# justinhj/minbpe-cc

Hardware: AMD Instinct MI355X
Metric: bpe_train_merges_per_sec (higher is better)
Workload: dtype u16; 1 GPU; BASELINE config 4: SplitMix64(seed 42) uniform-random bytes, 4294967296 bytes whole job, basic encoder (one chunk), vocab 32000, lexicographic tie-break; a step is ONE WHOLE TRAINING (pair-count scan, stream and table setup, every merge up to the vocabulary: 31744 merges); corpus_bytes=4294967296, vocab_size=32000

## Files before the change

### include/mbpe.h

```cpp
#ifndef MBPE_H
#define MBPE_H

#include <stdint.h>

#ifdef __cplusplus
extern "C" {
#endif

#define MBPE_API __attribute__((visibility("default")))

#define MBPE_MAX_VOCAB_BASIC   65534u
#define MBPE_MAX_VOCAB_ENDBIT  32766u
#define MBPE_MAX_VOCAB_CHUNKED 65518u
#define MBPE_MAX_VOCAB_WIDE    16777216u
#define MBPE_NO_BARRIER 0xFFFFFFFFu

typedef enum {
    MBPE_NEED_EXCHANGE =  1,
    MBPE_OK            =  0,
    MBPE_ERR_ARG       = -1,
    MBPE_ERR_NO_DEVICE = -2,
    MBPE_ERR_HIP       = -3,
    MBPE_ERR_VOCAB     = -4,
    MBPE_ERR_STATE     = -5,
    MBPE_ERR_OOM       = -6,
    MBPE_ERR_REGEX     = -7,
    MBPE_ERR_SPLIT_GAP = -8,
    MBPE_ERR_COMM      = -9,
    MBPE_ERR_OVERFLOW  = -10,
    MBPE_ERR_IO        = -11
} mbpe_status;

typedef struct mbpe_ctx mbpe_ctx;

typedef struct {
    uint64_t n_bytes;
    uint64_t n_chunks;
    uint64_t n_slots;
    uint64_t n_live;
    uint32_t n_merges;
    uint32_t n_compactions;
    uint64_t n_pairs;
    float    ms_pair_count;
    float    ms_begin;
    float    ms_steps;
    uint32_t pair_count_launches;
    uint32_t merge_launches;
    float    ms_merge_kernel;
    uint32_t n_batches;
    uint32_t n_fused;
    uint32_t n_fused_dropped;
    uint32_t cut_conflict;
    uint32_t cut_bucket;
    uint32_t cut_single;
    uint32_t cut_full;
    uint32_t n_validation_drops;
    float    ms_grow_table;
    float    ms_compact;
    uint32_t n_table_grows;
    uint32_t n_sel_fallback;
    uint32_t fused_launches;
    float    ms_fused_kernel;
    uint64_t fused_slots;
    uint32_t n_sel_retry;
    uint32_t adapt_limit;
    uint64_t n_sel_blocks;
    uint32_t size_hist[8];
    uint32_t n_skipped;
    uint32_t n_skip_cut;
    uint64_t exchange_words;
    uint32_t exchanges;
    uint32_t pad_;
    uint64_t fused_live_tokens;
    float    ms_pair_count_kernel;
    uint32_t pad2_;
} mbpe_stats;

MBPE_API const char *mbpe_last_error(void);
MBPE_API const char *mbpe_version(void);


MBPE_API int  mbpe_create(int device_id, mbpe_ctx **out);
MBPE_API void mbpe_destroy(mbpe_ctx *ctx);


MBPE_API int mbpe_load_corpus(mbpe_ctx *ctx, const uint8_t *text, uint64_t n_bytes,
                              const uint64_t *chunk_off, uint64_t n_chunks,
                              int text_on_device);

MBPE_API int mbpe_load_corpus_endmask(mbpe_ctx *ctx, const uint8_t *text, uint64_t n_bytes, int text_on_device,
                                      const uint8_t *endmask_dev);

MBPE_API int mbpe_load_corpus_ranges(mbpe_ctx *ctx, const uint8_t *text, uint64_t n_bytes,
                                     const uint64_t *starts, const uint64_t *ends, uint64_t n_chunks,
                                     int text_on_device);

MBPE_API int mbpe_pair_count_u8(mbpe_ctx *ctx, uint32_t *table65536_out);


MBPE_API int mbpe_train_begin(mbpe_ctx *ctx, uint32_t vocab_size);

MBPE_API int mbpe_train_steps(mbpe_ctx *ctx, uint32_t n_steps, uint32_t *steps_done_out);

MBPE_API int mbpe_train_sequences(mbpe_ctx *ctx, uint32_t n_sequences, uint32_t *merges_done_out);

MBPE_API int mbpe_train_result(mbpe_ctx *ctx, uint32_t *merges_out, int32_t *counts_out,
                               uint32_t cap_merges, uint32_t *n_merges_out);

MBPE_API int mbpe_train_lexical(mbpe_ctx *ctx, const uint8_t *text, uint64_t n_bytes,
                                const uint64_t *chunk_off, uint64_t n_chunks,
                                uint32_t vocab_size,
                                uint32_t *merges_out, int32_t *counts_out,
                                uint32_t *n_merges_out, mbpe_stats *stats_out);

MBPE_API int mbpe_train(mbpe_ctx *ctx, const uint8_t *text, uint64_t n_bytes,
                        const uint64_t *chunk_off, uint64_t n_chunks, uint32_t vocab_size,
                        int conflict_resolution,
                        uint32_t *merges_out, int32_t *counts_out,
                        uint32_t *n_merges_out, mbpe_stats *stats_out);


MBPE_API int mbpe_merges_check(const uint32_t *merges, uint32_t n_merges);

MBPE_API int mbpe_train_begin_from(mbpe_ctx *ctx, uint32_t vocab_size, const uint32_t *prior_merges, uint32_t n_prior);

MBPE_API int mbpe_train_from(mbpe_ctx *ctx, const uint8_t *text, uint64_t n_bytes,
                             const uint64_t *chunk_off, uint64_t n_chunks, uint32_t vocab_size,
                             int conflict_resolution, const uint32_t *prior_merges, uint32_t n_prior,
                             uint32_t *merges_out, int32_t *counts_out,
                             uint32_t *n_merges_out, mbpe_stats *stats_out);

MBPE_API int mbpe_get_stats(mbpe_ctx *ctx, mbpe_stats *out);


MBPE_API int mbpe_get_stream(mbpe_ctx *ctx, uint32_t *tokens_out, uint8_t *chunk_end_out,
                             uint64_t cap, uint64_t *n_out);

MBPE_API int mbpe_stream_device(mbpe_ctx *ctx, const void **slots_out, uint64_t *n_slots_out,
                                uint32_t *slot_bits_out, uint32_t *end_bit_out, uint32_t *barrier_out);

MBPE_API int mbpe_table_device(mbpe_ctx *ctx, const void **cells_out, uint32_t *vshift_out);

MBPE_API int mbpe_get_pairs(mbpe_ctx *ctx, uint32_t *first_out, uint32_t *second_out,
                            int32_t *count_out, uint64_t cap, uint64_t *n_out);

MBPE_API int mbpe_compact(mbpe_ctx *ctx);

MBPE_API int mbpe_set_option(mbpe_ctx *ctx, const char *name, int64_t value);


MBPE_API int mbpe_encode_chunks(int device_id, const uint8_t *text, uint64_t n_bytes,
                                const uint64_t *chunk_off, uint64_t n_chunks,
                                const uint32_t *merges, uint32_t n_merges,
                                uint32_t *tokens_out, uint64_t cap, uint64_t *n_out,
                                uint32_t *n_passes_out);

MBPE_API int mbpe_encode_chunks_device(int device_id, const uint8_t *text, uint64_t n_bytes,
                                       const uint64_t *chunk_off, uint64_t n_chunks,
// ... 189 lines not shown
```

### minbpe-cc_amd/csrc/kernels.hip

```cpp
#include "mbpe_dev.h"
#include <hip/hip_ext.h>

#include <algorithm>
#include <cstdlib>

namespace mbpe {

namespace {

constexpr int kWave = 64;
constexpr uint32_t kSent = 0x10000u;

__device__ __forceinline__ uint32_t lane_id() { return threadIdx.x & (kWave - 1); }
__device__ __forceinline__ uint32_t rfl(uint32_t v) { return __builtin_amdgcn_readfirstlane(v); }

typedef unsigned int u32x4 __attribute__((ext_vector_type(4)));

__device__ __forceinline__ uint32_t wave_from_next(uint32_t v, uint32_t edge) {
    return (uint32_t)__builtin_amdgcn_update_dpp((int)edge, (int)v, 0x130, 0xf, 0xf, false);
}
__device__ __forceinline__ uint32_t wave_from_prev(uint32_t v, uint32_t edge) {
    return (uint32_t)__builtin_amdgcn_update_dpp((int)edge, (int)v, 0x138, 0xf, 0xf, false);
}

// ... 2286 lines not shown
    for (int j = 0; j < 8; ++j) {
        if (s[j] != kHole) {
            if (last == kHole) first_id = s[j] & idmask;
            if ((s[j] & idmask) == last) { ++len; repeats = true; }
            else { full = full && last == kHole; len = 1; }
            lodd |= (len & 1u) ? 0u : 1u << j;
            lead |= full ? 1u << j : 0u;
            last = s[j];
        }
    }
    const bool p1_runs = h.p1 != kHole && !(h.p1 & endbit);
    const uint32_t in_last = h.p1, in_len = p1_runs ? (rb_small & 1u) : 1u;
    uint32_t rl, rn;
    const bool cross = first_id == wave_from_prev(last, in_last);
    if (__ballot(last == kHole) == 0ull && __ballot(repeats || cross) == 0ull) {
        rl = rlane(last, kWave - 1);
        rn = 1u;
    } else {
    auto join = [&](uint32_t o_last, uint32_t o_len, bool o_full) {
        if (last == kHole) { last = o_last; len = o_len; full = o_full; }
        else if (o_last != kHole) {
            if (full && (last & idmask) == o_last) { len += o_len; full = o_full; }
            else full = false;
        }
    };
    if (__ballot(last == kHole || (full && cross)) != 0ull) {
        if (lane == 0) join(in_last, in_len, false);
#pragma unroll
        for (int d = 1; d < kWave; d <<= 1) {
            const uint32_t ol = __shfl_up(last, d, kWave), on = __shfl_up(len | (full ? 0x80000000u : 0u), d, kWave);
            if (lane >= (uint32_t)d) join(ol, on & 0x7FFFFFFFu, (on >> 31) != 0u);
        }
    }
    const uint32_t lv = wave_from_prev(last, in_last), ln = wave_from_prev(len, in_len);
    const uint32_t odd = lodd ^ ((first_id == lv && (ln & 1u)) ? lead : 0u);
    if (__ballot(odd != 0u) != 0ull) {
#pragma unroll
        for (int j = 0; j < 8; ++j)
            if ((odd >> j) & 1u) s[j] = stand_in(s[j]);
    }
    rl = rlane(last, kWave - 1);
    rn = rlane(len, kWave - 1);
    }
    if (h.n1 != kHole) {
        const uint32_t n1 = h.n1;
        const bool c1 = (n1 & idmask) == rl;
        if (c1 && (rn & 1u)) h.n1 = stand_in(n1);
        rn = c1 ? rn + 1u : 1u;
        rl = n1;
        if (h.n2 != kHole && (h.n2 & idmask) == rl && (rn & 1u)) h.n2 = stand_in(h.n2);
    }
    if (p1_runs) {
        const uint32_t p1 = h.p1, p2 = h.p2;
        if (!(rb_small & 1u)) h.p1 = stand_in(p1);
        if (p2 == p1 && (rb_small & 1u)) h.p2 = stand_in(p2);
    }
}

template <int MODE>
__device__ __forceinline__ bool tt_needed(const uint32_t s[8], const uint32_t nxt[8], const Halo &h,
                                          uint32_t tile_first, const TTInfo &ti, uint32_t live_mask = 0xFFu) {
    constexpr uint32_t idmask = MODE == 1 ? 0x7FFFu : 0xFFFFu;
    auto member = [&](uint32_t v) -> bool {
        const uint32_t id = v & idmask;
        return (ti.map[id & (kTTSlots - 1u)] & 0xFFFFu) == id;
    };
    uint32_t eqm = 0;
#pragma unroll
    for (int j = 0; j < 8; ++j) eqm |= (((s[j] ^ nxt[j]) & idmask) == 0u ? 1u : 0u) << j;
    eqm &= live_mask;
    bool need = false;
    if (__ballot(eqm != 0u) != 0ull) {
#pragma unroll
        for (int j = 0; j < 8; ++j)
            if ((eqm >> j) & 1u) need = need || member(s[j]);
    }
    bool hneed = false;
    if (h.p1 != kHole && (((h.p1 ^ tile_first) & idmask) == 0u || (h.p2 != kHole && ((h.p2 ^ h.p1) & idmask) == 0u)))
        hneed = member(h.p1);
    if (h.n1 != kHole && h.n2 != kHole && ((h.n1 ^ h.n2) & idmask) == 0u) hneed = hneed || member(h.n1);
    return __ballot(need) != 0ull || hneed;
}

template <int MODE, int DIAG, bool WRITE, bool TT, class DC>
__device__ __forceinline__ uint4 fused_tile_pf(const uint4 q_orig, const uint32_t s[8], const Halo h,
                                               uint32_t old_x, uint32_t old_y, uint32_t old_z, const BatchLut &lut,
                                               uint32_t X0, uint32_t tile, TileSum *sout, uint32_t *hdr_adj, uint32_t *LR,
                                               DC &dc, bool dc_on, uint32_t &wave_rm, bool &wrote_sum,
                                               __amdgpu_buffer_rsrc_t lr_rsrc, uint32_t adj_pitch, uint16_t *stage,
                                               uint32_t *chg, bool renamed, TTInfo *ti, bool &need_rename,
                                               __amdgpu_buffer_rsrc_t t_rsrc = __amdgpu_buffer_rsrc_t(), bool use_t = false);

template <int MODE, bool HOT, bool TT, int DIAG = 0>
__global__ __launch_bounds__(kLutThreads) void k_scan_batch(const uint16_t *tok0, const uint16_t *tok1,
                                                              const TileSum *__restrict__ sin, uint32_t n_tiles,
                                                              uint32_t *__restrict__ chg, const BatchState *bs,
                                                              uint32_t *hdr_m, uint32_t *hdr_adj, uint32_t *LR,
                                                              const DevCtl *ctl, const RankEdge *le,
                                                              const RankEdge *re,
                                                              const uint32_t *__restrict__ run_in, int hot_launched,
                                                              uint32_t *T) {
    constexpr uint32_t idmask = MODE == 1 ? 0x7FFFu : 0xFFFFu;
    __shared__ BatchLutMem lut_mem;
    const uint32_t waves_per_block = kLutThreads / kWave;
    const uint32_t n_waves = gridDim.x * waves_per_block;
    __shared__ DeltaCache dc;
    const uint32_t n_keys = ctl->batch_n;
    if (n_keys < 2 || ctl->fused) return;
    if ((bs->tt_index != kNoTT) != TT) return;
    __shared__ TTInfo ti;
    const uint16_t *tok = ctl->cur ? tok1 : tok0;
    const uint32_t ctl_k_done = rfl(ctl->k_done);
    const uint32_t adj_pitch = rfl(ctl->adj_pitch);
    if (hot_mismatch<HOT>(bs->packed[0] >> 32, ctl, hot_launched)) return;
    constexpr bool dc_on = HOT;
    if (dc_on) dc_init(dc);
    BatchLut lut(&lut_mem, bs, idmask);
    lut_build(lut, bs, n_keys, idmask - 1u);
    if (TT) tt_build(ti, bs, n_keys, idmask - 1u);
    uint32_t tile = rfl(blockIdx.x * waves_per_block + threadIdx.x / kWave);
    if (tile < n_tiles) {

    const uint32_t last_tile = n_tiles - 1;
    auto clamp_tile = [&](uint64_t t) { return (uint32_t)(t < n_tiles ? t : last_tile); };
    const __amdgpu_buffer_rsrc_t sums_rsrc =
        __builtin_amdgcn_make_buffer_rsrc(const_cast<TileSum *>(sin), 0, n_tiles * 16u, 0x00020000);
    const __amdgpu_buffer_rsrc_t lr_rsrc = __builtin_amdgcn_make_buffer_rsrc(LR, 0, 0xFFFFFFFCu, 0x00020000);
    const bool use_t = T != nullptr && !HOT && ctl->cells_on != 0u && n_keys >= ctl->cells_min;
    const __amdgpu_buffer_rsrc_t t_rsrc = __builtin_amdgcn_make_buffer_rsrc(T ? T : LR, 0, T ? 0xFFFFFFFCu : 0u, 0x00020000);
    TileIn t0 = tile_issue(tok, sums_rsrc, tile);
    TileIn t1 = tile_issue(tok, sums_rsrc, clamp_tile((uint64_t)tile + n_waves));
    bool v1 = (uint64_t)tile + n_waves < n_tiles;
    for (;;) {
        const bool v2 = (uint64_t)tile + 2ull * n_waves < n_tiles;
        TileIn t2 = tile_issue(tok, sums_rsrc, clamp_tile((uint64_t)tile + 2ull * n_waves));

        const uint32_t me_nlive = rlane(t0.smw, 6) & 0xFFFFu;
        if (me_nlive != 0) {
            uint32_t s[8];
            unpack8(t0.q, s);
            Halo h;
            const uint32_t pw1 = rlane(t0.smw, 1), pw2 = rlane(t0.smw, 2);
            const uint32_t nw0 = rlane(t0.smw, 8), nw2 = rlane(t0.smw, 10);
            const bool fast = tile > 0 && tile + 1 < n_tiles && (pw2 & 0xFFFFu) >= 2 && (nw2 & 0xFFFFu) >= 2;
            if (fast) {
                h.p1 = pw1 >> 16; h.p2 = pw1 & 0xFFFFu;
                h.n1 = nw0 & 0xFFFFu; h.n2 = nw0 >> 16;
            } else {
                h = halo_slow(sin, n_tiles, tile, le, re);
            }
            uint32_t rm_unused = 0;
            bool ws_unused = false, no_rename = false;
            if (TT) tt_rename<MODE>(s, h, ti, run_in[tile]);
            fused_tile_pf<MODE, 0, false, TT>(t0.q, s, h, rlane(t0.smw, 4), rlane(t0.smw, 5), rlane(t0.smw, 6), lut,
                                              256u + ctl_k_done, tile, nullptr, hdr_adj, LR, dc, dc_on, rm_unused, ws_unused,
                                              lr_rsrc, adj_pitch, nullptr, chg, TT, &ti, no_rename, t_rsrc, use_t);
        }
        if (!v1) break;
        tile += n_waves;
        t0 = t1; t1 = t2;
        v1 = v2;
    }
    }
    if (dc_on) dc_flush(dc, LR);
    if (TT) {
        tt_flush(ti, hdr_m);
    }
}

template <int MODE, int DIAG, bool WRITE, bool TT, class DC>
__device__ __forceinline__ uint4 fused_tile_pf(const uint4 q_orig, const uint32_t s[8], const Halo h,
                                               uint32_t old_x, uint32_t old_y, uint32_t old_z, const BatchLut &lut,
                                               uint32_t X0, uint32_t tile, TileSum *sout, uint32_t *hdr_adj, uint32_t *LR,
                                               DC &dc, bool dc_on, uint32_t &wave_rm, bool &wrote_sum,
                                               __amdgpu_buffer_rsrc_t lr_rsrc, uint32_t adj_pitch, uint16_t *stage,
                                               uint32_t *chg, bool renamed, TTInfo *ti, bool &need_rename,
                                               __amdgpu_buffer_rsrc_t t_rsrc, bool use_t) {
    constexpr uint32_t idmask = MODE == 1 ? 0x7FFFu : 0xFFFFu;
    constexpr uint32_t endbit = MODE == 1 ? kEndBit : 0u;
    constexpr uint32_t kNone = 0xFFFFu;
    const uint32_t pitch = lr_pitch(X0);
    const uint32_t xcd_off = DIAG == 6 ? (__builtin_amdgcn_s_getreg((3 << 11) | 20) & 7u) * (2u * 512u * pitch) : 0u;
    auto delta_add = [&](uint32_t idx, uint32_t delta) {
        if (dc_on) dc_add(dc, true, LR, idx, delta);
        else __builtin_amdgcn_raw_ptr_buffer_atomic_add_i32((int)delta, lr_rsrc, (idx + xcd_off) << 2, 0, 0);
    };
    uint32_t lane = lane_id();
    asm volatile("" : "+v"(lane));
    const uint32_t live = old_z & 0xFFFFu;
    if (live == 0u) return q_orig;
    uint32_t tile_first = old_x & 0xFFFFu, tile_last = old_y >> 16;
    if (TT && renamed) {
        const uint32_t li = live - 1u;
        uint32_t sl = s[0];
#pragma unroll
        for (uint32_t j = 1; j < 8; ++j) sl = (li & 7u) == j ? s[j] : sl;
        tile_first = rlane(s[0], 0);
        tile_last = rlane(sl, li >> 3);
    }
    uint32_t n[8];
#pragma unroll
    for (int j = 0; j < 7; ++j) n[j] = s[j + 1];
    n[7] = wave_from_next(s[0], h.n1);
    const uint32_t ef = lane == 0 ? h.p1 : lane == 1 ? h.p2 : lane == 2 ? tile_last : (TT && lane == 3) ? h.n1 : kHole;
    const uint32_t es = (lane == 0 ? tile_first : lane == 1 ? h.p1 : (TT && lane == 3) ? h.n2 : h.n1) & idmask;
    uint32_t idx[8], eidx;
    if (lut.bytes) {
#pragma unroll
        for (int j = 0; j < 8; ++j) idx[j] = byte_entry<TT>(lut, s[j], MODE == 1 ? n[j] & idmask : n[j], idmask);
        eidx = byte_entry<TT>(lut, ef, es, idmask);
        const uint32_t all = idx[0] & idx[1] & idx[2] & idx[3] & idx[4] & idx[5] & idx[6] & idx[7] & eidx;
        if (__ballot(all != kNone) == 0ull && DIAG != 3 && DIAG != 5) return q_orig;
        if (TT) {
            bool mark = eidx == kTTMark;
#pragma unroll
            for (int j = 0; j < 8; ++j) mark = mark || idx[j] == kTTMark;
            if (__ballot(mark) != 0ull) {
                if (!renamed) { need_rename = true; return q_orig; }
#pragma unroll
                for (int j = 0; j < 8; ++j) idx[j] = idx[j] == kTTMark ? kNone : idx[j];
                eidx = eidx == kTTMark ? kNone : eidx;
            }
            eidx = lane == 3 ? kNone : eidx;
        }
    } else {
        uint32_t Hm = 0, Wm = 0;
        {
            bool second_key;
            const bool hit = pair_hit2(lut, ef, es, second_key) && !(TT && lane == 3);
            Hm = hit ? 1u : 0u;
            Wm = second_key ? 1u : 0u;
        }
#pragma unroll
        for (int j = 7; j >= 0; --j) {
            bool second_key;
            const bool hit = pair_hit2(lut, s[j], MODE == 1 ? n[j] & idmask : n[j], second_key);
            Hm = Hm + Hm + (hit ? 1u : 0u);
            Wm = Wm + Wm + (second_key ? 1u : 0u);
        }
        if (__ballot(Hm != 0u) == 0ull && DIAG != 3 && DIAG != 5) return q_orig;
#pragma unroll
        for (int j = 0; j < 8; ++j) {
            idx[j] = kNone;
            if (__ballot(((Hm >> j) & 1u) != 0u) != 0ull) {
                const uint32_t got = lut_index_known(lut, s[j], MODE == 1 ? n[j] & idmask : n[j], ((Wm >> j) & 1u) != 0u);
                idx[j] = (Hm >> j) & 1u ? got : kNone;
            }
        }
        eidx = kNone;
        if (__ballot(((Hm >> 8) & 1u) != 0u) != 0ull) {
            const uint32_t got = lut_index_known(lut, ef, es, ((Wm >> 8) & 1u) != 0u);
            eidx = (Hm >> 8) & 1u ? got : kNone;
        }
    }
    if (DIAG == 3 || DIAG == 5) {
#pragma unroll
        for (int j = 0; j < 8; ++j) asm volatile("" :: "v"(idx[j]));
        asm volatile("" :: "v"(eidx));
        return q_orig;
    }
    const uint32_t in1 = rlane(eidx, 0), in2 = rlane(eidx, 1), out1 = rlane(eidx, 2);
    {
        const uint32_t li = live - 1u;
        const bool mine = lane == (li >> 3);
#pragma unroll
        for (uint32_t j = 0; j < 8; ++j)
            if ((li & 7u) == j) { n[j] = mine ? h.n1 : n[j]; idx[j] = mine ? out1 : idx[j]; }
    }
    const uint32_t prev7 = wave_from_prev(idx[7] | (s[7] << 16), in1 | (h.p1 << 16));
    const uint32_t prev6 = wave_from_prev(idx[6], in2);
    const int lrem = (int)live - (int)(lane * 8u);
    const uint32_t Lm = lrem >= 8 ? 0xFFu : lrem <= 0 ? 0u : (1u << lrem) - 1u;
    uint32_t Am = 0, Bm = 0;
#pragma unroll
    for (int j = 0; j < 8; ++j) {
        const uint32_t pj = j == 0 ? (prev7 & 0xFFFFu) : idx[j - 1];
        Am |= (idx[j] != kNone ? 1u : 0u) << j;
        Bm |= (pj != kNone ? 1u : 0u) << j;
    }
    Bm &= Lm;
    const uint32_t ABm = Am | Bm;
    if (__ballot(ABm != 0u) == 0ull) return q_orig;

    uint32_t n2_7 = wave_from_next(n[0], h.n2);
    uint32_t n2_patch = kSent;
    if (out1 != kNone) {
        const uint32_t li = live - 1u;
        if (lane == (li >> 3)) n2_patch = li & 7u;
    }
    uint32_t out[8];
#pragma unroll
    for (int j = 0; j < 8; ++j) {
        const uint32_t self = s[j];
        uint32_t nv = ((Bm >> j) & 1u) ? kHole : self;
        if (__ballot(((Am >> j) & 1u) != 0u) != 0ull) {
            if ((Am >> j) & 1u) {
                const uint32_t p1 = j == 0 ? prev7 >> 16 : s[j > 0 ? j - 1 : 0];
                const uint32_t ppj = j == 0 ? prev6 : j == 1 ? (prev7 & 0xFFFFu) : idx[j > 1 ? j - 2 : 0];
                const uint32_t ja = idx[j];
                const uint32_t btok = n[j];
                uint32_t n2 = j < 7 ? n[j < 7 ? j + 1 : 7] : n2_7;
                n2 = n2_patch == (uint32_t)j ? h.n2 : n2;
                nv = (X0 + ja) | (btok & endbit);
                if (TT && renamed && (btok & idmask) >= idmask - (uint32_t)kTTMax)
                    atomicAdd(&ti->cnt[idmask - 1u - (btok & idmask)], 1u);
                if (DIAG != 2) {
                    const bool lo = left_open<MODE>(p1), ro = right_open<MODE>(btok, n2);
                    const uint32_t xl = p1 & idmask, yr = n2 & idmask;
                    if (use_t && lo && ro && ppj == kNone && xl < 256u && yr < 256u) {
                        __builtin_amdgcn_raw_ptr_buffer_atomic_add_i32(1, t_rsrc, ((ja << 16) | (xl << 8) | yr) << 2, 0, 0);
                    } else {
                        if (lo) {
                            if (ppj != kNone) {
                                atomicAdd(&hdr_adj[ppj * adj_pitch + ja], 1u);
                                delta_add(lr_idx(pitch, self, ppj, 1), 0xFFFFFFFFu);
                            } else {
                                delta_add(lr_idx(pitch, xl, ja, 0u), 1u);
                            }
                        }
                        if (ro) delta_add(lr_idx(pitch, yr, ja, 1u), 1u);
                    }
                }
            }
        }
        out[j] = nv;
    }
    if (TT && renamed) {
#pragma unroll
        for (int j = 0; j < 8; ++j)
            if (out[j] != kHole && (out[j] & idmask) >= idmask - (uint32_t)kTTMax)
                out[j] = ti->tok[idmask - 1u - (out[j] & idmask)] | (out[j] & endbit);
    }
    if (!WRITE) {
        if (lane == 0) atomicOr(&chg[tile >> 5], 1u << (tile & 31u));
        return q_orig;
    }
    uint32_t n_out;
    const uint4 qc = tile_compact(out, stage, n_out);
    wave_rm += live - n_out;
    uint32_t em = lane == 0 ? 3u : 0u;
    {
        const uint32_t l1 = live - 1u, l2 = live >= 2u ? live - 2u : 0u;
        em |= lane == (l1 >> 3) ? 1u << (l1 & 7u) : 0u;
        em |= lane == (l2 >> 3) ? 1u << (l2 & 7u) : 0u;
    }
    const bool edge = __ballot((ABm & em) != 0u) != 0ull;
    uint4 ns;
    if (edge || (old_z >> 16) != 1u) {
        uint32_t c[8];
        unpack8(qc, c);
        ns = wave_summary(c);
    } else {
        ns = make_uint4(old_x, old_y, (old_z & 0xFFFF0000u) | n_out, 0u);
    }
    if (lane == 0) reinterpret_cast<uint4 *>(sout)[tile] = ns;
    wrote_sum = true;
    return qc;
}

#ifndef MBPE_SKIP_PENALTY0
#define MBPE_SKIP_PENALTY0 2
#endif
#ifndef MBPE_SKIP_PENALTY_MAX
#define MBPE_SKIP_PENALTY_MAX 256
#endif
#ifndef MBPE_FUSED_WAVES
#define MBPE_FUSED_WAVES 4
#endif
template <int MODE, bool HOT, bool TT, int DIAG = 0>
__global__ __launch_bounds__(kLutThreads, MBPE_FUSED_WAVES * 256 / kLutThreads) void k_fused_batch(uint16_t *tok0, uint16_t *tok1,
                                                               const TileSum *__restrict__ sin,
                                                               TileSum *__restrict__ sout, uint32_t n_tiles,
                                                               uint32_t *__restrict__ chg, const BatchState *bs,
                                                               uint32_t *hdr_adj, uint32_t *LR, DevCtl *ctl,
                                                               const RankEdge *le, const RankEdge *re,
                                                               uint32_t *hdr_m, const uint32_t *__restrict__ run_in,
                                                               int hot_launched, uint32_t *T) {
    constexpr uint32_t idmask = MODE == 1 ? 0x7FFFu : 0xFFFFu;
    __shared__ BatchLutMem lut_mem;
    const uint32_t lane = lane_id();
    const uint32_t waves_per_block = kLutThreads / kWave;
    const uint32_t n_waves = gridDim.x * waves_per_block;
    __shared__ DeltaCacheSmall dc;
    const uint32_t n_keys = ctl->batch_n;
    if (n_keys < 2 || !ctl->fused) return;
    if ((bs->tt_index != kNoTT) != TT) return;
    __shared__ TTInfo ti;
    __shared__ __attribute__((aligned(16))) uint16_t stage_mem[kLutThreads / kWave][kTileSlots];
    uint16_t *stage = stage_mem[threadIdx.x / kWave];
    const uint16_t *tok = ctl->cur ? tok1 : tok0;
    uint16_t *dst = ctl->cur ? tok0 : tok1;
    const uint32_t X0 = 256u + ctl->k_done;
    if (hot_mismatch<HOT>(bs->packed[0] >> 32, ctl, hot_launched)) return;
    constexpr bool dc_on = HOT;
    if (dc_on) dc_init(dc);
    BatchLut lut(&lut_mem, bs, idmask);
    lut_build(lut, bs, n_keys, idmask - 1u, TT);
    if (TT) tt_build(ti, bs, n_keys, idmask - 1u);
    if (blockIdx.x == 0 && threadIdx.x == 0) ctl->marks_all = 1;
    uint32_t tile = rfl(blockIdx.x * waves_per_block + threadIdx.x / kWave);
    uint32_t wave_rm = 0;
    if (tile < n_tiles) {

    const uint32_t last_tile = n_tiles - 1;
    auto clamp_tile = [&](uint64_t t) { return (uint32_t)(t < n_tiles ? t : last_tile); };
    const __amdgpu_buffer_rsrc_t sums_rsrc =
        __builtin_amdgcn_make_buffer_rsrc(const_cast<TileSum *>(sin), 0, n_tiles * 16u, 0x00020000);
    const __amdgpu_buffer_rsrc_t lr_rsrc = __builtin_amdgcn_make_buffer_rsrc(LR, 0, 0xFFFFFFFCu, 0x00020000);
    const bool use_t = T != nullptr && !HOT && ctl->cells_on != 0u && n_keys >= ctl->cells_min;
    const __amdgpu_buffer_rsrc_t t_rsrc = __builtin_amdgcn_make_buffer_rsrc(T ? T : LR, 0, T ? 0xFFFFFFFCu : 0u, 0x00020000);
    const uint32_t adj_pitch = rfl(ctl->adj_pitch);
#ifndef MBPE_FUSED_DEPTH
#define MBPE_FUSED_DEPTH 2
#endif
    constexpr int kDepth = MBPE_FUSED_DEPTH;
    TileIn ring[kDepth];
#pragma unroll
    for (int d = 0; d < kDepth; ++d) ring[d] = tile_issue(tok, sums_rsrc, clamp_tile((uint64_t)tile + (uint64_t)d * n_waves));
    for (;;) {
        const bool v1 = (uint64_t)tile + n_waves < n_tiles;
        const TileIn t_new = tile_issue(tok, sums_rsrc, clamp_tile((uint64_t)tile + (uint64_t)kDepth * n_waves));
        const TileIn t0 = ring[0];

        uint4 outq = t0.q;
        bool wrote_sum = false;
        const uint32_t old_x = rlane(t0.smw, 4), old_y = rlane(t0.smw, 5), old_z = rlane(t0.smw, 6);
        if (DIAG == 4) {
            asm volatile("" :: "v"(t0.smw));
        } else if ((old_z & 0xFFFFu) != 0) {
            uint32_t s[8];
            unpack8(t0.q, s);
            Halo h;
            const uint32_t pw1 = rlane(t0.smw, 1), pw2 = rlane(t0.smw, 2);
            const uint32_t nw0 = rlane(t0.smw, 8), nw2 = rlane(t0.smw, 10);
            const bool fast = tile > 0 && tile + 1 < n_tiles && (pw2 & 0xFFFFu) >= 2 && (nw2 & 0xFFFFu) >= 2;
            if (fast) {
                h.p1 = pw1 >> 16; h.p2 = pw1 & 0xFFFFu;
                h.n1 = nw0 & 0xFFFFu; h.n2 = nw0 >> 16;
            } else {
                h = halo_slow(sin, n_tiles, tile, le, re);
            }
            bool renamed = false;
            bool need_rename = false;
            if (TT && !lut.bytes) {
                uint32_t nx[8];
#pragma unroll
                for (int j = 0; j < 7; ++j) nx[j] = s[j + 1];
                nx[7] = wave_from_next(s[0], h.n1);
                const uint32_t li = (old_z & 0xFFFFu) - 1u;
                const bool mine = lane == (li >> 3);
#pragma unroll
                for (uint32_t j = 0; j < 8; ++j)
                    if ((li & 7u) == j) nx[j] = mine ? h.n1 : nx[j];
                const int lrem = (int)(old_z & 0xFFFFu) - (int)(lane * 8u);
                const uint32_t lm = lrem >= 8 ? 0xFFu : lrem <= 0 ? 0u : (1u << lrem) - 1u;
                if (tt_needed<MODE>(s, nx, h, old_x & 0xFFFFu, ti, lm)) {
                    tt_rename<MODE>(s, h, ti, run_in[tile]);
                    renamed = true;
                }
            }
            outq = fused_tile_pf<MODE, DIAG, true, TT>(t0.q, s, h, old_x, old_y, old_z, lut, X0, tile, sout, hdr_adj, LR, dc,
                                                       dc_on, wave_rm, wrote_sum, lr_rsrc, adj_pitch, stage, chg, renamed, &ti,
                                                       need_rename, t_rsrc, use_t);
            if (TT && need_rename) {
                tt_rename<MODE>(s, h, ti, run_in[tile]);
                outq = fused_tile_pf<MODE, DIAG, true, TT>(t0.q, s, h, old_x, old_y, old_z, lut, X0, tile, sout, hdr_adj, LR,
                                                           dc, dc_on, wave_rm, wrote_sum, lr_rsrc, adj_pitch, stage, chg, true,
                                                           &ti, need_rename, t_rsrc, use_t);
            }
        }
        if (!wrote_sum && lane == 0) reinterpret_cast<uint4 *>(sout)[tile] = make_uint4(old_x, old_y, old_z, 0u);
        MBPE_GLOBAL_AS char *obase =
            (MBPE_GLOBAL_AS char *)uniform_ptr(reinterpret_cast<uintptr_t>(dst) + (uint64_t)tile * (kWave * 16u));
        u32x4 oq; oq.x = outq.x; oq.y = outq.y; oq.z = outq.z; oq.w = outq.w;
        __builtin_nontemporal_store(oq, (MBPE_GLOBAL_AS u32x4 *)(obase + lane * 16u));

        if (!v1) break;
        tile += n_waves;
#pragma unroll
        for (int d = 0; d + 1 < kDepth; ++d) ring[d] = ring[d + 1];
        ring[kDepth - 1] = t_new;
    }
    }
    if (dc_on) dc_flush(dc, LR);
    if (lane == 0 && wave_rm) atomicAdd(&ctl->rm, wave_rm);
    if (TT) {
        tt_flush(ti, hdr_m);
    }
}

__global__ __launch_bounds__(256) void k_pair_cells_fold(uint32_t *__restrict__ T, uint32_t *__restrict__ LR, const DevCtl *ctl) {
    __shared__ uint32_t rows[256];
    const uint32_t n = ctl->batch_n;
    if (n < ctl->cells_min || !ctl->cells_on) return;
    const uint32_t pitch = lr_pitch(256u + ctl->k_done);
    uint32_t hits = 0;
    const uint32_t t = threadIdx.x;
    for (uint32_t j = blockIdx.x; j < n; j += gridDim.x) {
        uint32_t *tj = T + (size_t)j * 65536u;
        rows[t] = 0;
        __syncthreads();
        uint32_t col = 0;
#pragma unroll 8
        for (uint32_t x = 0; x < 256u; ++x) {
            const uint32_t v = tj[x * 256u + t];
            if (__ballot(v != 0u) == 0ull) continue;
            if (v) tj[x * 256u + t] = 0;
            col += v;
            const uint32_t rs = wave_sum(v);
            if (lane_id() == 0 && rs) atomicAdd(&rows[x], rs);
        }
        __syncthreads();
        if (col) LR[lr_idx(pitch, t, j, 1u)] += col;
        if (rows[t]) LR[lr_idx(pitch, t, j, 0u)] += rows[t];
        hits += col;
        __syncthreads();
    }
    hits = wave_sum(hits);
    if (lane_id() == 0 && hits) atomicAdd(const_cast<uint32_t *>(&ctl->cell_hits), hits);
}


__global__ __launch_bounds__(kWave) void k_adj_sums(const uint32_t *__restrict__ hdr_adj, BatchState *bs, const DevCtl *ctl) {
    const uint32_t n = ctl->batch_n;
    if (n < 2) return;
    for (uint32_t j = blockIdx.x; j < n; j += gridDim.x) {
        uint32_t in = 0, out = 0;
        for (uint32_t p = threadIdx.x; p < n; p += kWave) { in += hdr_adj[p * ctl->adj_pitch + j]; out += hdr_adj[j * ctl->adj_pitch + p]; }
        in = wave_sum(in);
        out = wave_sum(out);
        if (threadIdx.x == 0) { bs->adj_in[j] = in; bs->adj_out[j] = out; }
    }
}

constexpr uint32_t kLrChunk = 4096;
__global__ __launch_bounds__(256) void k_delta_max(const uint32_t *__restrict__ LR, BatchState *bs, const DevCtl *ctl) {
    const uint32_t n_keys = ctl->batch_n;
    if (n_keys < 2) return;
    const uint32_t X = 256u + ctl->k_done;
    const uint32_t pitch = lr_pitch(X);
    const uint32_t chunks = (X + kLrChunk - 1u) / kLrChunk;
    const uint32_t n_items = 2u * n_keys * chunks;
    for (uint32_t item = blockIdx.x; item < n_items; item += gridDim.x) {
        const uint32_t row = item / chunks, x0 = (item - row * chunks) * kLrChunk;
        const uint32_t j = row >> 1, side = row & 1u, Xj = X + j;
        const uint32_t add = side ? bs->adj_out[j] : bs->adj_in[j];
        const uint32_t *cells = LR + (size_t)row * pitch;
        unsigned long long mp = 0;
#pragma unroll 4
        for (uint32_t x = x0 + threadIdx.x; x < x0 + kLrChunk && x < X; x += 256u) {
            const uint32_t v = cells[x];
            if (v) {
                const unsigned long long p = pack_best((int32_t)(v + add), side ? (Xj << 16) | x : (x << 16) | Xj);
                mp = p > mp ? p : mp;
            }
        }
        mp = wave_max_u64(mp);
        if (lane_id() == 0 && mp > __hip_atomic_load(&bs->maxp[j], __ATOMIC_RELAXED, __HIP_MEMORY_SCOPE_AGENT))
            atomicMax(&bs->maxp[j], mp);
    }
}

constexpr int kValThreads = kBatchMax < 256 ? 256 : kBatchMax > 1024 ? 1024 : kBatchMax;
constexpr int kValSlots = kBatchMax < 256 ? 256 : kBatchMax;
__global__ __launch_bounds__(256) void k_adj_max(const uint32_t *__restrict__ hdr_adj, BatchState *bs, const DevCtl *ctl) {
    const uint32_t n = ctl->batch_n;
    if (n < 2) return;
    const uint32_t X0 = 256u + ctl->k_done;
    const uint32_t n_waves = gridDim.x * (blockDim.x / kWave);
    for (uint32_t p = blockIdx.x * (blockDim.x / kWave) + threadIdx.x / kWave; p < n; p += n_waves) {
        for (uint32_t q = lane_id(); q < n; q += kWave) {
            const uint32_t w = hdr_adj[p * ctl->adj_pitch + q];
            if (!w) continue;
            const uint32_t bp = bs->key[p] & 0xFFFFu, aq = bs->key[q] >> 16;
            auto raise = [&](uint32_t j, unsigned long long v) {
                if (v > __hip_atomic_load(&bs->maxp[j], __ATOMIC_RELAXED, __HIP_MEMORY_SCOPE_AGENT)) atomicMax(&bs->maxp[j], v);
            };
            raise(q > p ? q : p, pack_best((int32_t)w, ((X0 + p) << 16) | (X0 + q)));
            raise(q, pack_best((int32_t)bs->adj_in[q], (bp << 16) | (X0 + q)));
            raise(p, pack_best((int32_t)bs->adj_out[p], ((X0 + p) << 16) | aq));
        }
    }
}

__global__ __launch_bounds__(kValThreads) void k_validate(PairTable t, DevCtl *ctl, BatchState *bs, uint32_t *hdr_m,
                                                          uint32_t *hdr_adj, uint32_t *LR) {
    static_assert(kValSlots % kValThreads == 0, "one workgroup validates a batch, kValSlots / kValThreads pairs per thread");
    constexpr uint32_t kPer = kValSlots / kValThreads;
    __shared__ unsigned long long s_run[kValSlots];
    __shared__ uint32_t s_commit, s_minfrac;
    const uint32_t tid = threadIdx.x;
    const uint32_t n = ctl->batch_n;
    if (n < 2) return;
    if (tid == 0) s_minfrac = 0xFFFFFFFFu;
    const uint32_t X0 = 256u + ctl->k_done;
    const uint32_t pitch = lr_pitch(X0);
#pragma unroll
    for (uint32_t u = 0; u < kPer; ++u) { const uint32_t p = tid + u * kValThreads; s_run[p] = p < n ? bs->maxp[p] : 0ull; }
    if (tid == 0) s_commit = n;
    __syncthreads();
    uint32_t nsh = 6;
    while ((1u << nsh) < n) ++nsh;
// ... 345 lines not shown
    if (TT) tt_build(ti, bs, n_keys, idmask - 1u);
    const uint32_t lane = lane_id();
    const uint32_t waves_per_block = kLutThreads / kWave;
    const uint32_t n_waves = gridDim.x * waves_per_block;
    uint32_t i = rfl(blockIdx.x * waves_per_block + threadIdx.x / kWave);
    if (i >= n_list) return;
    const __amdgpu_buffer_rsrc_t sums_rsrc =
        __builtin_amdgcn_make_buffer_rsrc(const_cast<TileSum *>(sin), 0, n_tiles * 16u, 0x00020000);
    const uint32_t last = n_list - 1;
    auto tile_at = [&](uint64_t k) { return list[k < n_list ? k : last]; };
    uint32_t tile0 = tile_at(i), tile1 = tile_at((uint64_t)i + n_waves), tile2 = tile_at((uint64_t)i + 2ull * n_waves);
    TileIn t0 = tile_issue(tok, sums_rsrc, tile0);
    TileIn t1 = tile_issue(tok, sums_rsrc, tile1);
    uint32_t wave_rm = 0;
    for (;;) {
        const bool has_next = (uint64_t)i + n_waves < n_list;
        const uint32_t tile3 = tile_at((uint64_t)i + 3ull * n_waves);
        const TileIn t2 = tile_issue(tok, sums_rsrc, tile2);

        const uint32_t tile = tile0;
        uint32_t s[8];
        unpack8(t0.q, s);
        Halo h;
        const uint32_t pw1 = rlane(t0.smw, 1), pw2 = rlane(t0.smw, 2);
        const uint32_t nw0 = rlane(t0.smw, 8), nw2 = rlane(t0.smw, 10);
        const bool fast = tile > 0 && tile + 1 < n_tiles && (pw2 & 0xFFFFu) >= 2 && (nw2 & 0xFFFFu) >= 2;
        if (fast) {
            h.p1 = pw1 >> 16; h.p2 = pw1 & 0xFFFFu;
            h.n1 = nw0 & 0xFFFFu; h.n2 = nw0 >> 16;
        } else {
            h = halo_slow(sin, n_tiles, tile, le, re);
        }
        uint32_t rm = 0;
        bool wrote = false;
        bool no_rename = false;
        DeltaCacheSmall no_dc;
        if (TT) tt_rename<MODE>(s, h, ti, run_in[tile]);
        const uint4 qn = fused_tile_pf<MODE, 2, true, TT>(t0.q, s, h, rlane(t0.smw, 4), rlane(t0.smw, 5), rlane(t0.smw, 6), lut,
                                                          X0, tile, sout, nullptr, nullptr, no_dc, false, rm, wrote,
                                                          __amdgpu_buffer_rsrc_t(), 0u, stage, chg, TT, &ti, no_rename);
        if (wrote) {
            reinterpret_cast<uint4 *>(tok)[(uint64_t)tile * kWave + lane] = qn;
            if (lane == 0 && marks_all) atomicOr(&chg[tile >> 5], 1u << (tile & 31u));
        } else if (lane == 0 && !marks_all) {
            atomicAnd(&chg[tile >> 5], ~(1u << (tile & 31u)));
        }
        wave_rm += rm;

        if (!has_next) break;
        i += n_waves;
        tile0 = tile1; tile1 = tile2; tile2 = tile3;
        t0 = t1; t1 = t2;
    }
    if (lane == 0 && wave_rm) atomicAdd(&ctl->rm, wave_rm);
}

__global__ void k_seq_finish(DevCtl *ctl, uint32_t *fused_flag, const BatchState *bs) {
    if (blockIdx.x || threadIdx.x) return;
    const uint32_t bs_skip_n = bs->skip_n;
    const uint32_t rm_seq = ctl->batch_n >= 2 ? ctl->rm : 0u;
    if (fused_flag) *fused_flag = ctl->fused && ctl->batch_n >= 2 ? 1u : 0u;
    if (ctl->batch_n >= 2) {
        const uint32_t rm = ctl->rm;
        ctl->removed_total += rm;
        ctl->n_live -= rm;
        ctl->rm = 0;
    }
    if (ctl->batch_n >= 2) {
        uint32_t lim = ctl->adapt_limit ? ctl->adapt_limit : (uint32_t)kBatchMax;
        if (ctl->commit_n < ctl->batch_n) lim = ctl->commit_n * 2u < 4u ? 4u : ctl->commit_n * 2u;
        else if (ctl->batch_n >= lim) lim = lim * 2u;
        ctl->adapt_limit = lim > (uint32_t)kBatchMax ? (uint32_t)kBatchMax : lim;
    }
    if (ctl->skip_off) ctl->skip_off -= 1;
    if (ctl->batch_n >= 2 && ctl->skip_failed) {
        const uint32_t pen = ctl->skip_penalty ? (ctl->skip_penalty * 2u > (uint32_t)MBPE_SKIP_PENALTY_MAX ? (uint32_t)MBPE_SKIP_PENALTY_MAX : ctl->skip_penalty * 2u)
                                               : (uint32_t)MBPE_SKIP_PENALTY0;
        ctl->skip_penalty = pen;
        ctl->skip_off = pen;
    } else if (ctl->batch_n >= 2 && bs_skip_n > 0 && ctl->skip_penalty) {
        ctl->skip_penalty /= 2u;
    }
    ctl->skip_failed = 0;
    if (ctl->cells_on && ctl->cells_min >= kCellsMinBatch && ctl->batch_n >= ctl->cells_min &&
        ctl->cell_hits * 2ull < (unsigned long long)rm_seq)
        ctl->cells_on = 0;
    ctl->cell_hits = 0;
    if (ctl->fused && ctl->batch_n >= 2) {
        ctl->n_fused += 1;
        if (ctl->commit_n == ctl->batch_n) ctl->cur ^= 1u;
        else ctl->n_fused_dropped += 1;
    }
    ctl->fused = 0;
    ctl->marks_all = 0;
    if (ctl->commit_n) ctl->size_hist[31 - __builtin_clz(ctl->commit_n) > 7 ? 7 : 31 - __builtin_clz(ctl->commit_n)] += 1;
    if (fused_flag) {
        fused_flag[1] = (uint32_t)ctl->n_live;
        fused_flag[2] = (uint32_t)(ctl->n_live >> 32);
        fused_flag[3] = ctl->commit_n;
    }
    ctl->k_done += ctl->commit_n;
    ctl->batch_n = 0;
    ctl->commit_n = 0;
    ctl->n_marked = 0;
}


constexpr int kScanThreads = 256;
constexpr int kScanPerThread = 16;
constexpr uint32_t kScanChunk = kScanThreads * kScanPerThread;

__device__ __forceinline__ unsigned long long block_sum_u64(unsigned long long v, unsigned long long *sh) {
#pragma unroll
    for (int d = kWave / 2; d > 0; d >>= 1) v += shfl_xor_u64(v, d);
    __syncthreads();
    if (lane_id() == 0) sh[threadIdx.x / kWave] = v;
    __syncthreads();
    unsigned long long r = 0;
    for (uint32_t w = 0; w < blockDim.x / kWave; ++w) r += sh[w];
    return r;
}

__global__ __launch_bounds__(kScanThreads) void k_tile_scan_partial(const TileSum *__restrict__ sums,
                                                                    uint32_t n_tiles,
                                                                    unsigned long long *__restrict__ part) {
    __shared__ unsigned long long sh[kScanThreads / kWave];
    const uint64_t base = (uint64_t)blockIdx.x * kScanChunk;
    unsigned long long s = 0;
    for (uint32_t i = threadIdx.x; i < kScanChunk; i += kScanThreads)
        if (base + i < n_tiles) s += sums[base + i].n_live;
    s = block_sum_u64(s, sh);
    if (threadIdx.x == 0) part[blockIdx.x] = s;
}

__global__ __launch_bounds__(1024) void k_tile_scan_top(unsigned long long *__restrict__ part, uint32_t n_parts,
                                                        DevCtl *ctl) {
    __shared__ unsigned long long tot[1024];
    const uint32_t per = (n_parts + 1023u) / 1024u;
    const uint32_t lo = threadIdx.x * per < n_parts ? threadIdx.x * per : n_parts;
    const uint32_t hi = lo + per < n_parts ? lo + per : n_parts;
    unsigned long long s = 0;
    for (uint32_t i = lo; i < hi; ++i) s += part[i];
    tot[threadIdx.x] = s;
    __syncthreads();
    if (threadIdx.x == 0) {
        unsigned long long run = 0;
        for (int i = 0; i < 1024; ++i) { const unsigned long long v = tot[i]; tot[i] = run; run += v; }
        ctl->scan_total = run;
    }
    __syncthreads();
    unsigned long long run = tot[threadIdx.x];
    for (uint32_t i = lo; i < hi; ++i) { const unsigned long long v = part[i]; part[i] = run; run += v; }
}

__global__ __launch_bounds__(kScanThreads) void k_tile_scan_final(const TileSum *__restrict__ sums, uint32_t n_tiles,
                                                                  const unsigned long long *__restrict__ part,
                                                                  unsigned long long *__restrict__ offsets) {
    __shared__ unsigned long long th[kScanThreads];
    const uint64_t first = (uint64_t)blockIdx.x * kScanChunk + (uint64_t)threadIdx.x * kScanPerThread;
    uint32_t v[kScanPerThread];
    unsigned long long s = 0;
#pragma unroll
    for (int i = 0; i < kScanPerThread; ++i) {
        v[i] = first + i < n_tiles ? sums[first + i].n_live : 0u;
        s += v[i];
    }
    th[threadIdx.x] = s;
// ... 487 lines not shown
    if (!v.n_tiles) return;
    const uint32_t n_chunks = (v.n_tiles + kRunChunk - 1) / kRunChunk;
    hipLaunchKernelGGL(k_run_partial, dim3(n_chunks), dim3(kRunThreads), 0, v.stream, v.sums, v.n_tiles, best, v.ctl, seq, bs,
                       v.run_part);
    hipLaunchKernelGGL(k_run_final, dim3(n_chunks), dim3(kRunThreads), 0, v.stream, v.sums, v.n_tiles, best, v.ctl, seq, bs,
                       v.run_part, v.left_edge, v.run_in);
}

void launch_merge(const StreamView &v, const BatchView &b, const unsigned long long *best, uint32_t new_id,
                  uint32_t *m_adj, int seq, const Inst &w) {
    if (!v.n_tiles) return;
    const BatchState *bs = seq ? b.bs : nullptr;
    if (inst_may_tt(w)) launch_run_lengths(v, bs, best, seq);
    static const int occ[3] = {resident_blocks(k_merge<0, false, 0>), resident_blocks(k_merge<1, false, 0>),
                               resident_blocks(k_merge<2, false, 0>)};
    const dim3 grid(tile_grid(v.n_tiles, v.n_cus, occ[slot_mode(v.endbit)])), block(kMergeThreads);
    const int hot_launched = w.hot;
#define MBPE_MERGE_ARGS v.tok, v.tok_other, v.sums, v.side, v.n_tiles, v.chg, best, new_id, b.LR, v.ctl, m_adj, v.left_edge, \
                        v.right_edge, seq, v.run_in, hot_launched
#ifdef MBPE_DIAG
    static const int diag = getenv("MBPE_MERGE_DIAG") ? atoi(getenv("MBPE_MERGE_DIAG")) : 0;
    if (diag == 1 && !v.endbit) {
        hipLaunchKernelGGL((k_merge<0, false, 1>), grid, block, 0, v.stream, MBPE_MERGE_ARGS);
        return;
    }
    if (diag == 2 && !v.endbit) {
        hipLaunchKernelGGL((k_merge<0, false, 2>), grid, block, 0, v.stream, MBPE_MERGE_ARGS);
        return;
    }
#endif
    MBPE_BY_MODE(v.endbit, {
        if (inst_takes(w, w.tt, false)) hipLaunchKernelGGL((k_merge<M, false, 0>), grid, block, 0, v.stream, MBPE_MERGE_ARGS);
        if (inst_takes(w, w.tt, true)) hipLaunchKernelGGL((k_merge<M, true, 0>), grid, block, 0, v.stream, MBPE_MERGE_ARGS);
    });
#undef MBPE_MERGE_ARGS
}

void launch_apply(const StreamView &v, const BatchView &b, PairTable t, const unsigned long long *best, uint32_t new_id,
                  const uint32_t *gm_gadj, int seq) {
    const uint32_t n_words = (v.n_tiles + 31u) / 32u;
    uint32_t blocks = (new_id + 255) / 256;
    const uint32_t want = (n_words + 255) / 256;
    if (want > blocks) blocks = want < 2048 ? want : 2048;
    hipLaunchKernelGGL(k_apply, dim3(blocks), dim3(256), 0, v.stream, t, v.ctl, best, new_id, b.LR, gm_gadj, v.sums, v.side,
                       v.chg, n_words, seq);
}

void launch_patch_sums(const StreamView &v, const unsigned long long *best, int seq) {
    const uint32_t n_words = (v.n_tiles + 31u) / 32u;
    uint32_t blocks = (n_words + 255) / 256;
    if (blocks > 2048) blocks = 2048;
    if (blocks < 1) blocks = 1;
    hipLaunchKernelGGL(k_patch_sums, dim3(blocks), dim3(256), 0, v.stream, best, v.sums, v.side, v.chg, n_words, v.ctl, seq,
                       v.n_tiles);
}

void launch_select_batch(const StreamView &v, const BatchView &b, PairTable t, unsigned long long *best,
                         const SelectArgs &a, int attempts, int first_attempt, bool fallback) {
    const hipStream_t s = v.stream;
    const uint32_t fake_id = (v.endbit == kEndBit ? 0x7FFFu : 0xFFFFu) - 1u;
    const uint32_t tt_max = 256u + a.n_target <= fake_id + 1u - (uint32_t)kTTMax ? (uint32_t)kTTMax : 1u;
    const uint32_t sel_cap = a.sel_cap < 64u ? 64u : a.sel_cap > kSelCap ? kSelCap : a.sel_cap;
    if (a.sel) {
        const int blocks = (v.n_cus > 0 ? v.n_cus : 256) * 4;
        for (int attempt = first_attempt < 0 ? 0 : first_attempt; attempt < (attempts < 1 ? 1 : attempts > 3 ? 3 : attempts); ++attempt) {
            hipLaunchKernelGGL(k_sel_scan, dim3(blocks), dim3(256), 0, s, t, v.ctl, a.sel, a.n_target, sel_cap, attempt);
            hipLaunchKernelGGL(k_sel_pick, dim3(1), dim3(kPickThreads), 0, s, v.ctl, b.bs, a.sel, best, a.n_target, a.max_batch,
                               a.fused_min, (uint32_t)v.n_ranks, attempt, fake_id, sel_cap, tt_max, a.byte_table ? 1u : 0u);
        }
    }
    if (fallback)
        hipLaunchKernelGGL(k_select_batch, dim3(1), dim3(kHierThreads), 0, s, t, v.ctl, b.bs, best, a.n_target, a.max_batch,
                           a.fused_min, (uint32_t)v.n_ranks);
}

void launch_fused_batch(const StreamView &v, const BatchView &b, const Inst &w) {
    if (!v.n_tiles) return;
    static const int occ[3] = {resident_blocks(k_fused_batch<0, false, false, 0>, kLutThreads),
                               resident_blocks(k_fused_batch<1, false, false, 0>, kLutThreads),
                               resident_blocks(k_fused_batch<2, false, false, 0>, kLutThreads)};
    const dim3 grid(tile_grid(v.n_tiles, v.n_cus, occ[slot_mode(v.endbit)], kLutThreads)), block(kLutThreads);
    const int hot_launched = w.hot;
#define MBPE_FUSED_ARGS v.tok, v.tok_other, v.sums, v.side, v.n_tiles, v.chg, b.bs, b.hdr_adj, b.LR, v.ctl, v.left_edge, \
                        v.right_edge, b.hdr_m, v.run_in, hot_launched, b.pair_cells
#ifdef MBPE_DIAG
    const int diag = getenv("MBPE_FUSED_DIAG") ? atoi(getenv("MBPE_FUSED_DIAG")) : 0;
#define MBPE_FUSED_DIAG_CASE(D)                                                                                            \
    if (diag == D && !v.endbit) {                                                                                          \
        hipLaunchKernelGGL((k_fused_batch<0, false, false, D>), grid, block, 0, v.stream, MBPE_FUSED_ARGS);                \
        hipLaunchKernelGGL((k_fused_batch<0, false, true, D>), grid, block, 0, v.stream, MBPE_FUSED_ARGS);                 \
        return;                                                                                                            \
    }
    MBPE_FUSED_DIAG_CASE(2)
    MBPE_FUSED_DIAG_CASE(3)
    MBPE_FUSED_DIAG_CASE(4)
    MBPE_FUSED_DIAG_CASE(5)
    MBPE_FUSED_DIAG_CASE(6)
#undef MBPE_FUSED_DIAG_CASE
#endif
    MBPE_BY_MODE(v.endbit, MBPE_BY_INST(w, hipLaunchKernelGGL((k_fused_batch<M, HOT, TT>), grid, block, 0, v.stream, MBPE_FUSED_ARGS)));
#undef MBPE_FUSED_ARGS
}

void launch_scan_batch(const StreamView &v, const BatchView &b, const Inst &w) {
    if (!v.n_tiles) return;
    static const int occ[3] = {resident_blocks(k_scan_batch<0, false, false, 0>, kLutThreads),
                               resident_blocks(k_scan_batch<1, false, false, 0>, kLutThreads),
                               resident_blocks(k_scan_batch<2, false, false, 0>, kLutThreads)};
    const dim3 grid(tile_grid(v.n_tiles, v.n_cus, occ[slot_mode(v.endbit)], kLutThreads)), block(kLutThreads);
    const int hot_launched = w.hot;
    MBPE_BY_MODE(v.endbit, MBPE_BY_INST(w, hipLaunchKernelGGL((k_scan_batch<M, HOT, TT, 0>), grid, block, 0, v.stream, v.tok,
                                                             v.tok_other, v.sums, v.n_tiles, v.chg, b.bs, b.hdr_m, b.hdr_adj, b.LR,
                                                             v.ctl, v.left_edge, v.right_edge, v.run_in, hot_launched,
                                                             b.pair_cells)));
}

void launch_pair_cells_fold(const StreamView &v, const BatchView &b, uint32_t n_hint) {
    if (!b.pair_cells) return;
    if (n_hint < 64u) n_hint = 64u;
    if (n_hint > 1024u) n_hint = 1024u;
    hipLaunchKernelGGL(k_pair_cells_fold, dim3(n_hint), dim3(256), 0, v.stream, b.pair_cells, b.LR, v.ctl);
}

void launch_batch_tables(const StreamView &v, const BatchView &b, PairTable t, uint32_t id_upper, uint32_t n_hint) {
    const hipStream_t s = v.stream;
    if (n_hint < 64u) n_hint = 64u;
    if (n_hint > (uint32_t)kBatchMax) n_hint = kBatchMax;
    const uint64_t cells = (uint64_t)id_upper * kBatchMax;
    uint32_t blocks = (uint32_t)((cells + 255) / 256);
    if (blocks > 2048) blocks = 2048;
    if (blocks < 8) blocks = 8;
    hipLaunchKernelGGL(k_adj_sums, dim3(n_hint), dim3(kWave), 0, s, b.hdr_adj, b.bs, v.ctl);
    hipLaunchKernelGGL(k_delta_max, dim3(blocks < 1024 ? blocks : 1024), dim3(256), 0, s, b.LR, b.bs, v.ctl);
    hipLaunchKernelGGL(k_adj_max, dim3(n_hint / 4), dim3(256), 0, s, b.hdr_adj, b.bs, v.ctl);
    hipLaunchKernelGGL(k_validate, dim3(1), dim3(kValThreads), 0, s, t, v.ctl, b.bs, b.hdr_m, b.hdr_adj, b.LR);
    if (t.cells) {
        uint32_t j_parts = (n_hint + kApplyTile - 1) / kApplyTile;
        if (j_parts > kApplyJParts) j_parts = kApplyJParts;
        uint32_t grid = ((id_upper + kApplyTile - 1) / kApplyTile) * j_parts;
        if (grid < 256u) grid = 256u;
        hipLaunchKernelGGL(k_apply_batch_dense, dim3(grid), dim3(256), 0, s, t, v.ctl, b.bs, b.hdr_m, b.hdr_adj, b.LR, j_parts);
    } else {
        hipLaunchKernelGGL(k_apply_batch, dim3(blocks), dim3(256), 0, s, t, v.ctl, b.bs, b.hdr_m, b.hdr_adj, b.LR);
    }
}

void launch_rewrite_marked(const StreamView &v, const BatchView &b, const Inst &w) {
    if (!v.n_tiles) return;
    const uint32_t n_words = (v.n_tiles + 31u) / 32u;
    hipLaunchKernelGGL(k_list_marked, dim3((n_words + 255) / 256), dim3(256), 0, v.stream, v.chg, n_words, v.tile_list, v.ctl,
                       v.n_tiles);
    static const int occ[3] = {resident_blocks(k_rewrite_marked<0, false>, kLutThreads),
                               resident_blocks(k_rewrite_marked<1, false>, kLutThreads),
                               resident_blocks(k_rewrite_marked<2, false>, kLutThreads)};
    const dim3 grid(tile_grid(v.n_tiles, v.n_cus, occ[slot_mode(v.endbit)], kLutThreads)), block(kLutThreads);
#define MBPE_REWRITE_ARGS v.tok, v.tok_other, v.sums, v.side, v.n_tiles, v.chg, v.tile_list, b.bs, v.ctl, v.left_edge, \
                          v.right_edge, v.run_in
    MBPE_BY_MODE(v.endbit, {
        hipLaunchKernelGGL((k_rewrite_marked<M, false>), grid, block, 0, v.stream, MBPE_REWRITE_ARGS);
        if (inst_may_tt(w)) hipLaunchKernelGGL((k_rewrite_marked<M, true>), grid, block, 0, v.stream, MBPE_REWRITE_ARGS);
    });
#undef MBPE_REWRITE_ARGS
}

__global__ void k_seq_info(const DevCtl *ctl, const BatchState *bs, const unsigned long long *best, uint32_t *out) {
    if (blockIdx.x || threadIdx.x) return;
    const uint32_t n = ctl->batch_n;
    unsigned long long top = 0;
    uint32_t tt = 0;
    if (n >= 2) {
        top = bs->packed[0] >> 32;
        tt = bs->tt_index != kNoTT ? 1u : 0u;
    } else if (n == 1) {
        const unsigned long long b = best[ctl->k_done];
        const uint32_t key = ~(uint32_t)b;
        top = b >> 32;
        tt = (top != 0 && (key >> 16) == (key & 0xFFFFu)) ? 1u : 0u;
    }
    out[0] = ctl->k_done;
    out[1] = n;
    out[2] = ctl->fused;
    out[3] = tt;
    out[4] = dc_wanted(top, ctl->n_live * ctl->n_ranks) ? 1u : 0u;
    out[5] = ctl->k_limit;
    out[6] = ctl->sel_ok;
    out[7] = 0;
}

void launch_seq_info(const StreamView &v, const BatchView &b, const unsigned long long *best, uint32_t *out) {
    hipLaunchKernelGGL(k_seq_info, dim3(1), dim3(64), 0, v.stream, v.ctl, b.bs, best, out);
}

void launch_seq_finish(const StreamView &v, const BatchView &b, uint32_t *fused_flag) {
    hipLaunchKernelGGL(k_seq_finish, dim3(1), dim3(64), 0, v.stream, v.ctl, fused_flag, b.bs);
}

void launch_tile_scan(const StreamView &v, unsigned long long *offsets) {
    if (!v.n_tiles) return;
    unsigned long long *part = offsets + v.n_tiles;
    const uint32_t n_parts = (v.n_tiles + kScanChunk - 1) / kScanChunk;
    hipLaunchKernelGGL(k_tile_scan_partial, dim3(n_parts), dim3(kScanThreads), 0, v.stream, v.sums, v.n_tiles, part);
    hipLaunchKernelGGL(k_tile_scan_top, dim3(1), dim3(1024), 0, v.stream, part, n_parts, v.ctl);
    hipLaunchKernelGGL(k_tile_scan_final, dim3(n_parts), dim3(kScanThreads), 0, v.stream, v.sums, v.n_tiles, part, offsets);
}
// ... 70 lines not shown
```

### minbpe-cc_amd/csrc/mbpe_dev.h

```cpp
#ifndef MBPE_DEV_H
#define MBPE_DEV_H

#include <hip/hip_runtime.h>
#include <stdint.h>

namespace mbpe {

constexpr uint32_t kHole = 0xFFFFu;
constexpr uint32_t kEndBit = 0x8000u;
constexpr uint32_t kBarrier = 0xFFEEu;

constexpr int kTile = 512;
constexpr int kMergeThreads = 256;
#ifndef MBPE_LUT_THREADS
#define MBPE_LUT_THREADS 1024
#endif
constexpr int kLutThreads = MBPE_LUT_THREADS;
constexpr int kSlotsPerLane = 8;

struct __attribute__((aligned(16))) TileSum {
    uint16_t head0, head1;
    uint16_t tail1, tail0;
    uint16_t n_live;
    uint16_t tail_run;
    uint16_t pad0, pad1;
};
static_assert(sizeof(TileSum) == 16, "TileSum must be 16 bytes");

struct RankEdge {
    uint32_t head0, head1;
    uint32_t tail1, tail0;
    uint32_t n_live_lo, n_live_hi;
    uint32_t tail_run_lo, tail_run_hi;
};

constexpr uint32_t kEmptyKey = 0xFFFFFFFFu;
constexpr unsigned long long kEmptySlot = 0xFFFFFFFFFFFFFFFFull;

constexpr int kBlockShift = 10;
constexpr uint32_t kBlockSize = 1u << kBlockShift;

struct PairTable {
    unsigned long long *hslot;
    uint32_t *ekey;
    int32_t  *ecnt;
    unsigned long long *bmax;
    unsigned long long *smax;
    uint32_t  hmask;
    uint32_t  ecap;
    uint32_t *cells;
    uint32_t  vshift;
};
constexpr uint32_t kPresent = 0x80000000u;

struct DevCtl {
    uint32_t n_entries;
    uint32_t err;
    uint32_t m;
    uint32_t adj;
    unsigned long long removed_total;
    unsigned long long n_live;
    unsigned long long scan_total;
    uint32_t rm;
    uint32_t k_done;
    uint32_t k_limit;
    uint32_t batch_n;
    uint32_t commit_n;
    uint32_t n_batches;
    uint32_t n_marked;
    uint32_t cur;
    uint32_t fused;
    uint32_t n_fused;
    uint32_t n_fused_dropped;
    uint32_t cut_conflict, cut_bucket, cut_single, cut_full;
    uint32_t n_validation_drops;
    unsigned long long sel_T;
    uint32_t sel_n;
    uint32_t sel_ok;
    uint32_t n_sel_fallback;
    uint32_t sel_retry;
    uint32_t adapt_limit;
    uint32_t recent_n;
    uint32_t n_sel_retry;
    uint32_t sel_mode;
    uint32_t n_ranks;
    uint32_t size_hist[8];
    uint32_t n_skipped;
    uint32_t n_skip_cut;
    uint32_t skip_off;
    uint32_t skip_penalty;
    uint32_t skip_failed;
    uint32_t skip_red_q16;
    unsigned long long n_sel_blocks;
    uint32_t first_mode;
    uint32_t first_tie;
    uint32_t marks_all;
    uint32_t cells_on;
    uint32_t cell_hits;
    uint32_t cells_min;
    uint32_t adj_pitch;

};

#ifndef MBPE_BATCH_MAX
#define MBPE_BATCH_MAX 4096
#endif
constexpr int kBatchMax = MBPE_BATCH_MAX;
constexpr int kBatchDefault = kBatchMax;
static_assert((kBatchMax & (kBatchMax - 1)) == 0 && kBatchMax >= 64,
              "a power of two: grid strides over the delta arrays keep a thread on one pair index");
#ifndef MBPE_SEL_CAP
#define MBPE_SEL_CAP 8192
#endif
constexpr uint32_t kSelCap = MBPE_SEL_CAP;
struct SelList {
    unsigned long long packed[kSelCap];
    uint32_t eidx[kSelCap];
};

#ifndef MBPE_TT_MAX
#define MBPE_TT_MAX 16
#endif
constexpr int kTTMax = MBPE_TT_MAX;
static_assert(0xFFFFu - (uint32_t)MBPE_TT_MAX > kBarrier, "the barrier id must lie below the stand-in ids");
constexpr uint32_t kTTSlots = 256;
#ifndef MBPE_SKIP_MAX
#define MBPE_SKIP_MAX 32
#endif
constexpr int kSkipMax = MBPE_SKIP_MAX;
constexpr uint32_t kCellsMinBatch = 512;
constexpr uint32_t kNoTT = 0xFFFFFFFFu;
struct BatchState {
    uint32_t key[kBatchMax];
    uint32_t eidx[kBatchMax];
    unsigned long long packed[kBatchMax];
    unsigned long long maxp[kBatchMax];
    uint32_t adj_in[kBatchMax];
    uint32_t adj_out[kBatchMax];
    uint32_t tt_index;
    uint32_t tt_token;
    uint32_t tt_n;
    uint32_t hash_mul;
    uint32_t byte_lut;
    uint32_t skip_n;
    uint32_t skip_key[kSkipMax];
    uint32_t skip_pos[kSkipMax];
    unsigned long long skip_packed[kSkipMax];
};

inline uint32_t batch_header_words(uint32_t adj_pitch) { return (uint32_t)kBatchMax + adj_pitch * adj_pitch; }
__host__ __device__ inline uint32_t lr_pitch(uint32_t ids) { return (ids + 63u) & ~63u; }
__host__ __device__ inline unsigned long long lr_words(uint32_t ids, uint32_t n_pairs) {
    return 2ull * (n_pairs ? n_pairs : 1u) * lr_pitch(ids);
}

constexpr uint32_t kErrTableFull   = 1u;
constexpr uint32_t kErrNegCount    = 2u;
constexpr uint32_t kErrMissingPair = 4u;
constexpr uint32_t kErrCountRange  = 8u;
constexpr uint32_t kErrHotSkipped  = 16u;

__host__ __device__ inline unsigned long long pack_best(int32_t count, uint32_t key) {
    return ((unsigned long long)(uint32_t)count << 32) | (uint32_t)(~key);
}

struct StreamView {
    hipStream_t stream;
    uint16_t *tok, *tok_other;
    TileSum *sums;
    TileSum *side;
    uint32_t n_tiles;
    uint32_t *chg;
    uint32_t *tile_list;
    uint32_t *run_in;
    unsigned long long *run_part;
    DevCtl *ctl;
    const RankEdge *left_edge, *right_edge;
    int rank, n_ranks;
    uint32_t endbit;
    int n_cus;
};

struct BatchView {
    BatchState *bs;
    uint32_t *hdr_m, *hdr_adj;
    uint32_t *LR;
    uint32_t *pair_cells;
};

struct Inst { bool known, tt, hot; };
inline Inst inst_any(bool hot_possible) { return Inst{false, false, hot_possible}; }
inline Inst inst_known(bool tt, bool hot) { return Inst{true, tt, hot}; }
inline bool inst_takes(const Inst &w, bool tt, bool hot) { return w.known ? w.tt == tt && w.hot == hot : !hot || w.hot; }
inline bool inst_may_tt(const Inst &w) { return !w.known || w.tt; }

void launch_fill_u32(hipStream_t s, uint32_t *p, uint64_t n, uint32_t v);
void launch_fill_u16(hipStream_t s, uint16_t *p, uint64_t n, uint16_t v);

size_t pair_count_scratch_bytes(int n_workgroups);
void launch_pair_count_u8(hipStream_t s, const uint8_t *text, uint64_t n,
                          const uint8_t *endmask, uint32_t *bp, int n_workgroups, uint32_t *scratch,
                          hipEvent_t start = nullptr, hipEvent_t stop = nullptr);

void launch_widen(hipStream_t s, const uint8_t *text, uint64_t n, const uint8_t *endmask,
                  uint16_t *tok, uint64_t n_slots_padded);
void launch_widen_barrier(hipStream_t s, const uint8_t *text, uint64_t n, const uint8_t *endmask,
                          uint16_t *tok, uint64_t n_slots);

void launch_summarize(const StreamView &v);

void launch_table_init(hipStream_t s, const uint32_t *bp, PairTable t, DevCtl *ctl);
void launch_table_rehash(hipStream_t s, PairTable t, DevCtl *ctl);

void launch_argmax(hipStream_t s, PairTable t, const DevCtl *ctl, unsigned long long *best, bool hierarchical);

size_t first_state_bytes();
void launch_first_init(hipStream_t s, void *fs);
void launch_first_tiebreak(const StreamView &v, PairTable t, unsigned long long *best, void *fs, uint32_t *xf, int seq,
                           int phase);

void launch_merge(const StreamView &v, const BatchView &b, const unsigned long long *best, uint32_t new_id,
                  uint32_t *m_adj, int seq, const Inst &w);
void launch_run_lengths(const StreamView &v, const BatchState *bs, const unsigned long long *best, int seq);

void launch_apply(const StreamView &v, const BatchView &b, PairTable t, const unsigned long long *best, uint32_t new_id,
                  const uint32_t *gm_gadj, int seq);
void launch_patch_sums(const StreamView &v, const unsigned long long *best, int seq);

struct SelectArgs {
    SelList *sel;
    uint32_t n_target, max_batch, fused_min, sel_cap;
    bool byte_table;
};
void launch_select_batch(const StreamView &v, const BatchView &b, PairTable t, unsigned long long *best,
                         const SelectArgs &a, int attempts = 3,
                         int first_attempt = 0 ,
                         bool fallback = true );
void launch_scan_batch(const StreamView &v, const BatchView &b, const Inst &w);
void launch_fused_batch(const StreamView &v, const BatchView &b, const Inst &w);
void launch_pair_cells_fold(const StreamView &v, const BatchView &b, uint32_t n_hint);
void launch_batch_tables(const StreamView &v, const BatchView &b, PairTable t, uint32_t id_upper, uint32_t n_hint);
void launch_rewrite_marked(const StreamView &v, const BatchView &b, const Inst &w);
void launch_seq_info(const StreamView &v, const BatchView &b, const unsigned long long *best, uint32_t *out);
void launch_seq_finish(const StreamView &v, const BatchView &b, uint32_t *fused_flag);

inline size_t tile_scan_scratch(uint32_t n_tiles) { return (size_t)n_tiles / 4096 + 2; }
void launch_tile_scan(const StreamView &v, unsigned long long *offsets);
void launch_compact_scatter(const StreamView &v, const unsigned long long *offsets);

inline uint32_t exchange_header_words(int n_ranks) { return (uint32_t)((2 + 8 * n_ranks + 3) / 4 * 4); }
void launch_rank_edge(const StreamView &v, uint32_t *hdr);
void launch_compose_edges(hipStream_t s, uint32_t *hdr, int rank, int n_ranks, RankEdge *left, RankEdge *right);
constexpr uint32_t kPairCountWords = 4;
void launch_boundary_pairs(hipStream_t s, uint32_t *bp, const uint32_t *hdr, int n_ranks, uint32_t endbit,
                           uint32_t *pcount);
void launch_pair_total(hipStream_t s, const uint32_t *bp, const uint32_t *pcount, unsigned long long expect,
                       unsigned long long *sum_out, DevCtl *ctl);

struct PairBins { uint32_t *key, *cnt; uint32_t mask; };
struct ResumeTally { unsigned long long positions, total; uint32_t distinct, err; };
void launch_slots_from_tokens(hipStream_t s, const uint32_t *tok, uint64_t n_tok, uint32_t endbit, uint16_t *slots,
                              uint64_t n_slots);
void launch_token_ends(hipStream_t s, const uint32_t *tok, uint64_t n_tok, unsigned long long *n_ends);
void launch_pair_count_tokens(hipStream_t s, const uint32_t *tok, uint64_t n_tok, uint32_t ids, PairTable t, PairBins bins,
                              ResumeTally *tally, int n_cus);
void launch_bins_seal_dense(hipStream_t s, PairTable t, uint32_t ids, DevCtl *ctl, ResumeTally *tally);
void launch_bins_tally(hipStream_t s, PairBins bins, ResumeTally *tally);
void launch_bins_insert(hipStream_t s, PairBins bins, PairTable t, DevCtl *ctl);
void launch_resume_check(hipStream_t s, const ResumeTally *tally, DevCtl *ctl);

}

#endif
```

### minbpe-cc_amd/csrc/train.cpp

```cpp
#include "mbpe.h"
#include "mbpe_dev.h"
#include "wide.h"
#include "split.h"
#include "hip_host.h"

#include <dlfcn.h>
#include <rccl/rccl.h>

#include <algorithm>
#include <chrono>
#include <cstddef>
#include <cstdio>
#include <cstring>
#include <map>
#include <string>
#include <unordered_map>
#include <vector>

using namespace mbpe;

namespace {

#define HIPCHK(expr) MBPE_HIP_CHECK(expr, false)

// ... 37 lines not shown
    static Rccl r;
    static bool tried = false;
    if (tried) return r;
    tried = true;
    for (const char *n : {"librccl.so.1", "librccl.so", "/opt/rocm/lib/librccl.so.1"}) {
        r.lib = dlopen(n, RTLD_NOW | RTLD_LOCAL);
        if (r.lib) break;
    }
    if (!r.lib) { r.why = "librccl.so.1 not found"; return r; }
#define MBPE_BIND(field, name) \
    r.field = reinterpret_cast<decltype(r.field)>(dlsym(r.lib, name)); \
    if (!r.field) { r.why = std::string("missing RCCL symbol ") + name; return r; }
    MBPE_BIND(GetUniqueId, "ncclGetUniqueId")
    MBPE_BIND(CommInitRank, "ncclCommInitRank")
    MBPE_BIND(CommDestroy, "ncclCommDestroy")
    MBPE_BIND(AllReduce, "ncclAllReduce")
    MBPE_BIND(GetErrorString, "ncclGetErrorString")
#undef MBPE_BIND
    r.ok = true;
    return r;
}
}

enum class Phase {
    None,
    BeginCounts,
    BeginFirst,
    StepDeltas,
    StepFirst,
    SeqDeltas,
    SeqEdges,
};

struct Exchange { uint32_t *buf; size_t words; };

struct mbpe_ctx {
    int device = 0;
    hipStream_t stream = nullptr;
    hipEvent_t ev0 = nullptr, ev1 = nullptr;
    int n_cus = 256;

    const uint8_t *d_text = nullptr;
    uint8_t *d_text_owned = nullptr;
    uint8_t *d_endmask = nullptr;
    uint64_t n_bytes = 0;
    uint64_t n_chunks = 0;
    bool chunked = false;
    uint64_t n_barriers = 0;
    bool barrier = false;
    bool loaded = false;
    bool inert = false;

    uint32_t *pc_scratch = nullptr;
    uint32_t *pc_bp = nullptr;
    void *first_state = nullptr;
    uint32_t *xf = nullptr;

    uint16_t *tok[2] = {nullptr, nullptr};
    int cur = 0;
    uint64_t cap_slots = 0;
    uint64_t n_slots = 0;
    uint32_t n_tiles = 0;
    TileSum *sums = nullptr;
    TileSum *side = nullptr;
    uint32_t *chg = nullptr;
    uint32_t *tile_list = nullptr;
    SelList *sel = nullptr;
    uint32_t *run_in = nullptr;
    int seq_slot = -1;
    unsigned long long *offsets = nullptr;

    PairTable tab = {};
    uint32_t hcap = 0;
    DevCtl *ctl = nullptr;
    unsigned long long *best = nullptr;
    uint32_t *xb = nullptr;
    uint32_t hdr_words = 0;
    uint32_t hdrb_words = 0;
    uint32_t *hdr_m = nullptr, *hdr_adj = nullptr;
    uint32_t *LR = nullptr;
    BatchState *bs = nullptr;
    uint32_t *xb0 = nullptr;
    uint32_t h_pcount[kPairCountWords] = {};
    uint32_t *pair_cells = nullptr;
    RankEdge *d_left = nullptr, *d_right = nullptr;

    uint32_t vocab_size = 0;
    uint32_t n_target = 0;
    uint32_t k = 0;
    uint32_t n_valid = 0;
    bool begun = false;
    bool exhausted = false;
    uint32_t n_prior = 0;
    std::vector<unsigned long long> h_prior;
    ResumeTally *tally = nullptr;
    float ms_replay = 0;
    double merges_per_seq = 0;
    uint32_t first_b = 0, first_s = 0;
    bool first_legacy = false;
    DevCtl h_ctl = {};

    int rank = 0, n_ranks = 1;
    bool comm_external = false;
    void *nccl_comm = nullptr;
    Phase pending = Phase::None;
    Exchange pending_x = {};
    uint32_t pending_target = 0;

    int64_t opt_compact_den = 16;
    int64_t opt_batch = 16;
    int64_t opt_time_kernels = 0;
    int64_t opt_force_exchange = 0;
    int64_t opt_hier_argmax = -1;
    int64_t opt_multi_merge = 1;
    int64_t opt_max_batch = kBatchDefault;
    int64_t opt_fused_min = 24;
    bool opt_byte_table = true;
    int64_t opt_sel_cap = kSelCap;
    int64_t opt_threshold_select = 1;
    int64_t opt_dense_table = -1;
    int hot_possible = 1;
    unsigned long long last_top = ~0ull;
    int64_t opt_barrier = -1;
    int64_t opt_first_batches = 0;
    int64_t opt_first = 0;
    int64_t opt_pc_repeat = 1;
    uint32_t k_upper = 0;
    int sel_attempts = 3;
    uint32_t max_batch_eff = kBatchMax, adj_pitch = kBatchMax;
    uint32_t *h_seq = nullptr;
    uint32_t *d_seq_info = nullptr;
    int64_t opt_pair_cells = -1;
    int64_t opt_lockstep = -1;
    hipEvent_t ev_sel = nullptr;
    std::vector<hipEvent_t> kev;
    std::vector<hipEvent_t> kev_f;
    uint32_t *seq_flags = nullptr;
    std::vector<uint32_t> h_seq_flags;

    bool wide = false;
    bool wide_active = false;
    uint32_t vocab_total = 0;
    uint32_t n_target_total = 0;
    int64_t opt_wide_from = -1;
    int64_t opt_first_wide = 0;
    bool wfirst = false;
    uint32_t *wtok[2] = {nullptr, nullptr};
    int wcur = 0;
    uint32_t *wval = nullptr, *wscratch = nullptr;
    WideTable wtab = {};
    WideCtl *wctl = nullptr;
    WideBest *wbest = nullptr;
    unsigned long long *warg = nullptr;
    WideFirst *wfs = nullptr;
    uint64_t wn_upper = 0;
    uint32_t wk = 0;
    WideCtl h_wctl = {};
    std::vector<WideBest> h_wbest;

    mbpe_stats stats = {};

    std::unordered_map<void *, size_t> pool_live;
    std::multimap<size_t, void *> pool_idle;
};

namespace {

template <typename T>
hipError_t tmalloc(mbpe_ctx *c, T **p, size_t bytes) {
    if (bytes == 0) bytes = 4;
    auto it = c->pool_idle.find(bytes);
    if (it != c->pool_idle.end()) {
        *p = static_cast<T *>(it->second);
        c->pool_live[it->second] = bytes;
        c->pool_idle.erase(it);
        return hipSuccess;
    }
    void *q = nullptr;
    hipError_t e = hipMalloc(&q, bytes);
    if (e == hipErrorOutOfMemory && !c->pool_idle.empty()) {
        pool_trim(c);
        e = hipMalloc(&q, bytes);
    }
    if (e != hipSuccess) return e;
    c->pool_live[q] = bytes;
    *p = static_cast<T *>(q);
    return hipSuccess;
}

template <typename T>
void tfree(mbpe_ctx *c, T *&p) {
    if (!p) return;
    auto it = c->pool_live.find((void *)p);
    if (it != c->pool_live.end()) {
        c->pool_idle.emplace(it->second, it->first);
        c->pool_live.erase(it);
    } else {
        (void)hipFree((void *)p);
    }
    p = nullptr;
}

template <typename T>
void trelease(mbpe_ctx *c, T *p) {
    if (!p) return;
    c->pool_live.erase((void *)p);
    (void)hipFree((void *)p);
}

void pool_trim(mbpe_ctx *c) {
    for (auto &kv : c->pool_idle) (void)hipFree(kv.second);
    c->pool_idle.clear();
}

int sync_ctl(mbpe_ctx *c) {
    HIPCHK(hipMemcpyAsync(&c->h_ctl, c->ctl, sizeof(DevCtl), hipMemcpyDeviceToHost, c->stream));
    HIPCHK(hipStreamSynchronize(c->stream));
    c->cur = (int)(c->h_ctl.cur & 1u);
#ifdef MBPE_DIAG
    if (getenv("MBPE_MERGE_DIAG") || getenv("MBPE_FUSED_DIAG")) c->h_ctl.err = 0;
#endif
    if (c->h_ctl.err) {
        char buf[320];
        snprintf(buf, sizeof(buf), "device error flags 0x%x (1=pair table full, 2=negative count, 4=missing pair, "
                                   "8=a pair occurs 2^31 times or more, or the byte-pair counts do not add up to the "
                                   "pairs scanned (a count reached 2^32), 16=a stream pass was skipped)",
                 c->h_ctl.err);
        mbpe_host::set_last_error(buf);
        return MBPE_ERR_OVERFLOW;
    }
    return MBPE_OK;
}

template <typename Enqueue>
int timed_group(mbpe_ctx *c, Enqueue enqueue) {
    HIPCHK(hipEventRecord(c->ev0, c->stream));
    int rc = enqueue();
    if (rc != MBPE_OK) return rc;
    HIPCHK(hipEventRecord(c->ev1, c->stream));
    rc = sync_ctl(c);
    if (rc != MBPE_OK) return rc;
    HIPCHK(hipGetLastError());
    float ms = 0;
    HIPCHK(hipEventElapsedTime(&ms, c->ev0, c->ev1));
    c->stats.ms_steps += ms;
    return MBPE_OK;
}

void free_training(mbpe_ctx *c) {
    tfree(c, c->tok[0]); tfree(c, c->tok[1]);
    tfree(c, c->sums); tfree(c, c->side); tfree(c, c->chg); tfree(c, c->tile_list);
    tfree(c, c->offsets);
    tfree(c, c->tab.hslot); tfree(c, c->tab.ekey); tfree(c, c->tab.ecnt); tfree(c, c->tab.cells);
    tfree(c, c->tab.bmax); tfree(c, c->tab.smax);
    tfree(c, c->ctl); tfree(c, c->best); tfree(c, c->xb); tfree(c, c->xb0); tfree(c, c->pair_cells);
    tfree(c, c->d_left); tfree(c, c->d_right); tfree(c, c->bs); tfree(c, c->sel); tfree(c, c->seq_flags); tfree(c, c->run_in);
    tfree(c, c->first_state);
    tfree(c, c->xf);
    tfree(c, c->tally);
    tfree(c, c->wtok[0]); tfree(c, c->wtok[1]); tfree(c, c->wval); tfree(c, c->wscratch);
    tfree(c, c->wtab.keys); tfree(c, c->wtab.cnts); tfree(c, c->wctl); tfree(c, c->wbest); tfree(c, c->warg);
    tfree(c, c->wfs);
    c->wtab = {};
    c->wfirst = false;
    c->wide_active = false;
    c->wk = 0;
    c->wn_upper = 0;
    c->h_wbest.clear();
    c->LR = nullptr;
    c->pending = Phase::None;
    c->begun = false;
    c->k = c->n_valid = c->n_prior = 0;
    c->exhausted = false;
}

void free_corpus(mbpe_ctx *c) {
    dfree(c->d_text_owned);
    dfree(c->d_endmask);
    c->d_text = nullptr;
    c->loaded = false;
}

static inline bool dense_possible(const mbpe_ctx *c) { return c->vocab_size <= 32768; }
static inline bool use_dense(const mbpe_ctx *c) {
    if (!dense_possible(c)) return false;
    if (c->wide) return false;
    return c->opt_dense_table != 0;
}

int alloc_table_dense(mbpe_ctx *c) {
    uint32_t vshift = 8;
    while ((1u << vshift) < c->vocab_size) ++vshift;
    c->tab = {};
    c->tab.vshift = vshift;
    c->tab.ecap = 1u << (2 * vshift);
    const size_t cells = (size_t)1 << (2 * vshift);
    HIPCHK(tmalloc(c, &c->tab.cells, cells * 4));
    HIPCHK(hipMemsetAsync(c->tab.cells, 0, cells * 4, c->stream));
    const size_t nb = (cells >> kBlockShift) + 2, ns = (cells >> (2 * kBlockShift)) + 2;
    HIPCHK(tmalloc(c, &c->tab.bmax, nb * 8));
    HIPCHK(tmalloc(c, &c->tab.smax, ns * 8));
    HIPCHK(hipMemsetAsync(c->tab.bmax, 0, nb * 8, c->stream));
    HIPCHK(hipMemsetAsync(c->tab.smax, 0, ns * 8, c->stream));
    return MBPE_OK;
}

int alloc_table(mbpe_ctx *c, uint32_t ecap) {
    c->tab.ecap = ecap;
    c->hcap = next_pow2((uint64_t)ecap * 2);
    c->tab.hmask = c->hcap - 1;
    HIPCHK(tmalloc(c, &c->tab.hslot, (size_t)c->hcap * 8));
    HIPCHK(tmalloc(c, &c->tab.ekey, (size_t)ecap * 4));
    HIPCHK(tmalloc(c, &c->tab.ecnt, (size_t)ecap * 4));
    const size_t nb = ((size_t)ecap >> kBlockShift) + 2, ns = ((size_t)ecap >> (2 * kBlockShift)) + 2;
    HIPCHK(tmalloc(c, &c->tab.bmax, nb * 8));
    HIPCHK(tmalloc(c, &c->tab.smax, ns * 8));
    HIPCHK(hipMemsetAsync(c->tab.bmax, 0, nb * 8, c->stream));
    HIPCHK(hipMemsetAsync(c->tab.smax, 0, ns * 8, c->stream));
    launch_fill_u32(c->stream, reinterpret_cast<uint32_t *>(c->tab.hslot), (uint64_t)c->hcap * 2, 0xFFFFFFFFu);
    return MBPE_OK;
}

uint64_t batch_headroom(const mbpe_ctx *c, uint32_t steps) {
    uint64_t per = 2ull * c->vocab_size + 1;
    return per * steps;
}

uint64_t table_cap_limit(const mbpe_ctx *c) {
    uint64_t v = c->vocab_size;
    uint64_t lim = v * v;
    if (lim > (1ull << 30)) lim = 1ull << 30;
    return std::max<uint64_t>(lim, 1024);
}

struct WallTimer {
    float *acc;
    std::chrono::steady_clock::time_point t0 = std::chrono::steady_clock::now();
    explicit WallTimer(float *a) : acc(a) {}
    ~WallTimer() { *acc += std::chrono::duration<float, std::milli>(std::chrono::steady_clock::now() - t0).count(); }
};

int grow_table(mbpe_ctx *c, uint64_t want) {
    if (c->tab.cells) return MBPE_OK;
    WallTimer timer(&c->stats.ms_grow_table);
    c->stats.n_table_grows++;
    uint64_t lim = table_cap_limit(c);
    uint64_t ecap = std::min<uint64_t>(std::max<uint64_t>(want, (uint64_t)c->tab.ecap * 4), lim);
    if (ecap <= c->tab.ecap) return MBPE_OK;
    PairTable old = c->tab;
    c->tab = {};
    int rc = alloc_table(c, (uint32_t)ecap);
    if (rc != MBPE_OK) return rc;
    uint32_t n = c->h_ctl.n_entries;
    HIPCHK(hipMemcpyAsync(c->tab.ekey, old.ekey, (size_t)n * 4, hipMemcpyDeviceToDevice, c->stream));
    HIPCHK(hipMemcpyAsync(c->tab.ecnt, old.ecnt, (size_t)n * 4, hipMemcpyDeviceToDevice, c->stream));
    HIPCHK(hipMemcpyAsync(c->tab.bmax, old.bmax, (((size_t)old.ecap >> kBlockShift) + 2) * 8,
                          hipMemcpyDeviceToDevice, c->stream));
    HIPCHK(hipMemcpyAsync(c->tab.smax, old.smax, (((size_t)old.ecap >> (2 * kBlockShift)) + 2) * 8,
                          hipMemcpyDeviceToDevice, c->stream));
    launch_table_rehash(c->stream, c->tab, c->ctl);
    HIPCHK(hipStreamSynchronize(c->stream));
    trelease(c, old.hslot); trelease(c, old.ekey); trelease(c, old.ecnt);
    trelease(c, old.bmax); trelease(c, old.smax);
    return MBPE_OK;
}

int ensure_pc_scratch(mbpe_ctx *c) {
    if (!c->pc_scratch) HIPCHK(hipMalloc(&c->pc_scratch, pair_count_scratch_bytes(c->n_cus)));
    return MBPE_OK;
}

int ensure_events(std::vector<hipEvent_t> &pool, size_t n) {
    while (pool.size() < n) {
        hipEvent_t e;
        HIPCHK(hipEventCreate(&e));
        pool.push_back(e);
    }
    return MBPE_OK;
}

inline uint32_t endbit_of(const mbpe_ctx *c) { return !c->chunked ? 0u : c->barrier ? kBarrier : kEndBit; }

inline bool is_multi(const mbpe_ctx *c) { return c->n_ranks > 1 || c->opt_force_exchange; }

enum TokOrder { kBuffers01, kLiveFirst };

StreamView stream_view(const mbpe_ctx *c, TokOrder order) {
    const int first = order == kLiveFirst ? c->cur : 0;
    const bool multi = is_multi(c);
    StreamView v = {};
    v.stream = c->stream;
    v.tok = c->tok[first], v.tok_other = c->tok[1 - first];
    v.sums = c->sums, v.side = c->side, v.n_tiles = c->n_tiles;
    v.chg = c->chg, v.tile_list = c->tile_list;
    v.run_in = c->run_in, v.run_part = c->offsets + c->n_tiles;
    v.ctl = c->ctl;
    v.left_edge = multi ? c->d_left : nullptr, v.right_edge = multi ? c->d_right : nullptr;
    v.rank = c->rank, v.n_ranks = std::max(1, c->n_ranks);
    v.endbit = endbit_of(c), v.n_cus = c->n_cus;
    return v;
}

BatchView batch_view(const mbpe_ctx *c) { return BatchView{c->bs, c->hdr_m, c->hdr_adj, c->LR, c->pair_cells}; }

int do_compact(mbpe_ctx *c) {
    if (!c->n_tiles) return MBPE_OK;
    WallTimer timer(&c->stats.ms_compact);
    const int dst = 1 - c->cur;
    const StreamView v = stream_view(c, kLiveFirst);
    launch_tile_scan(v, c->offsets);
    launch_compact_scatter(v, c->offsets);
    const uint64_t live = c->h_ctl.n_live;
    const uint64_t padded = std::max<uint64_t>(round_up(live, kTile), kTile);
    launch_fill_u16(c->stream, c->tok[dst] + live, padded - live, (uint16_t)kHole);
    c->cur = dst;
    c->n_slots = padded;
    c->n_tiles = (uint32_t)(padded / kTile);
    launch_summarize(stream_view(c, kLiveFirst));
    DevCtl patch = c->h_ctl;
    patch.removed_total = 0;
    HIPCHK(hipMemcpyAsync(&c->ctl->removed_total, &patch.removed_total, sizeof(patch.removed_total),
                          hipMemcpyHostToDevice, c->stream));
    HIPCHK(hipMemsetD32Async(reinterpret_cast<hipDeviceptr_t>(&c->ctl->cur), c->cur, 1, c->stream));
    c->h_ctl.cur = (uint32_t)c->cur;
    HIPCHK(hipStreamSynchronize(c->stream));
    c->h_ctl.removed_total = 0;
    c->stats.n_compactions++;
    return MBPE_OK;
}

}

namespace mbpe_host {
int ctx_device(const mbpe_ctx *c) { return c->device; }
}

extern "C" {

int mbpe_create(int device_id, mbpe_ctx **out) {
    if (!out) { mbpe_host::set_last_error("mbpe_create: out is NULL"); return MBPE_ERR_ARG; }
    *out = nullptr;
    int n = 0;
    hipError_t e = hipGetDeviceCount(&n);
    if (e != hipSuccess || n <= 0 || device_id < 0 || device_id >= n) {
        mbpe_host::set_last_error("no usable HIP device (the MI355X path has no CPU fallback)");
        return MBPE_ERR_NO_DEVICE;
    }
    HIPCHK(hipSetDevice(device_id));
    mbpe_ctx *c = new mbpe_ctx();
    c->device = device_id;
    hipDeviceProp_t prop;
    if (hipGetDeviceProperties(&prop, device_id) == hipSuccess) c->n_cus = prop.multiProcessorCount;
    if (hipStreamCreateWithFlags(&c->stream, hipStreamNonBlocking) != hipSuccess ||
        hipEventCreate(&c->ev0) != hipSuccess || hipEventCreate(&c->ev1) != hipSuccess ||
        hipEventCreateWithFlags(&c->ev_sel, hipEventDisableTiming) != hipSuccess ||
        hipHostMalloc(reinterpret_cast<void **>(&c->h_seq), 64, hipHostMallocDefault) != hipSuccess) {
        mbpe_host::set_last_error("could not create HIP stream / events");
        delete c;
        return MBPE_ERR_HIP;
    }
    *out = c;
    return MBPE_OK;
}

void mbpe_destroy(mbpe_ctx *c) {
    if (!c) return;
    (void)hipSetDevice(c->device);
    if (c->stream) (void)hipStreamSynchronize(c->stream);
    free_training(c);
    pool_trim(c);
    free_corpus(c);
    dfree(c->pc_scratch);
    dfree(c->pc_bp);
    if (c->nccl_comm && rccl().ok) rccl().CommDestroy(c->nccl_comm);
    for (hipEvent_t e : c->kev) (void)hipEventDestroy(e);
    for (hipEvent_t e : c->kev_f) (void)hipEventDestroy(e);
    if (c->ev0) (void)hipEventDestroy(c->ev0);
    if (c->ev1) (void)hipEventDestroy(c->ev1);
    if (c->ev_sel) (void)hipEventDestroy(c->ev_sel);
    if (c->h_seq) (void)hipHostFree(c->h_seq);
    dfree(c->d_seq_info);
    if (c->stream) (void)hipStreamDestroy(c->stream);
    delete c;
}

int mbpe_set_option(mbpe_ctx *c, const char *name, int64_t value) {
    if (!c || !name) return MBPE_ERR_ARG;
    std::string n(name);
    if (n == "compact_den") c->opt_compact_den = value;
    else if (n == "batch") c->opt_batch = std::max<int64_t>(1, value);
    else if (n == "time_kernels") c->opt_time_kernels = value;
    else if (n == "force_exchange") c->opt_force_exchange = value;
    else if (n == "hier_argmax") c->opt_hier_argmax = value;
    else if (n == "multi_merge") c->opt_multi_merge = value;
    else if (n == "max_batch") c->opt_max_batch = std::min<int64_t>(std::max<int64_t>(1, value), kBatchMax);
    else if (n == "fused_min") c->opt_fused_min = std::max<int64_t>(2, value);
    else if (n == "dense_table") c->opt_dense_table = value;
    else if (n == "threshold_select") c->opt_threshold_select = value != 0;
    else if (n == "conflict_resolution") {
        if (value != 0 && value != 1) { mbpe_host::set_last_error("conflict_resolution: 0 = first, 1 = lexical"); return MBPE_ERR_ARG; }
        if (c->begun && (c->pending != Phase::None || (c->k < c->n_target && !c->exhausted))) {
            mbpe_host::set_last_error("conflict_resolution cannot change in the middle of a training");
            return MBPE_ERR_STATE;
        }
        c->opt_first = value == 0;
    }
    else if (n == "chunk_barrier") c->opt_barrier = value < 0 ? -1 : value != 0;
    else if (n == "first_batches") c->opt_first_batches = value != 0;
    else if (n == "sel_cap") c->opt_sel_cap = std::min<int64_t>(std::max<int64_t>(64, value), kSelCap);
    else if (n == "byte_table") c->opt_byte_table = value != 0;
    else if (n == "lockstep") c->opt_lockstep = value < 0 ? -1 : value != 0;
    else if (n == "pair_cells") c->opt_pair_cells = value < 0 ? -1 : value != 0;
    else if (n == "wide_from") c->opt_wide_from = value < 0 ? -1 : value;
    else if (n == "first_wide") c->opt_first_wide = value != 0;
    else if (n == "pc_repeat") c->opt_pc_repeat = std::min<int64_t>(std::max<int64_t>(1, value), 1000);
    else { mbpe_host::set_last_error("unknown option " + n); return MBPE_ERR_ARG; }
    return MBPE_OK;
}

static int load_reset(mbpe_ctx *c, uint64_t n_bytes, bool chunked, uint64_t n_chunks) {
    HIPCHK(hipSetDevice(c->device));
    free_training(c);
    free_corpus(c);
    if (n_bytes != c->n_bytes || chunked != c->chunked) pool_trim(c);
    c->n_bytes = n_bytes;
    c->chunked = chunked;
    c->n_chunks = chunked ? n_chunks : 1;
    c->n_barriers = 0;
    c->barrier = false;
    c->inert = false;
    return MBPE_OK;
}

static int load_finish(mbpe_ctx *c, const uint8_t *text, uint64_t n_bytes, int text_on_device, const uint8_t *mask,
                       size_t mask_bytes, hipMemcpyKind mask_kind) {
    const uint64_t n_vec = (n_bytes + 15) / 16;
    if (text_on_device) {
        c->d_text = text;
    } else {
        HIPCHK(hipMalloc(&c->d_text_owned, std::max<uint64_t>(n_vec * 16, 16)));
        if (n_bytes) HIPCHK(hipMemcpyAsync(c->d_text_owned, text, n_bytes, hipMemcpyHostToDevice, c->stream));
        c->d_text = c->d_text_owned;
    }
    if (mask) {
        HIPCHK(hipMalloc(&c->d_endmask, mask_bytes));
        HIPCHK(hipMemcpyAsync(c->d_endmask, mask, mask_bytes, mask_kind, c->stream));
    }
    HIPCHK(hipStreamSynchronize(c->stream));
    c->loaded = true;
    c->stats = {};
    c->stats.n_bytes = n_bytes;
    c->stats.n_chunks = c->n_chunks;
    return MBPE_OK;
}

int mbpe_load_corpus(mbpe_ctx *c, const uint8_t *text, uint64_t n_bytes, const uint64_t *chunk_off,
                     uint64_t n_chunks, int text_on_device) {
    if (!c || (!text && n_bytes)) { mbpe_host::set_last_error("mbpe_load_corpus: NULL argument"); return MBPE_ERR_ARG; }
    const int rc0 = load_reset(c, n_bytes, chunk_off != nullptr, n_chunks);
    if (rc0 != MBPE_OK) return rc0;
    if (chunk_off) {
        if (chunk_off[0] != 0 || chunk_off[n_chunks] != n_bytes) {
            mbpe_host::set_last_error("chunk_off must start at 0 and end at n_bytes");
            return MBPE_ERR_ARG;
        }
        for (uint64_t i = 0; i < n_chunks; ++i)
            if (chunk_off[i] > chunk_off[i + 1]) {
                mbpe_host::set_last_error("chunk_off must be ascending");
                return MBPE_ERR_ARG;
            }
    }
    if (text_on_device && ((uintptr_t)text & 15)) {
        mbpe_host::set_last_error("device text must be 16-byte aligned");
        return MBPE_ERR_ARG;
    }

    std::vector<uint8_t> tmp;
    const uint8_t *h_text = text;
    if (text_on_device && n_bytes) {
        bool need_all = chunk_off != nullptr;
        uint64_t take = need_all ? n_bytes : std::min<uint64_t>(n_bytes, 64);
        tmp.resize(take);
        HIPCHK(hipMemcpy(tmp.data(), text, take, hipMemcpyDeviceToHost));
        h_text = tmp.data();
    }
    const uint64_t n_vec = (n_bytes + 15) / 16;
    std::vector<uint8_t> mask;
    if (chunk_off) {
        mask.assign(n_vec * 2 + 16, 0);
        uint64_t dropped = 0;
        for (uint64_t ci = 0; ci < n_chunks; ++ci) {
            uint64_t s = chunk_off[ci], e = chunk_off[ci + 1];
            if (e == s) continue;
            mask[(e - 1) >> 3] |= (uint8_t)(1u << ((e - 1) & 7));
            if (h_text[s] == 0 && stoi_parses(h_text + s + 1, e - s - 1)) {
// ... 137 lines not shown
    c->stats.ms_pair_count /= (float)reps;
    c->stats.ms_pair_count_kernel = 0;
    if (!c->inert && c->n_bytes >= 2) {
        float sum = 0;
        for (int r = 0; r < reps; ++r) {
            float km = 0;
            HIPCHK(hipEventElapsedTime(&km, c->kev[2 * r], c->kev[2 * r + 1]));
            sum += km;
        }
        c->stats.ms_pair_count_kernel = sum / (float)reps;
    }
    c->stats.pair_count_launches += (uint32_t)reps;
#ifdef MBPE_PC_STAMPS
    {
        std::vector<unsigned long long> st((size_t)c->n_cus * 16);
        HIPCHK(hipMemcpy(st.data(), reinterpret_cast<const char *>(c->pc_scratch) + (size_t)c->n_cus * 32768 * 4, st.size() * 8,
                         hipMemcpyDeviceToHost));
        unsigned long long t0 = ~0ull;
        for (int w = 0; w < c->n_cus; ++w) if (st[16 * w] && st[16 * w] < t0) t0 = st[16 * w];
        for (int k = 0; k < 16; ++k) {
            double lo = 1e30, hi = 0, sum = 0; int cnt = 0;
            for (int w = 0; w < c->n_cus; ++w) {
                if (!st[16 * w + k]) continue;
                const double us = (double)(st[16 * w + k] - t0) * 0.01;
                lo = std::min(lo, us); hi = std::max(hi, us); sum += us; ++cnt;
            }
            if (cnt) fprintf(stderr, "pc stamp %2d: min %8.2f avg %8.2f max %8.2f us (%d workgroups)\n", k, lo, sum / cnt, hi, cnt);
        }
    }
#endif
    return MBPE_OK;
}


static inline bool use_hier(const mbpe_ctx *c) {
    if (c->opt_hier_argmax >= 0) return c->opt_hier_argmax != 0;
    if (c->tab.cells) return c->tab.ecap > (1u << 20);
    return c->h_ctl.n_entries > (1u << 20);
}

static size_t begin_exchange_words(const mbpe_ctx *c) { return 65536 + (size_t)c->hdr_words + kPairCountWords; }

struct ResumeSrc { const uint32_t *tok; uint64_t n_tok; const uint32_t *prior; uint32_t n_prior; };

static int count_token_pairs(mbpe_ctx *c, const ResumeSrc *rs, uint64_t want);

static int begin_local(mbpe_ctx *c, uint32_t vocab_size, const ResumeSrc *rs = nullptr) {
    free_training(c);
    c->vocab_size = vocab_size;
    c->n_target = vocab_size - 256;
    c->k = c->n_valid = c->n_prior = rs ? rs->n_prior : 0;
    c->exhausted = false;
    c->first_legacy = false;
    c->sel_attempts = 3;
    c->merges_per_seq = 0;
    c->first_b = c->first_s = 0;

    const uint64_t n = rs ? rs->n_tok : c->inert ? 0 : c->n_bytes;
    const uint64_t n_bar = c->barrier ? c->n_barriers : 0;
    const uint64_t dense_slots = std::max<uint64_t>(round_up(n + n_bar, kTile), kTile);
    c->n_slots = c->barrier ? std::max<uint64_t>(2 * round_up(n, kTile / 2), kTile) : dense_slots;
    c->cap_slots = dense_slots;
    if (c->n_slots / kTile > 0x0FFFFFF0ull) { mbpe_host::set_last_error("corpus shard too large"); return MBPE_ERR_ARG; }
    c->n_tiles = (uint32_t)(c->n_slots / kTile);
    c->hdr_words = exchange_header_words(c->n_ranks);
    c->max_batch_eff = (uint32_t)std::min<int64_t>(c->opt_max_batch, is_multi(c) ? 1024 : kBatchMax);
    c->adj_pitch = (uint32_t)round_up(std::max<uint32_t>(c->max_batch_eff, 64u), 64);
    c->hdrb_words = (batch_header_words(c->adj_pitch) + 3) / 4 * 4;
    HIPCHK(tmalloc(c, &c->tok[0], c->n_slots * 2));
    HIPCHK(tmalloc(c, &c->tok[1], c->cap_slots * 2));
    HIPCHK(tmalloc(c, &c->sums, (size_t)c->n_tiles * sizeof(TileSum)));
    HIPCHK(tmalloc(c, &c->side, (size_t)c->n_tiles * sizeof(TileSum)));
    HIPCHK(tmalloc(c, &c->chg, ((size_t)c->n_tiles / 32 + 2) * 4));
    HIPCHK(tmalloc(c, &c->tile_list, ((size_t)c->n_tiles + 64) * 4));
    HIPCHK(hipMemsetAsync(c->chg, 0, ((size_t)c->n_tiles / 32 + 2) * 4, c->stream));
    HIPCHK(tmalloc(c, &c->offsets, ((size_t)c->n_tiles + tile_scan_scratch(c->n_tiles)) * 8));
    const size_t xb_words = (size_t)c->hdr_words + c->hdrb_words + lr_words(vocab_size, c->max_batch_eff) + 8;
    const size_t xb0_words = begin_exchange_words(c);
    HIPCHK(tmalloc(c, &c->xb, xb_words * 4));
    HIPCHK(tmalloc(c, &c->xb0, xb0_words * 4));
    HIPCHK(hipMemsetAsync(c->xb, 0, xb_words * 4, c->stream));
    HIPCHK(hipMemsetAsync(c->xb0, 0, xb0_words * 4, c->stream));
    if (c->opt_pair_cells > 0 || (c->opt_pair_cells < 0 && c->n_slots >= (64ull << 20))) {
        const size_t cells = (size_t)c->max_batch_eff * 65536u;
        HIPCHK(tmalloc(c, &c->pair_cells, cells * 4));
        HIPCHK(hipMemsetAsync(c->pair_cells, 0, cells * 4, c->stream));
    }
    c->hdr_m = c->xb + c->hdr_words;
    c->hdr_adj = c->hdr_m + kBatchMax;
    c->LR = c->xb + c->hdr_words + c->hdrb_words;
    HIPCHK(tmalloc(c, &c->bs, sizeof(BatchState)));
    HIPCHK(tmalloc(c, &c->sel, sizeof(SelList)));
    HIPCHK(tmalloc(c, &c->run_in, ((size_t)c->n_tiles + 64) * 4));
    HIPCHK(tmalloc(c, &c->seq_flags, 4096 * 4 * 4));
    HIPCHK(hipMemsetAsync(c->bs, 0, sizeof(BatchState), c->stream));
    HIPCHK(hipMemsetAsync(c->seq_flags, 0, 4096 * 4 * 4, c->stream));
    if (c->opt_first) {
        HIPCHK(tmalloc(c, &c->first_state, first_state_bytes()));
        launch_first_init(c->stream, c->first_state);
        if (is_multi(c)) {
            HIPCHK(tmalloc(c, &c->xf, (size_t)c->hdr_words * 4));
            HIPCHK(hipMemsetAsync(c->xf, 0, (size_t)c->hdr_words * 4, c->stream));
        }
    }
    c->k_upper = c->k;
    HIPCHK(tmalloc(c, &c->d_left, sizeof(RankEdge)));
    HIPCHK(tmalloc(c, &c->d_right, sizeof(RankEdge)));
    HIPCHK(tmalloc(c, &c->ctl, sizeof(DevCtl)));
    HIPCHK(tmalloc(c, &c->best, ((size_t)c->n_target + 2) * 8));
    {
        DevCtl init = {};
        init.n_live = n + n_bar;
        init.k_done = c->k;
        init.n_ranks = (uint32_t)std::max(1, c->n_ranks);
        init.first_mode = c->opt_first ? 1u : 0u;
        init.adj_pitch = c->adj_pitch;
        init.cells_on = c->pair_cells ? 1u : 0u;
        init.cells_min = c->opt_pair_cells > 0 ? 2u : kCellsMinBatch;
        c->h_ctl = init;
        HIPCHK(hipMemcpyAsync(c->ctl, &c->h_ctl, sizeof(DevCtl), hipMemcpyHostToDevice, c->stream));
    }
    HIPCHK(hipMemsetAsync(c->best, 0, ((size_t)c->n_target + 2) * 8, c->stream));
    if (c->k) {
        c->h_prior.resize(c->k);
        for (uint32_t i = 0; i < c->k; ++i)
            c->h_prior[i] = pack_best(-1, (rs->prior[2 * i] << 16) | rs->prior[2 * i + 1]);
        HIPCHK(hipMemcpyAsync(c->best, c->h_prior.data(), (size_t)c->k * 8, hipMemcpyHostToDevice, c->stream));
    }

    uint64_t want = 65536 + 2 * batch_headroom(c, (uint32_t)c->opt_batch);
    want = std::max<uint64_t>(want, n / 8);
    want = std::min<uint64_t>(want, table_cap_limit(c));
    int rc = use_dense(c) ? alloc_table_dense(c) : rs ? MBPE_OK : alloc_table(c, (uint32_t)want);
    if (rc != MBPE_OK) return rc;

    rc = ensure_pc_scratch(c);
    if (rc != MBPE_OK) return rc;
    pool_trim(c);
    HIPCHK(hipEventRecord(c->ev0, c->stream));
    if (!rs && n >= 2) launch_pair_count_u8(c->stream, c->d_text, n, c->d_endmask, c->xb0, c->n_cus, c->pc_scratch);
    c->cur = 0;
    if (rs) launch_slots_from_tokens(c->stream, rs->tok, n, endbit_of(c), c->tok[0], c->n_slots);
    if (c->barrier) {
        if (!rs) launch_widen_barrier(c->stream, c->d_text, n, c->d_endmask, c->tok[0], c->n_slots);
        launch_summarize(stream_view(c, kLiveFirst));
        const double ms_compact = c->stats.ms_compact;
        rc = do_compact(c);
        if (rc != MBPE_OK) return rc;
        c->stats.n_compactions--;
        c->stats.ms_compact = ms_compact;
        tfree(c, c->tok[0]);
        pool_trim(c);
        HIPCHK(tmalloc(c, &c->tok[0], c->cap_slots * 2));
    } else {
        if (!rs) launch_widen(c->stream, c->d_text, n, c->d_endmask, c->tok[0], c->n_slots);
        launch_summarize(stream_view(c, kLiveFirst));
    }
    if (rs) return count_token_pairs(c, rs, want);
    if (is_multi(c)) {
        uint32_t *hdr = c->xb0 + 65536;
        launch_rank_edge(stream_view(c, kLiveFirst), hdr);
        const uint64_t p = pairs_scanned(c);
        for (uint32_t i = 0; i < kPairCountWords; ++i) c->h_pcount[i] = (uint32_t)(p >> (16 * i)) & 0xFFFFu;
        HIPCHK(hipMemcpyAsync(hdr + c->hdr_words, c->h_pcount, sizeof(c->h_pcount), hipMemcpyHostToDevice, c->stream));
    }
    return MBPE_OK;
}

static int count_token_pairs(mbpe_ctx *c, const ResumeSrc *rs, uint64_t want) {
    const uint32_t ids = 256 + rs->n_prior;
    HIPCHK(tmalloc(c, &c->tally, sizeof(ResumeTally)));
    HIPCHK(hipMemsetAsync(c->tally, 0, sizeof(ResumeTally), c->stream));
    if (c->tab.cells) {
        launch_pair_count_tokens(c->stream, rs->tok, rs->n_tok, ids, c->tab, PairBins{nullptr, nullptr, 0}, c->tally, c->n_cus);
        launch_bins_seal_dense(c->stream, c->tab, ids, c->ctl, c->tally);
    } else {
        const uint64_t most = std::min<uint64_t>(rs->n_tok, (uint64_t)ids * ids);
        if (most > (1ull << 30)) {
            mbpe_host::set_last_error("mbpe_train_begin_from: more than 2^30 pairs to count into the hashed table");
            return MBPE_ERR_OVERFLOW;
        }
        PairBins bins = {nullptr, nullptr, next_pow2(std::max<uint64_t>(2 * most, 1024)) - 1};
        const size_t slots = (size_t)bins.mask + 1;
        HIPCHK(tmalloc(c, &bins.key, slots * 4));
        HIPCHK(tmalloc(c, &bins.cnt, slots * 4));
        launch_fill_u32(c->stream, bins.key, slots, kEmptyKey);
        HIPCHK(hipMemsetAsync(bins.cnt, 0, slots * 4, c->stream));
        launch_pair_count_tokens(c->stream, rs->tok, rs->n_tok, ids, c->tab, bins, c->tally, c->n_cus);
        launch_bins_tally(c->stream, bins, c->tally);
        ResumeTally h = {};
        HIPCHK(hipMemcpyAsync(&h, c->tally, sizeof(h), hipMemcpyDeviceToHost, c->stream));
        HIPCHK(hipStreamSynchronize(c->stream));
        int rc = MBPE_OK;
        if (h.distinct > table_cap_limit(c)) {
            mbpe_host::set_last_error("mbpe_train_begin_from: the stream holds more distinct pairs than the pair table can");
            rc = MBPE_ERR_OVERFLOW;
        }
        want = std::max<uint64_t>(want, (uint64_t)h.distinct + 2 * batch_headroom(c, (uint32_t)c->opt_batch));
        want = std::min<uint64_t>(want, table_cap_limit(c));
        if (rc == MBPE_OK) rc = alloc_table(c, (uint32_t)want);
// ... 65 lines not shown
    }
}

static void step_finish_a(mbpe_ctx *c) {
    const bool multi = is_multi(c);
    launch_apply(stream_view(c, kLiveFirst), batch_view(c), c->tab, c->best + c->k, 256 + c->k, multi ? c->xb : nullptr, 0);
    if (multi) launch_compose_edges(c->stream, c->xb, c->rank, c->n_ranks, c->d_left, c->d_right);
    launch_argmax(c->stream, c->tab, c->ctl, c->best + c->k + 1, use_hier(c));
    if (c->opt_first) first_tiebreak(c, c->best + c->k + 1, 0, first_sharded(c) ? 1 : 0);
}

static size_t exchange_words(const mbpe_ctx *c, uint32_t ids, uint32_t n_pairs) {
    return (size_t)c->hdr_words + c->hdrb_words + (size_t)lr_words(ids, n_pairs);
}

static_assert(offsetof(DevCtl, batch_n) == offsetof(DevCtl, k_done) + 8 && offsetof(DevCtl, commit_n) == offsetof(DevCtl, k_done) + 12,
              "seq_info_enqueue copies k_done, k_limit, batch_n, commit_n as four consecutive words");
static int seq_info_enqueue(mbpe_ctx *c) {
    HIPCHK(hipMemcpyAsync(c->h_seq, &c->ctl->k_done, 16, hipMemcpyDeviceToHost, c->stream));
    HIPCHK(hipEventRecord(c->ev_sel, c->stream));
    return MBPE_OK;
}
static int seq_info_wait(mbpe_ctx *c, uint32_t *ids, uint32_t *n_pairs) {
    HIPCHK(hipEventSynchronize(c->ev_sel));
    *ids = 256u + c->h_seq[0];
    *n_pairs = c->h_seq[2];
    return MBPE_OK;
}


static inline bool use_batches(const mbpe_ctx *c) {
    return c->opt_multi_merge != 0 && (!c->opt_first || (c->opt_first_batches && !c->first_legacy && !is_multi(c)));
}

static constexpr uint64_t kLockstepSlots = 32ull << 20;
static inline bool use_lockstep(const mbpe_ctx *c) {
    if (is_multi(c) || c->opt_first) return false;
    if (c->opt_lockstep >= 0) return c->opt_lockstep != 0;
    return c->n_slots <= kLockstepSlots;
}

static SelectArgs select_args(const mbpe_ctx *c) {
    SelectArgs a = {};
    a.sel = c->opt_threshold_select ? c->sel : nullptr;
    a.n_target = c->n_target, a.max_batch = std::min<uint32_t>((uint32_t)c->opt_max_batch, c->max_batch_eff);
    a.fused_min = (uint32_t)c->opt_fused_min, a.sel_cap = (uint32_t)c->opt_sel_cap, a.byte_table = c->opt_byte_table;
    return a;
}

static uint32_t *seq_flags_of(const mbpe_ctx *c) { return c->seq_slot >= 0 ? c->seq_flags + 4 * c->seq_slot : nullptr; }

static uint32_t batch_hint(const mbpe_ctx *c) {
    return c->merges_per_seq > 0 && c->merges_per_seq < 128.0 ? 256u : c->max_batch_eff;
}

static int seq_lockstep(mbpe_ctx *c, int ev_slot, bool *nothing_left) {
    const StreamView v = stream_view(c, kBuffers01);
    const BatchView b = batch_view(c);
    const SelectArgs sa = select_args(c);
    *nothing_left = false;
    const bool stepwise = sa.sel != nullptr;
    launch_select_batch(v, b, c->tab, c->best, sa, stepwise ? 1 : c->sel_attempts, 0, !stepwise);
    if (!c->d_seq_info) HIPCHK(hipMalloc(&c->d_seq_info, 32));
    for (int round = 0;; ++round) {
        launch_seq_info(v, b, c->best, c->d_seq_info);
        HIPCHK(hipMemcpyAsync(c->h_seq + 8, c->d_seq_info, 32, hipMemcpyDeviceToHost, c->stream));
        HIPCHK(hipEventRecord(c->ev_sel, c->stream));
        HIPCHK(hipEventSynchronize(c->ev_sel));
        if (!stepwise || round > 0 || c->h_seq[14] != 0) break;
        launch_select_batch(v, b, c->tab, c->best, sa, 3, 1, true);
    }
    const uint32_t batch_n = c->h_seq[9], fused = c->h_seq[10];
    const Inst w = inst_known(c->h_seq[11] != 0, c->h_seq[12] != 0);
    if (ev_slot >= 0) { (void)hipEventRecord(c->kev[2 * ev_slot], c->stream); (void)hipEventRecord(c->kev_f[2 * ev_slot], c->stream); }
    if (batch_n == 0) {
        if (ev_slot >= 0) { (void)hipEventRecord(c->kev_f[2 * ev_slot + 1], c->stream); (void)hipEventRecord(c->kev[2 * ev_slot + 1], c->stream); }
        *nothing_left = true;
        return MBPE_OK;
    }
    if (batch_n == 1) {
        launch_merge(v, b, c->best, 0, &c->ctl->m, 1, w);
    } else {
        if (w.tt) launch_run_lengths(v, b.bs, c->best, 1);
        if (fused) launch_fused_batch(v, b, w);
        else launch_scan_batch(v, b, w);
        launch_pair_cells_fold(v, b, batch_n);
    }
    if (ev_slot >= 0) { (void)hipEventRecord(c->kev_f[2 * ev_slot + 1], c->stream); (void)hipEventRecord(c->kev[2 * ev_slot + 1], c->stream); }
    c->k_upper = std::min<uint32_t>(c->n_target, c->h_seq[8] + batch_n);
    const uint32_t id_upper = 256 + c->k_upper;
    if (batch_n == 1) {
        launch_apply(v, b, c->tab, c->best, id_upper, nullptr, 1);
    } else {
        launch_batch_tables(v, b, c->tab, id_upper, batch_n);
        launch_rewrite_marked(v, b, w);
        launch_patch_sums(v, c->best, 1);
    }
    launch_seq_finish(v, b, seq_flags_of(c));
    return MBPE_OK;
}

static int seq_stage_a(mbpe_ctx *c, int ev_slot) {
    const StreamView v = stream_view(c, kBuffers01);
    const BatchView b = batch_view(c);
    const Inst w = inst_any(c->hot_possible != 0);
    launch_select_batch(v, b, c->tab, c->best, select_args(c), c->sel_attempts);
    if (c->opt_first) first_tiebreak(c, c->best, 1, 0);
    if (is_multi(c)) {
        const int rc = seq_info_enqueue(c);
        if (rc != MBPE_OK) return rc;
    }
    if (ev_slot >= 0) (void)hipEventRecord(c->kev[2 * ev_slot], c->stream);
    launch_merge(v, b, c->best, 0, is_multi(c) ? c->xb : &c->ctl->m, 1, w);
    launch_scan_batch(v, b, w);
    if (ev_slot >= 0) (void)hipEventRecord(c->kev_f[2 * ev_slot], c->stream);
    launch_fused_batch(v, b, w);
    launch_pair_cells_fold(v, b, batch_hint(c));
    if (ev_slot >= 0) {
        (void)hipEventRecord(c->kev_f[2 * ev_slot + 1], c->stream);
        (void)hipEventRecord(c->kev[2 * ev_slot + 1], c->stream);
    }
    return MBPE_OK;
}

static void seq_stage_b(mbpe_ctx *c) {
    const StreamView v = stream_view(c, kBuffers01);
    const BatchView b = batch_view(c);
    c->k_upper = std::min<uint32_t>(c->n_target, c->k_upper + std::min<uint32_t>((uint32_t)c->opt_max_batch, c->max_batch_eff));
    const uint32_t id_upper = 256 + c->k_upper;
    launch_batch_tables(v, b, c->tab, id_upper, batch_hint(c));
    launch_apply(v, b, c->tab, c->best, id_upper, is_multi(c) ? c->xb : nullptr, 1);
    launch_rewrite_marked(v, b, inst_any(c->hot_possible != 0));
    launch_patch_sums(v, c->best, 1);
    launch_seq_finish(v, b, seq_flags_of(c));
    if (is_multi(c)) launch_rank_edge(v, c->xb);
}

static void seq_stage_c(mbpe_ctx *c) {
    if (is_multi(c)) launch_compose_edges(c->stream, c->xb, c->rank, c->n_ranks, c->d_left, c->d_right);
}


static int phase_exchange(mbpe_ctx *c, Phase p, Exchange *x) {
    switch (p) {
    case Phase::BeginCounts: *x = {c->xb0, begin_exchange_words(c)}; return MBPE_OK;
    case Phase::StepDeltas: *x = {c->xb, exchange_words(c, 256 + c->k, 1)}; return MBPE_OK;
    case Phase::SeqDeltas: {
        uint32_t ids = 0, n_pairs = 0;
        const int rc = seq_info_wait(c, &ids, &n_pairs);
        if (rc != MBPE_OK) return rc;
        *x = {c->xb, exchange_words(c, ids, n_pairs)};
        c->stats.exchange_words += x->words;
        c->stats.exchanges++;
        return MBPE_OK;
    }
    case Phase::SeqEdges: *x = {c->xb, c->hdr_words}; return MBPE_OK;
    case Phase::BeginFirst: case Phase::StepFirst: *x = {c->xf, c->hdr_words}; return MBPE_OK;
    case Phase::None: break;
    }
    *x = {};
    return MBPE_OK;
}

static Phase continue_after(mbpe_ctx *c, Phase p) {
    switch (p) {
    case Phase::BeginCounts: begin_finish_a(c); return first_sharded(c) ? Phase::BeginFirst : Phase::None;
    case Phase::BeginFirst: first_tiebreak(c, c->best, 0, 2); return Phase::None;
    case Phase::StepDeltas: step_finish_a(c); return first_sharded(c) ? Phase::StepFirst : Phase::None;
    case Phase::StepFirst: first_tiebreak(c, c->best + c->k + 1, 0, 2); return Phase::None;
    case Phase::SeqDeltas: seq_stage_b(c); return Phase::SeqEdges;
    case Phase::SeqEdges: seq_stage_c(c); return Phase::None;
    case Phase::None: break;
    }
    return Phase::None;
}

static int comm_allreduce(mbpe_ctx *c, uint32_t *buf, size_t count);

static int finish_unit(mbpe_ctx *c, Phase p) {
    for (; p != Phase::None; p = continue_after(c, p)) {
        if (!is_multi(c)) continue;
        Exchange x = {};
        int rc = phase_exchange(c, p, &x);
        if (rc == MBPE_OK) rc = comm_allreduce(c, x.buf, x.words);
        if (rc != MBPE_OK) return rc;
    }
    return MBPE_OK;
}

static int suspend(mbpe_ctx *c, Phase p) {
    HIPCHK(hipStreamSynchronize(c->stream));
    const int rc = phase_exchange(c, p, &c->pending_x);
    if (rc != MBPE_OK) return rc;
    c->pending = p;
    return MBPE_NEED_EXCHANGE;
}

static uint64_t seq_headroom(const mbpe_ctx *c) {
    return (uint64_t)c->opt_max_batch * (2ull * c->vocab_size + kBatchMax + 1);
}
// ... 413 lines not shown
                }
                rc = after_batch(c);
                if (rc != MBPE_OK) return rc;
                break;
            }
        }
        done += batch;
        rc = after_batch(c);
        if (rc != MBPE_OK) return rc;
    }
    if (steps_done_out) *steps_done_out = done;
    return MBPE_OK;
}


static int wide_alloc_table(mbpe_ctx *c, WideTable *t, uint64_t want_entries) {
    uint32_t bits = 12;
    while ((1ull << bits) < 2 * want_entries && bits < 31) ++bits;
    if ((1ull << bits) < 2 * want_entries) { mbpe_host::set_last_error("pair table beyond 2^30 entries"); return MBPE_ERR_OVERFLOW; }
    *t = {};
    t->mask = (uint32_t)((1ull << bits) - 1);
    t->shift = 64 - bits;
    HIPCHK(tmalloc(c, &t->keys, (size_t)8 << bits));
    HIPCHK(tmalloc(c, &t->cnts, (size_t)4 << bits));
    launch_wide_table_clear(c->stream, *t);
    return MBPE_OK;
}

static uint64_t wide_headroom(unsigned long long top, uint32_t merges) { return (uint64_t)merges * (2ull * top + 2); }

static int wide_sync(mbpe_ctx *c) {
    HIPCHK(hipMemcpyAsync(&c->h_wctl, c->wctl, sizeof(WideCtl), hipMemcpyDeviceToHost, c->stream));
    HIPCHK(hipStreamSynchronize(c->stream));
    HIPCHK(hipGetLastError());
    if (c->h_wctl.err) {
        mbpe_host::set_last_error("device error: the 32-bit pair table is full");
        return MBPE_ERR_OVERFLOW;
    }
    return MBPE_OK;
}

static int wide_convert(mbpe_ctx *c) {
    int rc = sync_ctl(c);
    if (rc != MBPE_OK) return rc;
    rc = do_compact(c);
    if (rc != MBPE_OK) return rc;
    const uint64_t n_live_slots = c->h_ctl.n_live;
    const uint64_t n_tok = n_live_slots - (c->barrier ? c->n_barriers : 0);
    const uint32_t n_wide = c->n_target_total - c->n_target;
    HIPCHK(tmalloc(c, &c->wtok[0], std::max<uint64_t>(n_tok, 1) * 4));
    HIPCHK(tmalloc(c, &c->wtok[1], std::max<uint64_t>(n_tok, 1) * 4));
    HIPCHK(tmalloc(c, &c->wval, std::max<uint64_t>(n_live_slots, 1) * 4));
    HIPCHK(tmalloc(c, &c->wscratch, wide_scratch_words(n_live_slots) * 4));
    HIPCHK(tmalloc(c, &c->wctl, sizeof(WideCtl)));
    HIPCHK(tmalloc(c, &c->wbest, ((size_t)n_wide + 2) * sizeof(WideBest)));
    HIPCHK(tmalloc(c, &c->warg, 2 * 1024 * 8));
    HIPCHK(hipMemsetAsync(c->wctl, 0, sizeof(WideCtl), c->stream));
    c->wfirst = c->opt_first != 0;
    if (c->wfirst) {
        HIPCHK(tmalloc(c, &c->wfs, sizeof(WideFirst)));
        HIPCHK(hipMemsetAsync(c->wfs, 0, sizeof(WideFirst), c->stream));
        HIPCHK(hipMemsetAsync(&c->wfs->pos, 0xFF, sizeof(c->wfs->pos), c->stream));
        HIPCHK(hipMemsetD32Async(reinterpret_cast<hipDeviceptr_t>(&c->wctl->first), 1, 1, c->stream));
    }
    const uint32_t barrier = c->barrier ? kBarrier : 0xFFFFFFFFu;
    const uint32_t endbit = c->chunked && !c->barrier ? kEndBit : 0u;
    launch_wide_from_slots(c->stream, c->tok[c->cur], n_live_slots, barrier, endbit, c->wval, c->wscratch, c->wtok[0], c->wctl);
    c->wcur = 0;
    unsigned long long top = c->last_top == ~0ull ? n_tok : c->last_top;
    rc = wide_alloc_table(c, &c->wtab, (uint64_t)c->h_ctl.n_entries + wide_headroom(top, 16));
    if (rc != MBPE_OK) return rc;
    launch_wide_table_from16(c->stream, c->tab.ekey, c->tab.ecnt, c->h_ctl.n_entries, c->wtab, c->wctl);
    rc = wide_sync(c);
    if (rc != MBPE_OK) return rc;
    if (c->h_wctl.n != n_tok || c->h_wctl.n_entries != c->h_ctl.n_entries) {
        mbpe_host::set_last_error("conversion to 32-bit tokens lost tokens or pairs");
        return MBPE_ERR_OVERFLOW;
    }
    c->wn_upper = n_tok;
    c->wk = 0;
    c->h_wbest.clear();
    c->wide_active = true;
    tfree(c, c->tok[0]); tfree(c, c->tok[1]); tfree(c, c->sums); tfree(c, c->side); tfree(c, c->chg); tfree(c, c->tile_list);
    tfree(c, c->offsets); tfree(c, c->run_in); tfree(c, c->xb); tfree(c, c->pair_cells);
    tfree(c, c->tab.hslot); tfree(c, c->tab.ekey); tfree(c, c->tab.ecnt); tfree(c, c->tab.bmax); tfree(c, c->tab.smax);
    tfree(c, c->first_state);
    c->LR = nullptr;
    pool_trim(c);
    return MBPE_OK;
}

static int wide_steps(mbpe_ctx *c, uint32_t n_steps, uint32_t *done_out) {
    *done_out = 0;
    const uint32_t n_wide = c->n_target_total - c->n_target;
    uint32_t done = 0;
    unsigned long long top = c->h_wbest.empty() ? (c->last_top == ~0ull ? c->wn_upper : c->last_top)
                                                : (unsigned long long)c->h_wbest.back().count;
    while (done < n_steps && c->wk < n_wide) {
        const uint32_t group = std::min<uint32_t>({16u, n_steps - done, n_wide - c->wk});
        if (2 * ((uint64_t)c->h_wctl.n_entries + wide_headroom(top, group)) > (uint64_t)c->wtab.mask + 1) {
            WideTable old = c->wtab;
            int rc = wide_alloc_table(c, &c->wtab, 2 * ((uint64_t)c->h_wctl.n_entries + wide_headroom(top, group)));
            if (rc != MBPE_OK) return rc;
            HIPCHK(hipMemsetD32Async(reinterpret_cast<hipDeviceptr_t>(&c->wctl->n_entries), 0, 1, c->stream));
            launch_wide_rehash(c->stream, old, c->wtab, c->wctl);
            HIPCHK(hipStreamSynchronize(c->stream));
            trelease(c, old.keys); trelease(c, old.cnts);
            c->stats.n_table_grows++;
        }
        HIPCHK(hipMemsetD32Async(reinterpret_cast<hipDeviceptr_t>(&c->wctl->k_limit), (int)(c->wk + group), 1, c->stream));
        HIPCHK(hipEventRecord(c->ev0, c->stream));
        for (uint32_t g = 0; g < group; ++g) {
            launch_wide_argmax(c->stream, c->wtab, c->wctl, c->wbest, c->warg);
            if (c->wfirst)
                launch_wide_first(c->stream, c->wtok[c->wcur ^ (g & 1)], c->wn_upper, c->wtab, c->wctl, c->wbest, c->warg,
                                  c->wfs);
            launch_wide_merge(c->stream, c->wtok[c->wcur ^ (g & 1)], c->wtok[c->wcur ^ (g & 1) ^ 1], c->wn_upper, c->wval,
                              c->wscratch, c->wtab, c->wctl, 256 + c->n_target);
        }
        HIPCHK(hipEventRecord(c->ev1, c->stream));
        int rc = wide_sync(c);
        if (rc != MBPE_OK) return rc;
        float ms = 0;
        HIPCHK(hipEventElapsedTime(&ms, c->ev0, c->ev1));
        c->stats.ms_steps += ms;
        const uint32_t ran = c->h_wctl.k - c->wk;
        if (ran == 0) break;
        c->h_wbest.resize((size_t)c->wk + ran);
        HIPCHK(hipMemcpy(c->h_wbest.data() + c->wk, c->wbest + c->wk, (size_t)ran * sizeof(WideBest), hipMemcpyDeviceToHost));
        c->wcur ^= (int)(ran & 1u);
        c->wn_upper = c->h_wctl.n;
        c->wk += ran;
        done += ran;
        top = (unsigned long long)std::max(0, c->h_wbest.back().count);
        if (!c->wfirst && c->h_wbest.back().count == 0 && done < n_steps && c->wk < n_wide) {
            const uint32_t fill = std::min<uint32_t>(n_steps - done, n_wide - c->wk);
            c->h_wbest.resize((size_t)c->wk + fill, c->h_wbest.back());
            c->wk += fill;
            done += fill;
            HIPCHK(hipMemsetD32Async(reinterpret_cast<hipDeviceptr_t>(&c->wctl->k), (int)c->wk, 1, c->stream));
            HIPCHK(hipStreamSynchronize(c->stream));
            c->h_wctl.k = c->wk;
        }
        if (ran < group) break;
    }
    *done_out = done;
    return MBPE_OK;
}

int mbpe_train_sequences(mbpe_ctx *c, uint32_t n_sequences, uint32_t *merges_done_out) {
    if (merges_done_out) *merges_done_out = 0;
    if (!c) return MBPE_ERR_ARG;
    if (!c->begun) { mbpe_host::set_last_error("mbpe_train_sequences before mbpe_train_begin"); return MBPE_ERR_STATE; }
    if (c->pending != Phase::None || (is_multi(c) && c->comm_external)) {
        mbpe_host::set_last_error("mbpe_train_sequences: not available with an external transport (use mbpe_train_steps)");
        return MBPE_ERR_STATE;
    }
    if (c->wide_active || (c->wide && c->k >= c->n_target))
        return mbpe_train_steps(c, n_sequences, merges_done_out);
    if (!use_batches(c)) return mbpe_train_steps(c, n_sequences, merges_done_out);
    HIPCHK(hipSetDevice(c->device));
    return train_steps_batched(c, c->n_target, merges_done_out, n_sequences);
}

int mbpe_comm_exchange_buffer(mbpe_ctx *c, void **dev_ptr_out, uint64_t *n_u32_out) {
    if (!c || !dev_ptr_out || !n_u32_out) return MBPE_ERR_ARG;
    if (c->pending == Phase::None) { mbpe_host::set_last_error("no exchange pending"); return MBPE_ERR_STATE; }
    *dev_ptr_out = c->pending_x.buf;
    *n_u32_out = c->pending_x.words;
    return MBPE_OK;
}

int mbpe_comm_exchange_done(mbpe_ctx *c) {
    if (!c) return MBPE_ERR_ARG;
    HIPCHK(hipSetDevice(c->device));
    const Phase p = c->pending;
    if (p == Phase::None) { mbpe_host::set_last_error("no exchange pending"); return MBPE_ERR_STATE; }
    c->pending = Phase::None;
    const Phase next = continue_after(c, p);
    if (next != Phase::None) return suspend(c, next);
    if (p == Phase::BeginCounts || p == Phase::BeginFirst) return begin_end(c);
    const bool batched = p == Phase::SeqEdges;
    if (!batched) c->k++;
    int rc = sync_ctl(c);
    if (rc != MBPE_OK) return rc;
    HIPCHK(hipGetLastError());
    const uint32_t before = c->k;
    if (batched) c->k = c->h_ctl.k_done;
    rc = after_batch(c);
    if (rc != MBPE_OK) return rc;
    if (c->k >= c->pending_target || (batched && c->k == before)) return MBPE_OK;
    return start_unit_external(c, batched);
}

int mbpe_train_result(mbpe_ctx *c, uint32_t *merges_out, int32_t *counts_out, uint32_t cap_merges,
                      uint32_t *n_merges_out) {
    if (!c) return MBPE_ERR_ARG;
    if (!c->begun) { mbpe_host::set_last_error("mbpe_train_result before mbpe_train_begin"); return MBPE_ERR_STATE; }
    HIPCHK(hipSetDevice(c->device));
    uint32_t n = c->exhausted ? c->n_prior : c->n_valid;
    std::vector<unsigned long long> h(n);
    if (n) HIPCHK(hipMemcpy(h.data(), c->best, (size_t)n * 8, hipMemcpyDeviceToHost));
    if (c->opt_first) {
        uint32_t real = 0;
        while (real < n && (h[real] >> 32) != 0) ++real;
        n = real;
    }
    const uint32_t nw = c->wide_active ? (uint32_t)c->h_wbest.size() : 0u;
    if (n_merges_out) *n_merges_out = n + nw;
    if (n + nw > cap_merges && merges_out) { mbpe_host::set_last_error("merges_out too small"); return MBPE_ERR_ARG; }
    if (!(n + nw) || !merges_out) return MBPE_OK;
    for (uint32_t i = 0; i < n; ++i) {
        uint32_t key = ~(uint32_t)h[i];
        merges_out[2 * i] = key >> 16;
        merges_out[2 * i + 1] = key & 0xFFFFu;
        if (counts_out) counts_out[i] = (int32_t)(h[i] >> 32);
    }
    for (uint32_t i = 0; i < nw; ++i) {
        merges_out[2 * (n + i)] = c->h_wbest[i].first;
        merges_out[2 * (n + i) + 1] = c->h_wbest[i].second;
        if (counts_out) counts_out[n + i] = c->h_wbest[i].count;
    }
    return MBPE_OK;
}

int mbpe_get_stats(mbpe_ctx *c, mbpe_stats *out) {
    if (!c || !out) return MBPE_ERR_ARG;
    c->stats.n_slots = c->begun ? c->n_slots : 0;
    c->stats.n_live = c->begun ? c->h_ctl.n_live - (c->barrier ? c->n_barriers : 0) : 0;
    c->stats.n_merges = c->exhausted ? c->n_prior : c->n_valid;
    c->stats.n_pairs = c->begun ? c->h_ctl.n_entries : 0;
    c->stats.n_batches = c->begun ? (use_batches(c) ? c->h_ctl.n_batches : c->k - c->n_prior) : 0;
    c->stats.n_fused = c->begun ? c->h_ctl.n_fused : 0;
    c->stats.n_fused_dropped = c->begun ? c->h_ctl.n_fused_dropped : 0;
    c->stats.cut_conflict = c->begun ? c->h_ctl.cut_conflict : 0;
    c->stats.cut_bucket = c->begun ? c->h_ctl.cut_bucket : 0;
    c->stats.cut_single = c->begun ? c->h_ctl.cut_single : 0;
    c->stats.cut_full = c->begun ? c->h_ctl.cut_full : 0;
    c->stats.n_validation_drops = c->begun ? c->h_ctl.n_validation_drops : 0;
    c->stats.n_sel_fallback = c->begun ? c->h_ctl.n_sel_fallback : 0;
    c->stats.n_sel_retry = c->begun ? c->h_ctl.n_sel_retry : 0;
    c->stats.adapt_limit = c->begun ? c->h_ctl.adapt_limit : 0;
    c->stats.n_sel_blocks = c->begun ? c->h_ctl.n_sel_blocks : 0;
    for (int i = 0; i < 8; ++i) c->stats.size_hist[i] = c->begun ? c->h_ctl.size_hist[i] : 0;
    c->stats.n_skipped = c->begun ? c->h_ctl.n_skipped : 0;
    c->stats.n_skip_cut = c->begun ? c->h_ctl.n_skip_cut : 0;
    if (c->begun && c->wide_active) {
        c->stats.n_slots = c->h_wctl.n;
        c->stats.n_live = c->h_wctl.n;
        c->stats.n_merges += (uint32_t)c->h_wbest.size();
        c->stats.n_pairs = c->h_wctl.n_entries;
        c->stats.n_batches += c->wk;
    }
    *out = c->stats;
    return MBPE_OK;
}

int mbpe_train(mbpe_ctx *c, const uint8_t *text, uint64_t n_bytes, const uint64_t *chunk_off, uint64_t n_chunks,
               uint32_t vocab_size, int conflict_resolution, uint32_t *merges_out, int32_t *counts_out,
               uint32_t *n_merges_out, mbpe_stats *stats_out) {
    return mbpe_train_from(c, text, n_bytes, chunk_off, n_chunks, vocab_size, conflict_resolution, nullptr, 0, merges_out,
                           counts_out, n_merges_out, stats_out);
}

int mbpe_train_from(mbpe_ctx *c, const uint8_t *text, uint64_t n_bytes, const uint64_t *chunk_off, uint64_t n_chunks,
                    uint32_t vocab_size, int conflict_resolution, const uint32_t *prior_merges, uint32_t n_prior,
                    uint32_t *merges_out, int32_t *counts_out, uint32_t *n_merges_out, mbpe_stats *stats_out) {
    if (!c || !merges_out) { mbpe_host::set_last_error("mbpe_train: NULL argument"); return MBPE_ERR_ARG; }
    if (conflict_resolution != 0 && conflict_resolution != 1) {
        mbpe_host::set_last_error("conflict_resolution: 0 = first, 1 = lexical");
        return MBPE_ERR_ARG;
    }
    int rc = mbpe_load_corpus(c, text, n_bytes, chunk_off, n_chunks, 0);
    if (rc != MBPE_OK) return rc;
    const int64_t keep = c->opt_first;
    c->opt_first = conflict_resolution == 0;
    rc = mbpe_train_begin_from(c, vocab_size, prior_merges, n_prior);
    if (rc == MBPE_OK) rc = mbpe_train_steps(c, vocab_size - 256, nullptr);
    if (rc == MBPE_OK) rc = mbpe_train_result(c, merges_out, counts_out, vocab_size - 256, n_merges_out);
    if (rc == MBPE_OK && stats_out) mbpe_get_stats(c, stats_out);
    c->opt_first = keep;
    return rc;
}

int mbpe_train_lexical(mbpe_ctx *c, const uint8_t *text, uint64_t n_bytes, const uint64_t *chunk_off,
                       uint64_t n_chunks, uint32_t vocab_size, uint32_t *merges_out, int32_t *counts_out,
                       uint32_t *n_merges_out, mbpe_stats *stats_out) {
    return mbpe_train(c, text, n_bytes, chunk_off, n_chunks, vocab_size, 1, merges_out, counts_out, n_merges_out,
                      stats_out);
}

int mbpe_get_stream(mbpe_ctx *c, uint32_t *tokens_out, uint8_t *chunk_end_out, uint64_t cap, uint64_t *n_out) {
    if (!c || !n_out) return MBPE_ERR_ARG;
    if (!c->begun) { mbpe_host::set_last_error("mbpe_get_stream before mbpe_train_begin"); return MBPE_ERR_STATE; }
    HIPCHK(hipSetDevice(c->device));
    HIPCHK(hipStreamSynchronize(c->stream));
    if (c->wide_active) {
        const uint64_t n = c->h_wctl.n;
        *n_out = n;
        if (!tokens_out) return MBPE_OK;
        if (cap < n) { mbpe_host::set_last_error("tokens_out too small"); return MBPE_ERR_ARG; }
        if (n) HIPCHK(hipMemcpy(tokens_out, c->wtok[c->wcur], n * 4, hipMemcpyDeviceToHost));
        for (uint64_t i = 0; i < n; ++i) {
            if (chunk_end_out) chunk_end_out[i] = c->chunked ? (uint8_t)(tokens_out[i] >> 31) : 0;
            tokens_out[i] &= kTokIdMask;
        }
        return MBPE_OK;
    }
    std::vector<uint16_t> h(c->n_slots);
    HIPCHK(hipMemcpy(h.data(), c->tok[c->cur], c->n_slots * 2, hipMemcpyDeviceToHost));
    const bool endflag = c->chunked && !c->barrier;
    const uint32_t idmask = endflag ? 0x7FFFu : 0xFFFFu;
    uint64_t w = 0;
    for (uint64_t i = 0; i < c->n_slots; ++i) {
        if (h[i] == kHole) continue;
        if (c->barrier && h[i] == kBarrier) {
            if (tokens_out && chunk_end_out && w) chunk_end_out[w - 1] = 1;
            continue;
        }
        if (tokens_out) {
            if (w >= cap) { mbpe_host::set_last_error("tokens_out too small"); return MBPE_ERR_ARG; }
            tokens_out[w] = h[i] & idmask;
            if (chunk_end_out) chunk_end_out[w] = endflag ? (h[i] >> 15) & 1 : 0;
// ... 190 lines not shown
```

### minbpe-cc_amd/python/mbpe/__init__.py

```python
import ctypes
import os

import numpy as np

_PKG_DIR = os.path.dirname(os.path.dirname(os.path.dirname(os.path.abspath(__file__))))
LIB_PATH = os.environ.get("MBPE_LIB") or os.path.join(_PKG_DIR, "libmbpe.so")

OK = 0
NEED_EXCHANGE = 1
ERR_ARG, ERR_NO_DEVICE, ERR_HIP, ERR_VOCAB, ERR_STATE = -1, -2, -3, -4, -5
ERR_OOM, ERR_REGEX, ERR_SPLIT_GAP, ERR_COMM, ERR_OVERFLOW, ERR_IO = -6, -7, -8, -9, -10, -11
COMM_ID_BYTES = 128

EXPORTS = [
    "mbpe_last_error", "mbpe_version", "mbpe_create", "mbpe_destroy", "mbpe_load_corpus",
    "mbpe_pair_count_u8", "mbpe_train_begin", "mbpe_train_steps", "mbpe_train_sequences", "mbpe_train_result",
    "mbpe_train_lexical", "mbpe_train", "mbpe_get_stats", "mbpe_get_stream", "mbpe_stream_device", "mbpe_table_device", "mbpe_get_pairs", "mbpe_compact",
    "mbpe_set_option", "mbpe_comm_unique_id", "mbpe_comm_init", "mbpe_comm_init_external",
    "mbpe_comm_exchange_buffer", "mbpe_comm_exchange_done", "mbpe_presplit",
    "mbpe_split_count", "mbpe_split_offsets", "mbpe_split_has_gaps", "mbpe_split_starts", "mbpe_split_ends",
    "mbpe_split_free", "mbpe_load_corpus_ranges", "mbpe_split_pattern", "mbpe_encode_chunks",
    "mbpe_encode_chunks_device", "mbpe_decoder_create", "mbpe_decoder_destroy", "mbpe_decode_tokens",
    "mbpe_decode_slots", "mbpe_decoder_kernel_ms", "mbpe_decode_stream", "mbpe_encoder_create",
    "mbpe_encoder_destroy", "mbpe_encoder_encode", "mbpe_encoder_set_option", "mbpe_encoder_kernel_ms",
    "mbpe_encoder_alloc_count", "mbpe_encoder_pass_tokens", "mbpe_decode_batch", "mbpe_decoder_alloc_count",
    "mbpe_pack_tokens", "mbpe_unpack_tokens", "mbpe_pack_kernel_ms", "mbpe_encoder_encode_batch", "mbpe_encoder_pack_ms",
    "mbpe_pack_tokens_aux", "mbpe_pack_cu_seqlens", "mbpe_encoder_encode_batch_aux",
    "mbpe_load_corpus_endmask", "mbpe_splitter_create", "mbpe_splitter_destroy", "mbpe_splitter_split",
    "mbpe_splitter_endmask", "mbpe_splitter_set_option", "mbpe_splitter_kernel_ms", "mbpe_splitter_alloc_count",
    "mbpe_splitter_host_spans", "mbpe_splitter_split_docs", "mbpe_splitter_ranges", "mbpe_splitter_find_ms",
    "mbpe_encoder_encode_endmask", "mbpe_encoder_encode_batch_endmask", "mbpe_split_unicode_table",
    "mbpe_merges_check", "mbpe_train_begin_from", "mbpe_train_from",
]
TOK_EXPORTS = [
    "mbpe_tok_create", "mbpe_tok_destroy", "mbpe_tok_set_special_tokens", "mbpe_tok_train", "mbpe_tok_set_merges",
    "mbpe_tok_get_merges", "mbpe_tok_save", "mbpe_tok_load", "mbpe_tok_encode", "mbpe_tok_encode_device",
    "mbpe_tok_decode", "mbpe_tok_decode_device", "mbpe_tok_encode_batch_device", "mbpe_tok_decode_batch_device",
    "mbpe_tok_encode_batch_packed_device", "mbpe_tok_decode_padded_device", "mbpe_tok_encode_batch_aux_device",
    "mbpe_tok_train_split_device", "mbpe_tok_set_encode_split", "mbpe_tok_set_split_unicode",
    "mbpe_tok_set_encode_order", "mbpe_tok_train_continue",
]


class Stats(ctypes.Structure):
    _fields_ = [
        ("n_bytes", ctypes.c_uint64), ("n_chunks", ctypes.c_uint64), ("n_slots", ctypes.c_uint64),
        ("n_live", ctypes.c_uint64), ("n_merges", ctypes.c_uint32), ("n_compactions", ctypes.c_uint32),
        ("n_pairs", ctypes.c_uint64), ("ms_pair_count", ctypes.c_float), ("ms_begin", ctypes.c_float),
        ("ms_steps", ctypes.c_float), ("pair_count_launches", ctypes.c_uint32), ("merge_launches", ctypes.c_uint32),
        ("ms_merge_kernel", ctypes.c_float), ("n_batches", ctypes.c_uint32),
        ("n_fused", ctypes.c_uint32), ("n_fused_dropped", ctypes.c_uint32), ("cut_conflict", ctypes.c_uint32),
        ("cut_bucket", ctypes.c_uint32), ("cut_single", ctypes.c_uint32), ("cut_full", ctypes.c_uint32),
        ("n_validation_drops", ctypes.c_uint32), ("ms_grow_table", ctypes.c_float), ("ms_compact", ctypes.c_float),
        ("n_table_grows", ctypes.c_uint32), ("n_sel_fallback", ctypes.c_uint32),
        ("fused_launches", ctypes.c_uint32), ("ms_fused_kernel", ctypes.c_float), ("fused_slots", ctypes.c_uint64),
        ("n_sel_retry", ctypes.c_uint32), ("adapt_limit", ctypes.c_uint32), ("n_sel_blocks", ctypes.c_uint64), ("size_hist", ctypes.c_uint32 * 8),
        ("n_skipped", ctypes.c_uint32), ("n_skip_cut", ctypes.c_uint32),
        ("exchange_words", ctypes.c_uint64), ("exchanges", ctypes.c_uint32), ("pad_", ctypes.c_uint32),
        ("fused_live_tokens", ctypes.c_uint64), ("ms_pair_count_kernel", ctypes.c_float), ("pad2_", ctypes.c_uint32),
    ]

    def as_dict(self):
        d = {k: getattr(self, k) for k, _ in self._fields_}
        d["size_hist"] = list(self.size_hist)
        return d



PACK_PADDED, PACK_PACKED = 0, 1
SPLIT_BLOCK, SPLIT_TILE, SPLIT_MAX_SPAN = 64, 16384, 4096
NO_TOKEN = 0xFFFFFFFF


class PackSpec(ctypes.Structure):
    _fields_ = [
        ("layout", ctypes.c_uint32), ("seq_len", ctypes.c_uint32), ("out_bits", ctypes.c_uint32),
        ("pad_id", ctypes.c_uint32), ("bos_id", ctypes.c_uint32), ("eos_id", ctypes.c_uint32),
        ("pad_left", ctypes.c_uint32), ("trunc_left", ctypes.c_uint32),
    ]


class PackAux(ctypes.Structure):
    _fields_ = [
        ("labels", ctypes.c_void_p), ("pos", ctypes.c_void_p), ("seg", ctypes.c_void_p),
        ("ignore_label", ctypes.c_int64),
    ]


_ID_DTYPES = {16: np.uint16, 32: np.uint32, 64: np.uint64}
_LABEL_DTYPES = {16: np.uint16, 32: np.int32, 64: np.int64}


def pack_spec(seq_len, layout="padded", out_bits=32, pad_id=0, bos_id=None, eos_id=None, pad_left=False,
              trunc_left=False):
    if isinstance(layout, str):
        if layout not in ("padded", "packed"):
            raise ValueError("layout must be \"padded\" or \"packed\"")
        layout = PACK_PADDED if layout == "padded" else PACK_PACKED
    return PackSpec(layout, seq_len, out_bits, pad_id, NO_TOKEN if bos_id is None else bos_id,
                    NO_TOKEN if eos_id is None else eos_id, int(bool(pad_left)), int(bool(trunc_left)))


class MbpeError(RuntimeError):
    def __init__(self, code, msg):
        super().__init__("mbpe error %d: %s" % (code, msg))
        self.code = code


_lib = None


def lib():
    global _lib
    if _lib is not None:
        return _lib
    if not os.path.exists(LIB_PATH):
        raise ImportError("libmbpe.so is not built (%s); run __graft_entry__.build()" % LIB_PATH)
    L = ctypes.CDLL(LIB_PATH)
    vp, u64, u32, i32, i64 = ctypes.c_void_p, ctypes.c_uint64, ctypes.c_uint32, ctypes.c_int, ctypes.c_int64
    L.mbpe_last_error.restype = ctypes.c_char_p
    L.mbpe_version.restype = ctypes.c_char_p
    L.mbpe_create.argtypes = [i32, ctypes.POINTER(vp)]
    L.mbpe_destroy.argtypes = [vp]
    L.mbpe_destroy.restype = None
    L.mbpe_load_corpus.argtypes = [vp, vp, u64, vp, u64, i32]
    L.mbpe_pair_count_u8.argtypes = [vp, vp]
    L.mbpe_train_begin.argtypes = [vp, u32]
    L.mbpe_train_steps.argtypes = [vp, u32, vp]
    L.mbpe_train_sequences.argtypes = [vp, u32, vp]
    L.mbpe_train_result.argtypes = [vp, vp, vp, u32, vp]
    L.mbpe_train_lexical.argtypes = [vp, vp, u64, vp, u64, u32, vp, vp, vp, vp]
    L.mbpe_train.argtypes = [vp, vp, u64, vp, u64, u32, i32, vp, vp, vp, vp]
    L.mbpe_merges_check.argtypes = [vp, u32]
    L.mbpe_train_begin_from.argtypes = [vp, u32, vp, u32]
    L.mbpe_train_from.argtypes = [vp, vp, u64, vp, u64, u32, i32, vp, u32, vp, vp, vp, vp]
    L.mbpe_get_stats.argtypes = [vp, vp]
    L.mbpe_get_stream.argtypes = [vp, vp, vp, u64, vp]
    L.mbpe_stream_device.argtypes = [vp, ctypes.POINTER(vp), ctypes.POINTER(u64), ctypes.POINTER(u32), ctypes.POINTER(u32),
                                     ctypes.POINTER(u32)]
    L.mbpe_table_device.argtypes = [vp, ctypes.POINTER(vp), ctypes.POINTER(u32)]
    L.mbpe_get_pairs.argtypes = [vp, vp, vp, vp, u64, vp]
    L.mbpe_compact.argtypes = [vp]
# ... 1140 lines not shown
```

Measured before the change: 80760 merges/s.

## Replace dense pair-cell atomic table with per-wave delta log and partitioned consume

Instead of doing atomic adds into a dense max_batch×65536 pair-cell table and folding it afterwards, the scan and fused kernels now append compact delta records to a device log. Each wave claims chunks of the log with one atomic. A planning kernel sizes per-bucket partitions, and a partition/consume pass bucket-sorts the records before applying them. The aim is to remove scattered global atomics and the cost of folding a large table, at the price of extra kernels, chunk-refill atomics, and a spill path back to direct atomics when the log fills.

```diff
diff --git a/include/mbpe.h b/include/mbpe.h
--- a/include/mbpe.h
+++ b/include/mbpe.h
@@ -70,10 +70,12 @@
     uint32_t n_skip_cut;
     uint64_t exchange_words;
     uint32_t exchanges;
-    uint32_t pad_;
+    uint32_t log_spilled;
     uint64_t fused_live_tokens;
     float    ms_pair_count_kernel;
-    uint32_t pad2_;
+    uint32_t log_passes;
+    uint32_t log_refills;
+    uint32_t pad3_;
 } mbpe_stats;
 
 MBPE_API const char *mbpe_last_error(void);
diff --git a/minbpe-cc_amd/csrc/kernels.hip b/minbpe-cc_amd/csrc/kernels.hip
--- a/minbpe-cc_amd/csrc/kernels.hip
+++ b/minbpe-cc_amd/csrc/kernels.hip
@@ -2392,6 +2392,47 @@
     return __ballot(need) != 0ull || hneed;
 }
 
+struct LogWave {
+    uint32_t pos, end;
+    uint32_t cap, chunk;
+    bool full;
+    uint32_t spilled;
+    LogState *ls;
+    uint32_t *refills;
+};
+__device__ __forceinline__ LogWave log_wave(LogState *ls, bool use_log, const DevCtl *ctl) {
+    return LogWave{0u, 0u, use_log ? rfl(ls->cap) : 0u, use_log ? rfl(ls->chunk) : 0u, false, 0u, ls,
+                   const_cast<uint32_t *>(&ctl->log_refills)};
+}
+__device__ __forceinline__ void log_pad(const LogWave &lw, __amdgpu_buffer_rsrc_t log_rsrc) {
+    for (uint32_t i = lw.pos + lane_id(); i < lw.end; i += kWave)
+        __builtin_amdgcn_raw_buffer_store_b32(kLogNull, log_rsrc, i << 2, 0, 0);
+}
+__device__ __forceinline__ void log_refill(LogWave *lw, __amdgpu_buffer_rsrc_t log_rsrc) {
+    log_pad(*lw, log_rsrc);
+    uint32_t base = 0;
+    if (lane_id() == 0) {
+        if (lw->end) atomicAdd(lw->refills, 1u);
+        base = atomicAdd(&lw->ls->cursor, lw->chunk);
+    }
+    base = rfl(base);
+    if (base <= lw->cap - lw->chunk) {
+        lw->pos = base;
+        lw->end = base + lw->chunk;
+    } else {
+        lw->pos = lw->end = 0u;
+        lw->full = true;
+    }
+}
+__device__ __forceinline__ void log_finish(const LogWave &lw, __amdgpu_buffer_rsrc_t log_rsrc, const DevCtl *ctl) {
+    log_pad(lw, log_rsrc);
+    const uint32_t sp = wave_sum(lw.spilled);
+    if (lane_id() == 0 && sp) {
+        atomicAdd(const_cast<uint32_t *>(&ctl->cell_hits), sp);
+        atomicAdd(const_cast<uint32_t *>(&ctl->log_spilled), sp);
+    }
+}
+
 template <int MODE, int DIAG, bool WRITE, bool TT, class DC>
 __device__ __forceinline__ uint4 fused_tile_pf(const uint4 q_orig, const uint32_t s[8], const Halo h,
                                                uint32_t old_x, uint32_t old_y, uint32_t old_z, const BatchLut &lut,
@@ -2399,9 +2440,10 @@
                                                DC &dc, bool dc_on, uint32_t &wave_rm, bool &wrote_sum,
                                                __amdgpu_buffer_rsrc_t lr_rsrc, uint32_t adj_pitch, uint16_t *stage,
                                                uint32_t *chg, bool renamed, TTInfo *ti, bool &need_rename,
-                                               __amdgpu_buffer_rsrc_t t_rsrc = __amdgpu_buffer_rsrc_t(), bool use_t = false);
-
-template <int MODE, bool HOT, bool TT, int DIAG = 0>
+                                               __amdgpu_buffer_rsrc_t log_rsrc = __amdgpu_buffer_rsrc_t(), bool use_log = false,
+                                               LogWave *lw = nullptr);
+
+template <int MODE, bool HOT, bool TT, int DIAG = 0, bool LOG = false>
 __global__ __launch_bounds__(kLutThreads) void k_scan_batch(const uint16_t *tok0, const uint16_t *tok1,
                                                               const TileSum *__restrict__ sin, uint32_t n_tiles,
                                                               uint32_t *__restrict__ chg, const BatchState *bs,
@@ -2409,7 +2451,7 @@
                                                               const DevCtl *ctl, const RankEdge *le,
                                                               const RankEdge *re,
                                                               const uint32_t *__restrict__ run_in, int hot_launched,
-                                                              uint32_t *T) {
+                                                              uint32_t *dlog, LogState *ls) {
     constexpr uint32_t idmask = MODE == 1 ? 0x7FFFu : 0xFFFFu;
     __shared__ BatchLutMem lut_mem;
     const uint32_t waves_per_block = kLutThreads / kWave;
@@ -2429,6 +2471,9 @@
     lut_build(lut, bs, n_keys, idmask - 1u);
     if (TT) tt_build(ti, bs, n_keys, idmask - 1u);
     uint32_t tile = rfl(blockIdx.x * waves_per_block + threadIdx.x / kWave);
+    LogWave lw = log_wave(ls, false, ctl);
+    __amdgpu_buffer_rsrc_t lw_rsrc = __amdgpu_buffer_rsrc_t();
+    bool lw_on = false;
     if (tile < n_tiles) {
 
     const uint32_t last_tile = n_tiles - 1;
@@ -2436,8 +2481,12 @@
     const __amdgpu_buffer_rsrc_t sums_rsrc =
         __builtin_amdgcn_make_buffer_rsrc(const_cast<TileSum *>(sin), 0, n_tiles * 16u, 0x00020000);
     const __amdgpu_buffer_rsrc_t lr_rsrc = __builtin_amdgcn_make_buffer_rsrc(LR, 0, 0xFFFFFFFCu, 0x00020000);
-    const bool use_t = T != nullptr && !HOT && ctl->cells_on != 0u && n_keys >= ctl->cells_min;
-    const __amdgpu_buffer_rsrc_t t_rsrc = __builtin_amdgcn_make_buffer_rsrc(T ? T : LR, 0, T ? 0xFFFFFFFCu : 0u, 0x00020000);
+    const bool use_log = LOG && !HOT && dlog != nullptr && rfl(ls->on) != 0u;
+    const __amdgpu_buffer_rsrc_t log_rsrc =
+        __builtin_amdgcn_make_buffer_rsrc(use_log ? dlog : LR, 0, use_log ? rfl(ls->cap) << 2 : 0u, 0x00020000);
+    lw = log_wave(ls, use_log, ctl);
+    lw_rsrc = log_rsrc;
+    lw_on = use_log;
     TileIn t0 = tile_issue(tok, sums_rsrc, tile);
     TileIn t1 = tile_issue(tok, sums_rsrc, clamp_tile((uint64_t)tile + n_waves));
     bool v1 = (uint64_t)tile + n_waves < n_tiles;
@@ -2464,7 +2513,7 @@
             if (TT) tt_rename<MODE>(s, h, ti, run_in[tile]);
             fused_tile_pf<MODE, 0, false, TT>(t0.q, s, h, rlane(t0.smw, 4), rlane(t0.smw, 5), rlane(t0.smw, 6), lut,
                                               256u + ctl_k_done, tile, nullptr, hdr_adj, LR, dc, dc_on, rm_unused, ws_unused,
-                                              lr_rsrc, adj_pitch, nullptr, chg, TT, &ti, no_rename, t_rsrc, use_t);
+                                              lr_rsrc, adj_pitch, nullptr, chg, TT, &ti, no_rename, log_rsrc, use_log, &lw);
         }
         if (!v1) break;
         tile += n_waves;
@@ -2472,6 +2521,7 @@
         v1 = v2;
     }
     }
+    if (lw_on) log_finish(lw, lw_rsrc, ctl);
     if (dc_on) dc_flush(dc, LR);
     if (TT) {
         tt_flush(ti, hdr_m);
@@ -2485,7 +2535,7 @@
                                                DC &dc, bool dc_on, uint32_t &wave_rm, bool &wrote_sum,
                                                __amdgpu_buffer_rsrc_t lr_rsrc, uint32_t adj_pitch, uint16_t *stage,
                                                uint32_t *chg, bool renamed, TTInfo *ti, bool &need_rename,
-                                               __amdgpu_buffer_rsrc_t t_rsrc, bool use_t) {
+                                               __amdgpu_buffer_rsrc_t log_rsrc, bool use_log, LogWave *lw) {
     constexpr uint32_t idmask = MODE == 1 ? 0x7FFFu : 0xFFFFu;
     constexpr uint32_t endbit = MODE == 1 ? kEndBit : 0u;
     constexpr uint32_t kNone = 0xFFFFu;
@@ -2598,11 +2648,20 @@
         const uint32_t li = live - 1u;
         if (lane == (li >> 3)) n2_patch = li & 7u;
     }
+    bool logging = false;
+    uint32_t lpos = 0;
+    if (use_log) {
+        if (lw->end - lw->pos < kLogChunkMin && !lw->full) log_refill(lw, log_rsrc);
+        logging = lw->end - lw->pos >= kLogChunkMin;
+        lpos = lw->pos;
+    }
     uint32_t out[8];
 #pragma unroll
     for (int j = 0; j < 8; ++j) {
         const uint32_t self = s[j];
         uint32_t nv = ((Bm >> j) & 1u) ? kHole : self;
+        bool el = false;
+        uint32_t rec = 0;
         if (__ballot(((Am >> j) & 1u) != 0u) != 0ull) {
             if ((Am >> j) & 1u) {
                 const uint32_t p1 = j == 0 ? prev7 >> 16 : s[j > 0 ? j - 1 : 0];
@@ -2617,9 +2676,12 @@
                 if (DIAG != 2) {
                     const bool lo = left_open<MODE>(p1), ro = right_open<MODE>(btok, n2);
                     const uint32_t xl = p1 & idmask, yr = n2 & idmask;
-                    if (use_t && lo && ro && ppj == kNone && xl < 256u && yr < 256u) {
-                        __builtin_amdgcn_raw_ptr_buffer_atomic_add_i32(1, t_rsrc, ((ja << 16) | (xl << 8) | yr) << 2, 0, 0);
+                    const bool elig = use_log && lo && ro && ppj == kNone && xl < 256u && yr < 256u;
+                    if (elig && logging) {
+                        el = true;
+                        rec = (ja << 16) | (xl << 8) | yr;
                     } else {
+                        if (elig) lw->spilled += 1u;
                         if (lo) {
                             if (ppj != kNone) {
                                 atomicAdd(&hdr_adj[ppj * adj_pitch + ja], 1u);
@@ -2632,9 +2694,16 @@
                     }
                 }
             }
+            if (logging) {
+                const uint64_t m = __ballot(el);
+                const uint32_t at = __builtin_amdgcn_mbcnt_hi((uint32_t)(m >> 32), __builtin_amdgcn_mbcnt_lo((uint32_t)m, 0u));
+                if (el) __builtin_amdgcn_raw_buffer_store_b32(rec, log_rsrc, (lpos + at) << 2, 0, 0);
+                lpos += (uint32_t)__popcll(m);
+            }
         }
         out[j] = nv;
     }
+    if (logging) lw->pos = lpos;
     if (TT && renamed) {
 #pragma unroll
         for (int j = 0; j < 8; ++j)
@@ -2677,7 +2746,7 @@
 #ifndef MBPE_FUSED_WAVES
 #define MBPE_FUSED_WAVES 4
 #endif
-template <int MODE, bool HOT, bool TT, int DIAG = 0>
+template <int MODE, bool HOT, bool TT, int DIAG = 0, bool LOG = false>
 __global__ __launch_bounds__(kLutThreads, MBPE_FUSED_WAVES * 256 / kLutThreads) void k_fused_batch(uint16_t *tok0, uint16_t *tok1,
                                                                const TileSum *__restrict__ sin,
                                                                TileSum *__restrict__ sout, uint32_t n_tiles,
@@ -2685,7 +2754,7 @@
                                                                uint32_t *hdr_adj, uint32_t *LR, DevCtl *ctl,
                                                                const RankEdge *le, const RankEdge *re,
                                                                uint32_t *hdr_m, const uint32_t *__restrict__ run_in,
-                                                               int hot_launched, uint32_t *T) {
+                                                               int hot_launched, uint32_t *dlog, LogState *ls) {
     constexpr uint32_t idmask = MODE == 1 ? 0x7FFFu : 0xFFFFu;
     __shared__ BatchLutMem lut_mem;
     const uint32_t lane = lane_id();
@@ -2710,6 +2779,9 @@
     if (blockIdx.x == 0 && threadIdx.x == 0) ctl->marks_all = 1;
     uint32_t tile = rfl(blockIdx.x * waves_per_block + threadIdx.x / kWave);
     uint32_t wave_rm = 0;
+    LogWave lw = log_wave(ls, false, ctl);
+    __amdgpu_buffer_rsrc_t lw_rsrc = __amdgpu_buffer_rsrc_t();
+    bool lw_on = false;
     if (tile < n_tiles) {
 
     const uint32_t last_tile = n_tiles - 1;
@@ -2717,8 +2789,12 @@
     const __amdgpu_buffer_rsrc_t sums_rsrc =
         __builtin_amdgcn_make_buffer_rsrc(const_cast<TileSum *>(sin), 0, n_tiles * 16u, 0x00020000);
     const __amdgpu_buffer_rsrc_t lr_rsrc = __builtin_amdgcn_make_buffer_rsrc(LR, 0, 0xFFFFFFFCu, 0x00020000);
-    const bool use_t = T != nullptr && !HOT && ctl->cells_on != 0u && n_keys >= ctl->cells_min;
-    const __amdgpu_buffer_rsrc_t t_rsrc = __builtin_amdgcn_make_buffer_rsrc(T ? T : LR, 0, T ? 0xFFFFFFFCu : 0u, 0x00020000);
+    const bool use_log = LOG && !HOT && dlog != nullptr && rfl(ls->on) != 0u;
+    const __amdgpu_buffer_rsrc_t log_rsrc =
+        __builtin_amdgcn_make_buffer_rsrc(use_log ? dlog : LR, 0, use_log ? rfl(ls->cap) << 2 : 0u, 0x00020000);
+    lw = log_wave(ls, use_log, ctl);
+    lw_rsrc = log_rsrc;
+    lw_on = use_log;
     const uint32_t adj_pitch = rfl(ctl->adj_pitch);
 #ifndef MBPE_FUSED_DEPTH
 #define MBPE_FUSED_DEPTH 2
@@ -2771,12 +2847,12 @@
             }
             outq = fused_tile_pf<MODE, DIAG, true, TT>(t0.q, s, h, old_x, old_y, old_z, lut, X0, tile, sout, hdr_adj, LR, dc,
                                                        dc_on, wave_rm, wrote_sum, lr_rsrc, adj_pitch, stage, chg, renamed, &ti,
-                                                       need_rename, t_rsrc, use_t);
+                                                       need_rename, log_rsrc, use_log, &lw);
             if (TT && need_rename) {
                 tt_rename<MODE>(s, h, ti, run_in[tile]);
                 outq = fused_tile_pf<MODE, DIAG, true, TT>(t0.q, s, h, old_x, old_y, old_z, lut, X0, tile, sout, hdr_adj, LR,
                                                            dc, dc_on, wave_rm, wrote_sum, lr_rsrc, adj_pitch, stage, chg, true,
-                                                           &ti, need_rename, t_rsrc, use_t);
+                                                           &ti, need_rename, log_rsrc, use_log, &lw);
             }
         }
         if (!wrote_sum && lane == 0) reinterpret_cast<uint4 *>(sout)[tile] = make_uint4(old_x, old_y, old_z, 0u);
@@ -2792,6 +2868,7 @@
         ring[kDepth - 1] = t_new;
     }
     }
+    if (lw_on) log_finish(lw, lw_rsrc, ctl);
     if (dc_on) dc_flush(dc, LR);
     if (lane == 0 && wave_rm) atomicAdd(&ctl->rm, wave_rm);
     if (TT) {
@@ -2799,35 +2876,149 @@
     }
 }
 
-__global__ __launch_bounds__(256) void k_pair_cells_fold(uint32_t *__restrict__ T, uint32_t *__restrict__ LR, const DevCtl *ctl) {
-    __shared__ uint32_t rows[256];
+static_assert(kLogBuckets <= (uint32_t)kWave, "k_log_plan and the scans of k_log_partition: one lane per bucket");
+constexpr uint32_t kLogBucketShift = 22;
+
+__global__ __launch_bounds__(kWave) void k_log_plan(DevCtl *ctl, const BatchState *bs, LogState *ls) {
+    const uint32_t b = threadIdx.x;
     const uint32_t n = ctl->batch_n;
-    if (n < ctl->cells_min || !ctl->cells_on) return;
+    bool on = n >= 2u && ctl->cells_on != 0u && n >= ctl->cells_min;
+    if (on) on = !dc_wanted(bs->packed[0] >> 32, ctl->n_live * ctl->n_ranks);
+    unsigned long long cnt = 0;
+    if (on && b < kLogBuckets) {
+        const uint32_t j1 = n < (b + 1u) * kLogBucketPairs ? n : (b + 1u) * kLogBucketPairs;
+        for (uint32_t j = b * kLogBucketPairs; j < j1; ++j) cnt += bs->packed[j] >> 32;
+    }
+    unsigned long long incl = cnt;
+#pragma unroll
+    for (int d = 1; d < kWave; d <<= 1) {
+        const unsigned long long t = __shfl_up(incl, d, kWave);
+        if (b >= (uint32_t)d) incl += t;
+    }
+    const unsigned long long total = __shfl(incl, kWave - 1, kWave);
+    const bool fits = total <= (unsigned long long)ls->part_cap;
+    if (b == 0u) ctl->log_refused = on && !fits ? 1u : 0u;
+    on = on && fits;
+    if (b < kLogBuckets) {
+        ls->base[b + 1u] = on ? (uint32_t)incl : 0u;
+        ls->fill[b] = 0u;
+    }
+    if (b == 0u) {
+        ls->base[0] = 0u;
+        ls->on = on ? 1u : 0u;
+        ls->cursor = 0u;
+        ls->n_buckets = (n + kLogBucketPairs - 1u) / kLogBucketPairs;
+    }
+}
+
+constexpr int kPartThreads = 1024;
+constexpr uint32_t kLogSlice = 8192;
+static_assert(kLogChunkMin % 8u == 0u, "a thread's 8 records never straddle the end of the log");
+
+__global__ __launch_bounds__(kPartThreads) void k_log_partition(const uint32_t *__restrict__ dlog, uint32_t *__restrict__ part,
+                                                                LogState *ls, DevCtl *ctl) {
+    __shared__ uint32_t hist[kWave];
+    __shared__ uint32_t off[kWave + 1];
+    __shared__ uint32_t gb[kWave];
+    __shared__ uint32_t room[kWave];
+    __shared__ uint32_t sorted[kLogSlice];
+    if (!ls->on) return;
+    const uint32_t tid = threadIdx.x;
+    const uint32_t cursor = ls->cursor, cap = ls->cap;
+    const uint32_t n_rec = cursor < cap ? cursor : cap;
+    const uint32_t n_slices = (n_rec + kLogSlice - 1u) / kLogSlice;
+    for (uint32_t sl = blockIdx.x; sl < n_slices; sl += gridDim.x) {
+        if (tid < (uint32_t)kWave) hist[tid] = 0;
+        __syncthreads();
+        const uint32_t r0 = sl * kLogSlice + tid * 8u;
+        uint32_t rec[8];
+        if (r0 < n_rec) {
+            const uint4 q0 = reinterpret_cast<const uint4 *>(dlog + r0)[0], q1 = reinterpret_cast<const uint4 *>(dlog + r0)[1];
+            rec[0] = q0.x; rec[1] = q0.y; rec[2] = q0.z; rec[3] = q0.w;
+            rec[4] = q1.x; rec[5] = q1.y; rec[6] = q1.z; rec[7] = q1.w;
+        } else {
+#pragma unroll
+            for (int u = 0; u < 8; ++u) rec[u] = kLogNull;
+        }
+#pragma unroll
+        for (int u = 0; u < 8; ++u) {
+            if ((rec[u] >> kLogBucketShift) >= kLogBuckets) rec[u] = kLogNull;
+            if (rec[u] != kLogNull) atomicAdd(&hist[rec[u] >> kLogBucketShift], 1u);
+        }
+        __syncthreads();
+        if (tid < (uint32_t)kWave) {
+            const uint32_t a = hist[tid];
+            uint32_t incl = a;
+#pragma unroll
+            for (int d = 1; d < kWave; d <<= 1) {
+                const uint32_t t = __shfl_up(incl, d, kWave);
+                if (tid >= (uint32_t)d) incl += t;
+            }
+            off[tid] = incl - a;
+            if (tid == (uint32_t)kWave - 1u) off[kWave] = incl;
+            if (a && tid < kLogBuckets) {
+                const uint32_t at = atomicAdd(&ls->fill[tid], a);
+                const uint32_t size = ls->base[tid + 1u] - ls->base[tid];
+                gb[tid] = ls->base[tid] + at;
+                room[tid] = at >= size ? 0u : size - at < a ? size - at : a;
+                if (room[tid] < a) atomicOr(&ctl->err, kErrLog);
+            }
+            hist[tid] = 0;
+        }
+        __syncthreads();
+#pragma unroll
+        for (int u = 0; u < 8; ++u) {
+            if (rec[u] == kLogNull) continue;
+            const uint32_t bk = rec[u] >> kLogBucketShift;
+            const uint32_t r = atomicAdd(&hist[bk], 1u);
+            sorted[off[bk] + r] = rec[u];
+        }
+        __syncthreads();
+        const uint32_t n_sorted = off[kWave];
+        for (uint32_t t = tid; t < n_sorted; t += kPartThreads) {
+            const uint32_t v = sorted[t];
+            const uint32_t bk = v >> kLogBucketShift;
+            if (t - off[bk] < room[bk]) part[gb[bk] + (t - off[bk])] = v;
+        }
+        __syncthreads();
+    }
+}
+
+constexpr int kCountThreads = 1024;
+constexpr uint32_t kLogBucketCells = kLogBucketPairs * 512u;
+
+__global__ __launch_bounds__(kCountThreads) void k_log_count(const uint32_t *__restrict__ part, uint32_t *LR, const LogState *ls,
+                                                             DevCtl *ctl) {
+    __shared__ uint32_t hist[kLogBucketCells];
+    if (!ls->on) return;
+    const uint32_t P = ls->n_buckets;
+    const uint32_t S = P >= (uint32_t)gridDim.x ? 1u : (uint32_t)gridDim.x / P > 64u ? 64u : (uint32_t)gridDim.x / P;
+    const uint32_t tid = threadIdx.x;
     const uint32_t pitch = lr_pitch(256u + ctl->k_done);
-    uint32_t hits = 0;
-    const uint32_t t = threadIdx.x;
-    for (uint32_t j = blockIdx.x; j < n; j += gridDim.x) {
-        uint32_t *tj = T + (size_t)j * 65536u;
-        rows[t] = 0;
+    if (blockIdx.x == 0 && tid == 0 && ls->cursor) ctl->log_passes += 1u;
+    for (uint32_t w = blockIdx.x; w < P * S; w += gridDim.x) {
+        const uint32_t b = w / S, share = w - b * S;
+        const uint32_t start = ls->base[b];
+        uint32_t n = ls->fill[b];
+        if (n > ls->base[b + 1u] - start) n = ls->base[b + 1u] - start;
+        const uint32_t lo = (uint32_t)((uint64_t)n * share / S), hi = (uint32_t)((uint64_t)n * (share + 1u) / S);
+        if (lo == hi) continue;
+        for (uint32_t i = tid; i < kLogBucketCells; i += kCountThreads) hist[i] = 0;
         __syncthreads();
-        uint32_t col = 0;
-#pragma unroll 8
-        for (uint32_t x = 0; x < 256u; ++x) {
-            const uint32_t v = tj[x * 256u + t];
-            if (__ballot(v != 0u) == 0ull) continue;
-            if (v) tj[x * 256u + t] = 0;
-            col += v;
-            const uint32_t rs = wave_sum(v);
-            if (lane_id() == 0 && rs) atomicAdd(&rows[x], rs);
+        for (uint32_t i = lo + tid; i < hi; i += kCountThreads) {
+            const uint32_t v = part[start + i];
+            const uint32_t jl = (v >> 16) & (kLogBucketPairs - 1u);
+            atomicAdd(&hist[jl * 512u + ((v >> 8) & 255u)], 1u);
+            atomicAdd(&hist[jl * 512u + 256u + (v & 255u)], 1u);
         }
         __syncthreads();
-        if (col) LR[lr_idx(pitch, t, j, 1u)] += col;
-        if (rows[t]) LR[lr_idx(pitch, t, j, 0u)] += rows[t];
-        hits += col;
+        for (uint32_t i = tid; i < kLogBucketCells; i += kCountThreads) {
+            const uint32_t c = hist[i];
+            if (c) atomicAdd(&LR[lr_idx(pitch, i & 255u, b * kLogBucketPairs + (i >> 9), (i >> 8) & 1u)], c);
+        }
+        if (tid == 0) atomicAdd(&ctl->cell_hits, hi - lo);
         __syncthreads();
     }
-    hits = wave_sum(hits);
-    if (lane_id() == 0 && hits) atomicAdd(const_cast<uint32_t *>(&ctl->cell_hits), hits);
 }
 
 
@@ -3339,7 +3530,7 @@
         ctl->skip_penalty /= 2u;
     }
     ctl->skip_failed = 0;
-    if (ctl->cells_on && ctl->cells_min >= kCellsMinBatch && ctl->batch_n >= ctl->cells_min &&
+    if (ctl->cells_on && ctl->cells_min >= kCellsMinBatch && ctl->batch_n >= ctl->cells_min && !ctl->log_refused &&
         ctl->cell_hits * 2ull < (unsigned long long)rm_seq)
         ctl->cells_on = 0;
     ctl->cell_hits = 0;
@@ -3993,7 +4184,7 @@
     const dim3 grid(tile_grid(v.n_tiles, v.n_cus, occ[slot_mode(v.endbit)], kLutThreads)), block(kLutThreads);
     const int hot_launched = w.hot;
 #define MBPE_FUSED_ARGS v.tok, v.tok_other, v.sums, v.side, v.n_tiles, v.chg, b.bs, b.hdr_adj, b.LR, v.ctl, v.left_edge, \
-                        v.right_edge, b.hdr_m, v.run_in, hot_launched, b.pair_cells
+                        v.right_edge, b.hdr_m, v.run_in, hot_launched, b.dlog, b.ls
 #ifdef MBPE_DIAG
     const int diag = getenv("MBPE_FUSED_DIAG") ? atoi(getenv("MBPE_FUSED_DIAG")) : 0;
 #define MBPE_FUSED_DIAG_CASE(D)                                                                                            \
@@ -4009,7 +4200,10 @@
     MBPE_FUSED_DIAG_CASE(6)
 #undef MBPE_FUSED_DIAG_CASE
 #endif
-    MBPE_BY_MODE(v.endbit, MBPE_BY_INST(w, hipLaunchKernelGGL((k_fused_batch<M, HOT, TT>), grid, block, 0, v.stream, MBPE_FUSED_ARGS)));
+    if (b.dlog)
+        MBPE_BY_MODE(v.endbit, MBPE_BY_INST(w, hipLaunchKernelGGL((k_fused_batch<M, HOT, TT, 0, !HOT>), grid, block, 0, v.stream, MBPE_FUSED_ARGS)));
+    else
+        MBPE_BY_MODE(v.endbit, MBPE_BY_INST(w, hipLaunchKernelGGL((k_fused_batch<M, HOT, TT, 0, false>), grid, block, 0, v.stream, MBPE_FUSED_ARGS)));
 #undef MBPE_FUSED_ARGS
 }
 
@@ -4020,17 +4214,25 @@
                                resident_blocks(k_scan_batch<2, false, false, 0>, kLutThreads)};
     const dim3 grid(tile_grid(v.n_tiles, v.n_cus, occ[slot_mode(v.endbit)], kLutThreads)), block(kLutThreads);
     const int hot_launched = w.hot;
-    MBPE_BY_MODE(v.endbit, MBPE_BY_INST(w, hipLaunchKernelGGL((k_scan_batch<M, HOT, TT, 0>), grid, block, 0, v.stream, v.tok,
-                                                             v.tok_other, v.sums, v.n_tiles, v.chg, b.bs, b.hdr_m, b.hdr_adj, b.LR,
-                                                             v.ctl, v.left_edge, v.right_edge, v.run_in, hot_launched,
-                                                             b.pair_cells)));
-}
-
-void launch_pair_cells_fold(const StreamView &v, const BatchView &b, uint32_t n_hint) {
-    if (!b.pair_cells) return;
-    if (n_hint < 64u) n_hint = 64u;
-    if (n_hint > 1024u) n_hint = 1024u;
-    hipLaunchKernelGGL(k_pair_cells_fold, dim3(n_hint), dim3(256), 0, v.stream, b.pair_cells, b.LR, v.ctl);
+#define MBPE_SCAN_ARGS v.tok, v.tok_other, v.sums, v.n_tiles, v.chg, b.bs, b.hdr_m, b.hdr_adj, b.LR, v.ctl, v.left_edge, \
+                       v.right_edge, v.run_in, hot_launched, b.dlog, b.ls
+    if (b.dlog)
+        MBPE_BY_MODE(v.endbit, MBPE_BY_INST(w, hipLaunchKernelGGL((k_scan_batch<M, HOT, TT, 0, !HOT>), grid, block, 0, v.stream, MBPE_SCAN_ARGS)));
+    else
+        MBPE_BY_MODE(v.endbit, MBPE_BY_INST(w, hipLaunchKernelGGL((k_scan_batch<M, HOT, TT, 0, false>), grid, block, 0, v.stream, MBPE_SCAN_ARGS)));
+#undef MBPE_SCAN_ARGS
+}
+
+void launch_log_plan(const StreamView &v, const BatchView &b) {
+    if (!b.dlog) return;
+    hipLaunchKernelGGL(k_log_plan, dim3(1), dim3(kWave), 0, v.stream, v.ctl, b.bs, b.ls);
+}
+
+void launch_log_consume(const StreamView &v, const BatchView &b) {
+    if (!b.dlog) return;
+    const int cus = v.n_cus > 0 ? v.n_cus : 256;
+    hipLaunchKernelGGL(k_log_partition, dim3(cus * 2), dim3(kPartThreads), 0, v.stream, b.dlog, b.part, b.ls, v.ctl);
+    hipLaunchKernelGGL(k_log_count, dim3(cus), dim3(kCountThreads), 0, v.stream, b.part, b.LR, b.ls, v.ctl);
 }
 
 void launch_batch_tables(const StreamView &v, const BatchView &b, PairTable t, uint32_t id_upper, uint32_t n_hint) {
diff --git a/minbpe-cc_amd/csrc/mbpe_dev.h b/minbpe-cc_amd/csrc/mbpe_dev.h
--- a/minbpe-cc_amd/csrc/mbpe_dev.h
+++ b/minbpe-cc_amd/csrc/mbpe_dev.h
@@ -99,6 +99,10 @@
     uint32_t cell_hits;
     uint32_t cells_min;
     uint32_t adj_pitch;
+    uint32_t log_spilled;
+    uint32_t log_passes;
+    uint32_t log_refills;
+    uint32_t log_refused;
 
 };
 
@@ -129,6 +133,23 @@
 #endif
 constexpr int kSkipMax = MBPE_SKIP_MAX;
 constexpr uint32_t kCellsMinBatch = 512;
+
+constexpr uint32_t kLogNull = 0xFFFFFFFFu;
+constexpr uint32_t kLogBucketPairs = 64;
+constexpr uint32_t kLogBuckets = (uint32_t)MBPE_BATCH_MAX / kLogBucketPairs;
+constexpr uint32_t kLogChunkMin = 256;
+constexpr uint32_t kLogChunkDefault = 4096;
+static_assert(MBPE_BATCH_MAX % 64 == 0 && MBPE_BATCH_MAX <= 65536, "a record holds the pair index in 16 bits");
+struct LogState {
+    uint32_t cap;
+    uint32_t chunk;
+    uint32_t part_cap;
+    uint32_t on;
+    uint32_t cursor;
+    uint32_t n_buckets;
+    uint32_t base[kLogBuckets + 1];
+    uint32_t fill[kLogBuckets];
+};
 constexpr uint32_t kNoTT = 0xFFFFFFFFu;
 struct BatchState {
     uint32_t key[kBatchMax];
@@ -159,6 +180,7 @@
 constexpr uint32_t kErrMissingPair = 4u;
 constexpr uint32_t kErrCountRange  = 8u;
 constexpr uint32_t kErrHotSkipped  = 16u;
+constexpr uint32_t kErrLog         = 32u;
 
 __host__ __device__ inline unsigned long long pack_best(int32_t count, uint32_t key) {
     return ((unsigned long long)(uint32_t)count << 32) | (uint32_t)(~key);
@@ -185,7 +207,8 @@
     BatchState *bs;
     uint32_t *hdr_m, *hdr_adj;
     uint32_t *LR;
-    uint32_t *pair_cells;
+    uint32_t *dlog, *part;
+    LogState *ls;
 };
 
 struct Inst { bool known, tt, hot; };
@@ -238,7 +261,8 @@
                          bool fallback = true );
 void launch_scan_batch(const StreamView &v, const BatchView &b, const Inst &w);
 void launch_fused_batch(const StreamView &v, const BatchView &b, const Inst &w);
-void launch_pair_cells_fold(const StreamView &v, const BatchView &b, uint32_t n_hint);
+void launch_log_plan(const StreamView &v, const BatchView &b);
+void launch_log_consume(const StreamView &v, const BatchView &b);
 void launch_batch_tables(const StreamView &v, const BatchView &b, PairTable t, uint32_t id_upper, uint32_t n_hint);
 void launch_rewrite_marked(const StreamView &v, const BatchView &b, const Inst &w);
 void launch_seq_info(const StreamView &v, const BatchView &b, const unsigned long long *best, uint32_t *out);
diff --git a/minbpe-cc_amd/csrc/train.cpp b/minbpe-cc_amd/csrc/train.cpp
--- a/minbpe-cc_amd/csrc/train.cpp
+++ b/minbpe-cc_amd/csrc/train.cpp
@@ -143,7 +143,9 @@
     BatchState *bs = nullptr;
     uint32_t *xb0 = nullptr;
     uint32_t h_pcount[kPairCountWords] = {};
-    uint32_t *pair_cells = nullptr;
+    uint32_t *dlog = nullptr;
+    uint32_t *dpart = nullptr;
+    LogState *log_state = nullptr;
     RankEdge *d_left = nullptr, *d_right = nullptr;
 
     uint32_t vocab_size = 0;
@@ -192,6 +194,9 @@
     uint32_t *h_seq = nullptr;
     uint32_t *d_seq_info = nullptr;
     int64_t opt_pair_cells = -1;
+    int64_t opt_log_cap = 0;
+    int64_t opt_log_chunk = 0;
+    LogState h_log = {};
     int64_t opt_lockstep = -1;
     hipEvent_t ev_sel = nullptr;
     std::vector<hipEvent_t> kev;
@@ -285,7 +290,7 @@
         char buf[320];
         snprintf(buf, sizeof(buf), "device error flags 0x%x (1=pair table full, 2=negative count, 4=missing pair, "
                                    "8=a pair occurs 2^31 times or more, or the byte-pair counts do not add up to the "
-                                   "pairs scanned (a count reached 2^32), 16=a stream pass was skipped)",
+                                   "pairs scanned (a count reached 2^32), 16=a stream pass was skipped, 32=delta log overflow)",
                  c->h_ctl.err);
         mbpe_host::set_last_error(buf);
         return MBPE_ERR_OVERFLOW;
@@ -314,7 +319,8 @@
     tfree(c, c->offsets);
     tfree(c, c->tab.hslot); tfree(c, c->tab.ekey); tfree(c, c->tab.ecnt); tfree(c, c->tab.cells);
     tfree(c, c->tab.bmax); tfree(c, c->tab.smax);
-    tfree(c, c->ctl); tfree(c, c->best); tfree(c, c->xb); tfree(c, c->xb0); tfree(c, c->pair_cells);
+    tfree(c, c->ctl); tfree(c, c->best); tfree(c, c->xb); tfree(c, c->xb0); tfree(c, c->dlog); tfree(c, c->dpart);
+    tfree(c, c->log_state);
     tfree(c, c->d_left); tfree(c, c->d_right); tfree(c, c->bs); tfree(c, c->sel); tfree(c, c->seq_flags); tfree(c, c->run_in);
     tfree(c, c->first_state);
     tfree(c, c->xf);
@@ -462,7 +468,7 @@
     return v;
 }
 
-BatchView batch_view(const mbpe_ctx *c) { return BatchView{c->bs, c->hdr_m, c->hdr_adj, c->LR, c->pair_cells}; }
+BatchView batch_view(const mbpe_ctx *c) { return BatchView{c->bs, c->hdr_m, c->hdr_adj, c->LR, c->dlog, c->dpart, c->log_state}; }
 
 int do_compact(mbpe_ctx *c) {
     if (!c->n_tiles) return MBPE_OK;
@@ -572,6 +578,8 @@
     else if (n == "byte_table") c->opt_byte_table = value != 0;
     else if (n == "lockstep") c->opt_lockstep = value < 0 ? -1 : value != 0;
     else if (n == "pair_cells") c->opt_pair_cells = value < 0 ? -1 : value != 0;
+    else if (n == "log_cap") c->opt_log_cap = value < 0 ? 0 : std::min<int64_t>(value, 1ll << 29);
+    else if (n == "log_chunk") c->opt_log_chunk = value < 0 ? 0 : std::min<int64_t>(value, 1ll << 16);
     else if (n == "wide_from") c->opt_wide_from = value < 0 ? -1 : value;
     else if (n == "first_wide") c->opt_first_wide = value != 0;
     else if (n == "pc_repeat") c->opt_pc_repeat = std::min<int64_t>(std::max<int64_t>(1, value), 1000);
@@ -875,9 +883,20 @@
     HIPCHK(hipMemsetAsync(c->xb, 0, xb_words * 4, c->stream));
     HIPCHK(hipMemsetAsync(c->xb0, 0, xb0_words * 4, c->stream));
     if (c->opt_pair_cells > 0 || (c->opt_pair_cells < 0 && c->n_slots >= (64ull << 20))) {
-        const size_t cells = (size_t)c->max_batch_eff * 65536u;
-        HIPCHK(tmalloc(c, &c->pair_cells, cells * 4));
-        HIPCHK(hipMemsetAsync(c->pair_cells, 0, cells * 4, c->stream));
+        LogState &init = c->h_log;
+        init = LogState{};
+        const uint64_t half = c->n_slots / 2 + 1;
+        uint64_t cap = c->opt_log_cap > 0 ? (uint64_t)c->opt_log_cap : std::min<uint64_t>(std::max<uint64_t>(half / 8, 1u << 20), 1u << 28);
+        uint64_t chunk = c->opt_log_chunk > 0 ? (uint64_t)c->opt_log_chunk : std::min<uint64_t>(kLogChunkDefault, cap / 8192);
+        chunk = std::max<uint64_t>(kLogChunkMin, std::min<uint64_t>(chunk, 1u << 16) / kLogChunkMin * kLogChunkMin);
+        cap = std::max<uint64_t>(chunk, std::min<uint64_t>(cap, 1u << 29) / chunk * chunk);
+        init.cap = (uint32_t)cap;
+        init.chunk = (uint32_t)chunk;
+        init.part_cap = (uint32_t)std::min<uint64_t>(half, 1u << 29);
+        HIPCHK(tmalloc(c, &c->dlog, (size_t)init.cap * 4));
+        HIPCHK(tmalloc(c, &c->dpart, (size_t)init.part_cap * 4));
+        HIPCHK(tmalloc(c, &c->log_state, sizeof(LogState)));
+        HIPCHK(hipMemcpyAsync(c->log_state, &init, sizeof(LogState), hipMemcpyHostToDevice, c->stream));
     }
     c->hdr_m = c->xb + c->hdr_words;
     c->hdr_adj = c->hdr_m + kBatchMax;
@@ -908,7 +927,7 @@
         init.n_ranks = (uint32_t)std::max(1, c->n_ranks);
         init.first_mode = c->opt_first ? 1u : 0u;
         init.adj_pitch = c->adj_pitch;
-        init.cells_on = c->pair_cells ? 1u : 0u;
+        init.cells_on = c->dlog ? 1u : 0u;
         init.cells_min = c->opt_pair_cells > 0 ? 2u : kCellsMinBatch;
         c->h_ctl = init;
         HIPCHK(hipMemcpyAsync(c->ctl, &c->h_ctl, sizeof(DevCtl), hipMemcpyHostToDevice, c->stream));
@@ -1140,9 +1159,10 @@
         launch_merge(v, b, c->best, 0, &c->ctl->m, 1, w);
     } else {
         if (w.tt) launch_run_lengths(v, b.bs, c->best, 1);
+        launch_log_plan(v, b);
         if (fused) launch_fused_batch(v, b, w);
         else launch_scan_batch(v, b, w);
-        launch_pair_cells_fold(v, b, batch_n);
+        launch_log_consume(v, b);
     }
     if (ev_slot >= 0) { (void)hipEventRecord(c->kev_f[2 * ev_slot + 1], c->stream); (void)hipEventRecord(c->kev[2 * ev_slot + 1], c->stream); }
     c->k_upper = std::min<uint32_t>(c->n_target, c->h_seq[8] + batch_n);
@@ -1170,10 +1190,11 @@
     }
     if (ev_slot >= 0) (void)hipEventRecord(c->kev[2 * ev_slot], c->stream);
     launch_merge(v, b, c->best, 0, is_multi(c) ? c->xb : &c->ctl->m, 1, w);
+    launch_log_plan(v, b);
     launch_scan_batch(v, b, w);
     if (ev_slot >= 0) (void)hipEventRecord(c->kev_f[2 * ev_slot], c->stream);
     launch_fused_batch(v, b, w);
-    launch_pair_cells_fold(v, b, batch_hint(c));
+    launch_log_consume(v, b);
     if (ev_slot >= 0) {
         (void)hipEventRecord(c->kev_f[2 * ev_slot + 1], c->stream);
         (void)hipEventRecord(c->kev[2 * ev_slot + 1], c->stream);
@@ -1753,7 +1774,7 @@
     c->h_wbest.clear();
     c->wide_active = true;
     tfree(c, c->tok[0]); tfree(c, c->tok[1]); tfree(c, c->sums); tfree(c, c->side); tfree(c, c->chg); tfree(c, c->tile_list);
-    tfree(c, c->offsets); tfree(c, c->run_in); tfree(c, c->xb); tfree(c, c->pair_cells);
+    tfree(c, c->offsets); tfree(c, c->run_in); tfree(c, c->xb); tfree(c, c->dlog); tfree(c, c->dpart); tfree(c, c->log_state);
     tfree(c, c->tab.hslot); tfree(c, c->tab.ekey); tfree(c, c->tab.ecnt); tfree(c, c->tab.bmax); tfree(c, c->tab.smax);
     tfree(c, c->first_state);
     c->LR = nullptr;
@@ -1910,6 +1931,9 @@
     c->stats.cut_full = c->begun ? c->h_ctl.cut_full : 0;
     c->stats.n_validation_drops = c->begun ? c->h_ctl.n_validation_drops : 0;
     c->stats.n_sel_fallback = c->begun ? c->h_ctl.n_sel_fallback : 0;
+    c->stats.log_spilled = c->begun ? c->h_ctl.log_spilled : 0;
+    c->stats.log_passes = c->begun ? c->h_ctl.log_passes : 0;
+    c->stats.log_refills = c->begun ? c->h_ctl.log_refills : 0;
     c->stats.n_sel_retry = c->begun ? c->h_ctl.n_sel_retry : 0;
     c->stats.adapt_limit = c->begun ? c->h_ctl.adapt_limit : 0;
     c->stats.n_sel_blocks = c->begun ? c->h_ctl.n_sel_blocks : 0;
diff --git a/minbpe-cc_amd/python/mbpe/__init__.py b/minbpe-cc_amd/python/mbpe/__init__.py
--- a/minbpe-cc_amd/python/mbpe/__init__.py
+++ b/minbpe-cc_amd/python/mbpe/__init__.py
@@ -56,8 +56,9 @@
         ("fused_launches", ctypes.c_uint32), ("ms_fused_kernel", ctypes.c_float), ("fused_slots", ctypes.c_uint64),
         ("n_sel_retry", ctypes.c_uint32), ("adapt_limit", ctypes.c_uint32), ("n_sel_blocks", ctypes.c_uint64), ("size_hist", ctypes.c_uint32 * 8),
         ("n_skipped", ctypes.c_uint32), ("n_skip_cut", ctypes.c_uint32),
-        ("exchange_words", ctypes.c_uint64), ("exchanges", ctypes.c_uint32), ("pad_", ctypes.c_uint32),
-        ("fused_live_tokens", ctypes.c_uint64), ("ms_pair_count_kernel", ctypes.c_float), ("pad2_", ctypes.c_uint32),
+        ("exchange_words", ctypes.c_uint64), ("exchanges", ctypes.c_uint32), ("log_spilled", ctypes.c_uint32),
+        ("fused_live_tokens", ctypes.c_uint64), ("ms_pair_count_kernel", ctypes.c_float), ("log_passes", ctypes.c_uint32),
+        ("log_refills", ctypes.c_uint32), ("pad3_", ctypes.c_uint32),
     ]
 
     def as_dict(self):
```

After: 84250 merges/s (median of 6 runs). +4.3%, better.
